# rezashkv/unlearn-ft

Hardware: AMD Instinct MI355X
Metric: bilevel train-step images/sec @512^2 pruned-SD2.1 (higher is better)
Workload: dtype bf16; 1 GPU; BASELINE configs[1] model+batch (MAC-budget-0.55 SD-2.1 student [ratio 0.556, 223.7 GMAC/img] + dense teacher [402.1 GMAC/img], B=8/GPU, 64x64 latents = 512^2 px, losses 1.0 ddpm(min-SNR 5) + 2.0 distill + 0.1 block) under the bilevel cadence of configs[2] (upper concept-suppression step every 10th iteration, second AdamW); global_batch=8, parallelism=dp1, student_params=483766084, weights=random-init, attention_precision=activation dtype, dist_backend=none, rccl_ranks=0, dp_mode=allreduce, teacher_prefetch=True

## Files before the change

### include/pdmk.h

```cpp
#ifndef PDMK_H
#define PDMK_H
#include <stdint.h>
#ifdef __cplusplus
extern "C" {
#endif

#define PDMK_F32 0
#define PDMK_BF16 1

typedef void* pdmk_stream;

int pdmk_version(void);

#define PDMK_A_ROWK 0
#define PDMK_A_CONV 1
#define PDMK_A_COLK 2
#define PDMK_B_ROWK 0
#define PDMK_B_COLK 1
#define PDMK_B_COLK_CONV 2

typedef struct pdmk_gemm_args {
    const void* A;
    const void* B;
    void* C;
    const float* bias;
    const float* rowvec;
    const void* R;
    float* colsum_out;
    int32_t M, N, K;
    int32_t lda, ldb, ldc, ldr;
    int32_t rows_per_b;
    int32_t a_mode, b_mode;
    int32_t conv_b, conv_hi, conv_wi, conv_ci, conv_ho, conv_wo, conv_mode, conv_ld;
    int32_t dtype;
    int32_t out_f32;
    int32_t accumulate;
    int32_t splitk;
    float alpha;
    int32_t ldrv;
    int32_t epilogue;
    int32_t ldc2;
    void* C2;
    int64_t* colstat;
    int32_t cs_ld;
    int32_t cs_col0;
    const float* ln_gamma;
    const float* ln_beta;
    float* ln_stats;
    void* ln_out;
    int32_t ld_ln_out;
    float ln_eps;
} pdmk_gemm_args;
int pdmk_gemm_ln_supported(const pdmk_gemm_args* args);

#define PDMK_EPI_NONE 0
#define PDMK_EPI_GEGLU 1
#define PDMK_EPI_GEGLU_BWD 2

int pdmk_gemm(const pdmk_gemm_args* args, pdmk_stream stream);
int pdmk_conv_up2_supported(int B, int H, int W, int Ci, int Co, int dtype);
int pdmk_groupnorm_apply_colstat(const void* x, void* y, const float* gamma, const float* beta, float* stats, const int64_t* colstat,
                                 int cs_ld, int cs_col0, int B, int HW, int C, int ldx, int ldy, int G, int gs, float eps,
                                 int silu, int dtype, pdmk_stream stream);
int pdmk_up2_pack_weights(const float* w3, void* wp, void* wpt, int Co, int Ci, int dtype, pdmk_stream stream);
int pdmk_up2_combine_wgrad(const float* dwp, float* dw3, int Co, int Ci, pdmk_stream stream);
#define PDMK_COLSTAT_SCALE 1073741824.0
#define PDMK_GEMM_GROUP_MAX 8
int pdmk_gemm_group(const pdmk_gemm_args* args, int n, pdmk_stream stream, int32_t* grouped_out);
int pdmk_gemm_plan(const pdmk_gemm_args* args, pdmk_stream stream, int32_t* splitk_out);
int pdmk_gemm_last_candidate(void);
int pdmk_gemm_candidate_name(int a_mode, int b_mode, int id, char* buf, int n);
int pdmk_splitk_finish(const float* ws, void* C, const float* bias, const float* rowvec, const void* R, int64_t M,
                       int N, int ldc, int ldr, int rows_per_b, int ldrv , int nslab ,
                       int accumulate, int dtype, pdmk_stream stream);
int pdmk_splitk_finish_colstat(const float* ws, void* C, const float* bias, const float* rowvec, const void* R, int64_t M,
                               int N, int ldc, int ldr, int rows_per_b, int ldrv, int nslab, int accumulate, int64_t* colstat,
                               int cs_ld, int cs_col0, int dtype, pdmk_stream stream);
#define PDMK_SLAB_GROUP_MAX 32
typedef struct pdmk_slab_item {
    const float* ws;
    float* dst;
    int64_t n;
    int32_t nslab, pad_;
} pdmk_slab_item;
int pdmk_splitk_finish_group(const pdmk_slab_item* items, int n_items, pdmk_stream stream);
int64_t pdmk_gemm_splitk_workspace_bytes(int64_t M, int N, int splitk);

int pdmk_plan_export(const char* path);
int pdmk_plan_import(const char* path);
int pdmk_plan_size(void);
int pdmk_plan_clear(void);
int pdmk_debug_scratch_violations(void);

int pdmk_groupnorm_fwd(const void* x, void* y, const float* gamma, const float* beta, float* stats, double* ws,
                       int B, int HW, int C, int ldx, int ldy, int G, int gs, float eps, int silu, int dtype,
                       pdmk_stream stream);
int pdmk_groupnorm_bwd(const void* x, const void* dy, void* dx, const float* gamma, const float* beta,
                       const float* stats, float* dgamma, float* dbeta, double* ws, float* part_ws,
                       int64_t part_ws_elems, int B, int HW, int C, int ldx, int lddy, int lddx, int G, int gs,
                       int silu, int accumulate_dx, const void* add, int ldadd, int dtype, pdmk_stream stream);
#define PDMK_PARTIAL_GROUP_MAX 32
typedef struct pdmk_partial_item {
    const float* part;
    float* out0;
    float* out1;
    int32_t nblk, n;
} pdmk_partial_item;
int pdmk_groupnorm_bwd_partial_dims(int B, int HW, int C, int G, int gs, int dtype, int32_t* nblk, int32_t* n);
int pdmk_layernorm_bwd_partial_dims(int M, int C, int32_t* nblk, int32_t* n);
int pdmk_reduce_partials_group(const pdmk_partial_item* items, int n_items, pdmk_stream stream);
int64_t pdmk_groupnorm_workspace_bytes(int B, int G);
int64_t pdmk_groupnorm_bwd_part_workspace_bytes(int G, int gs);

int pdmk_layernorm_fwd(const void* x, void* y, const float* gamma, const float* beta, float* stats, int M, int C,
                       int ldx, int ldy, float eps, int dtype, pdmk_stream stream);
int pdmk_layernorm_bwd(const void* x, const void* dy, void* dx, const float* gamma, const float* stats,
                       float* dgamma, float* dbeta, float* part_ws, int64_t part_ws_elems ,
                       int M, int C, int ldx, int lddy, int lddx, int accumulate_dx, const void* add, int ldadd, int dtype,
                       pdmk_stream stream);
int64_t pdmk_layernorm_bwd_part_workspace_bytes(int M, int C);

int pdmk_attn_fwd(const void* q, const void* k, const void* v, void* o, float* lse, int B, int H, int Nq, int Nk,
                  int64_t q_bs, int q_ld, int64_t k_bs, int k_ld, int64_t v_bs, int v_ld, int64_t o_bs, int o_ld,
                  float scale, int dtype, pdmk_stream stream);
int pdmk_attn_bwd(const void* q, const void* k, const void* v, const void* o, const void* d_o, const float* lse,
                  float* delta, void* dq, void* dk, void* dv, int B, int H, int Nq, int Nk, int64_t q_bs, int q_ld,
                  int64_t k_bs, int k_ld, int64_t v_bs, int v_ld, int64_t o_bs, int o_ld, int64_t dq_bs, int dq_ld,
                  int64_t dk_bs, int dk_ld, int64_t dv_bs, int dv_ld, float scale, float* ws, int64_t ws_elems,
                  int dtype, pdmk_stream stream);
int64_t pdmk_attn_bwd_workspace_bytes(int B, int H, int Nq, int Nk);

int pdmk_geglu_fwd(const void* x, void* y, int M, int F, int ldx, int ldy, int layout, int dtype, pdmk_stream stream);
int pdmk_geglu_bwd(const void* x, const void* dy, void* dx, int M, int F, int ldx, int lddy, int lddx, int layout,
                   int dtype, pdmk_stream stream);
int pdmk_silu_fwd(const void* x, void* y, int64_t n, int dtype, pdmk_stream stream);
int pdmk_quantize_e4m3(const void* x, void* y, int64_t n, int dtype, pdmk_stream stream);
int pdmk_silu_bwd(const void* x, const void* dy, void* dx, int64_t n, int dtype, pdmk_stream stream);
int pdmk_copy2d(const void* src, void* dst, int64_t rows, int cols, int lds, int ldd, int accumulate, int dtype,
                pdmk_stream stream);
// ... 113 lines not shown
```

### unlearn-ft_amd/csrc/abi_util.hip

```cpp
#include "common.h"

extern "C" int64_t pdmk_gemm_splitk_workspace_bytes(int64_t M, int N, int splitk) {
    if (M <= 0 || N <= 0) return -1;
    return (int64_t)(splitk > 1 ? splitk : 1) * M * N * 4;
}

extern "C" int64_t pdmk_groupnorm_workspace_bytes(int B, int G) {
    if (B <= 0 || G <= 0) return -1;
    return (int64_t)B * G * 64 * 8;
}

extern "C" int64_t pdmk_groupnorm_bwd_part_workspace_bytes(int G, int gs) {
    if (G <= 0 || gs <= 0) return -1;
    return (int64_t)2048 * 2 * G * gs * 4;
}

extern "C" int64_t pdmk_layernorm_bwd_part_workspace_bytes(int M, int C) {
    if (M <= 0 || C <= 0) return -1;
    return ((int64_t)M / 16 + 1) * 2 * C * 4;
}

extern "C" int64_t pdmk_attn_bwd_workspace_bytes(int B, int H, int Nq, int Nk) {
    if (B <= 0 || H <= 0 || Nq <= 0 || Nk <= 0) return -1;
    if (!(Nk <= 128 && Nq >= 512)) return 0;
    return (int64_t)2 * 16 * B * H * Nk * 64 * 4;
}
```

### unlearn-ft_amd/csrc/gemm.hip

```cpp
#include <cstdio>
#include <cstdlib>
#include <cstring>
#include <map>
#include <mutex>
#include <vector>

#include "common.h"
#include <algorithm>

namespace {

#define PDMK_GEMM_NBUF 2
#ifndef PDMK_GEMM_PF2
#define PDMK_GEMM_PF2 0
#endif
constexpr int BM = 128, BN = 128;
template <typename T, int KCHUNKS, int NW> struct TileCfg {
    static constexpr int NTHREADS = 64 * NW;
    static constexpr int IM = 8 / NW * 2;
    static constexpr int TPR = NTHREADS / 128;
    static constexpr int NLD = KCHUNKS / TPR;
    static constexpr int ROW_BYTES = KCHUNKS == 8 ? 144 : 96;
    static constexpr int OPERAND_BYTES = 128 * ROW_BYTES;
    static constexpr int CH = Mma<T>::CH;
// ... 446 lines not shown

struct PlanKey {
    int v[10];
    bool operator<(const PlanKey& o) const { return memcmp(v, o.v, sizeof v) < 0; }
};
std::mutex g_plan_mu;
std::map<PlanKey, int> g_plan_cfg;
std::map<PlanKey, int> g_plan_sk;
thread_local int g_last_candidate = -1;
bool g_plan_file_loaded = false;

void plan_file_load() {
    if (g_plan_file_loaded) return;
    g_plan_file_loaded = true;
    const char* path = getenv("PDMK_PLAN_CACHE");
    if (!path) return;
    FILE* f = fopen(path, "r");
    if (!f) return;
    int ver = 0;
    if (fscanf(f, " pdmk-plan %d", &ver) != 1 || ver != pdmk_version()) {
        fclose(f);
        return;
    }
    char kind;
    PlanKey k;
    int val;
    while (fscanf(f, " %c %d %d %d %d %d %d %d %d %d %d %d", &kind, &k.v[0], &k.v[1], &k.v[2], &k.v[3], &k.v[4], &k.v[5],
                  &k.v[6], &k.v[7], &k.v[8], &k.v[9], &val) == 12) {
        if (kind == 'c') g_plan_cfg[k] = val;
        else if (kind == 's') g_plan_sk[k] = val;
    }
    fclose(f);
}
void plan_file_append(char kind, const PlanKey& k, int val) {
    const char* path = getenv("PDMK_PLAN_CACHE");
    if (!path) return;
    FILE* probe = fopen(path, "r");
    int ver = 0;
    const bool fresh = !probe || fscanf(probe, " pdmk-plan %d", &ver) != 1 || ver != pdmk_version();
    if (probe) fclose(probe);
    FILE* f = fopen(path, fresh ? "w" : "a");
    if (!f) return;
    if (fresh) fprintf(f, "pdmk-plan %d\n", pdmk_version());
    fprintf(f, "%c %d %d %d %d %d %d %d %d %d %d %d\n", kind, k.v[0], k.v[1], k.v[2], k.v[3], k.v[4], k.v[5], k.v[6], k.v[7],
            k.v[8], k.v[9], val);
    fclose(f);
}
void* g_scratch = nullptr;
size_t g_scratch_bytes = 0;

PlanKey make_key(const pdmk_gemm_args& g, int sk) {
    PlanKey k;
    const bool cv = g.a_mode == PDMK_A_CONV || g.b_mode == PDMK_B_COLK_CONV;
    const int slabw = (g.a_mode == PDMK_A_COLK && g.accumulate == 2) ? 1000 : 0;
    const int v[10] = {g.M, g.N, g.K, g.a_mode, g.b_mode, (cv ? g.conv_mode : 100 * g.epilogue) + slabw, cv ? g.conv_hi : 0,
                       cv ? g.conv_wi : 0, cv ? g.conv_ci : 0, sk};
    memcpy(k.v, v, sizeof v);
    return k;
}

bool ring_eligible(const pdmk_gemm_args& g) {
    return g.dtype == PDMK_BF16 && g.b_mode == PDMK_B_ROWK && g.a_mode != PDMK_A_COLK;
}

bool wgrad_eligible(const pdmk_gemm_args& g) {
    return g.dtype == PDMK_BF16 && g.a_mode == PDMK_A_COLK && g.b_mode != PDMK_B_ROWK && g.out_f32 &&
           (g.b_mode == PDMK_B_COLK || g.conv_mode <= 2 || (g.conv_mode >= 5 && g.conv_mode <= 8));
}

bool operand_bytes(const pdmk_gemm_args& g, long* ab, long* bb) {
    const long in_px = (long)g.conv_b * g.conv_hi * g.conv_wi * ((g.a_mode == PDMK_A_CONV && g.conv_mode >= 9) ? 4 : 1);
    const long conv_bytes = ((in_px - 1) * g.conv_ld + g.conv_ci) * 2;
    const long krows = (g.a_mode == PDMK_A_COLK && g.b_mode == PDMK_B_COLK_CONV && g.conv_mode >= 5) ? 4L * g.K : (long)g.K;
    *ab = g.a_mode == PDMK_A_ROWK ? ((long)(g.M - 1) * g.lda + g.K) * 2
        : g.a_mode == PDMK_A_CONV ? conv_bytes : ((krows - 1) * g.lda + g.M) * 2;
    *bb = g.b_mode == PDMK_B_ROWK ? ((long)(g.N - 1) * g.ldb + g.K) * 2
        : g.b_mode == PDMK_B_COLK ? ((long)(g.K - 1) * g.ldb + g.N) * 2 : conv_bytes;
    return *ab < (1L << 31) && *bb < (1L << 31);
}

int launch_legacy(const pdmk_gemm_args& g, hipStream_t st) {
    if (g.colstat) return -2;
    if ((g.a_mode == PDMK_A_CONV || g.b_mode == PDMK_B_COLK_CONV) && g.conv_mode >= 5) return -2;
    const long nblocks = (long)((g.M + 127) / 128) * ((g.N + 127) / 128) * (g.splitk > 1 ? g.splitk : 1);
    long ab, bb;
    if (dma_mode() && (nblocks >= 384 || dma_mode() == 2) && ring_eligible(g) && (g.K % 32) == 0 && operand_bytes(g, &ab, &bb)) {
        const int rc = pdmk_gemm_dma_launch(g, st, ab, bb);
        if (rc <= 0) return rc;
    }
    return g.dtype == PDMK_BF16 ? launch<bf16>(g, st) : launch<float>(g, st);
}

int launch_candidate(const pdmk_gemm_args& g, hipStream_t st, int id) {
    if (id <= 0) return launch_legacy(g, st);
    long ab, bb;
    if (!operand_bytes(g, &ab, &bb)) return 1;
    if (g.a_mode == PDMK_A_COLK) return pdmk_wgrad_ring_launch(g, st, ab, bb, id - 1);
    return pdmk_gemm_ring_launch(g, st, ab, bb, id - 1);
}

static int debug_scratch();
long out_rows(const pdmk_gemm_args& g) {
    const bool phase_fwd = g.a_mode == PDMK_A_CONV && g.conv_mode >= 5 && g.conv_mode <= 8;
    if (phase_fwd && debug_scratch() == 2 && 3L * g.M * g.N * 4 + 4096 <= (1L << 20)) return (long)g.M;
    return phase_fwd ? 4L * g.M : (long)g.M;
}

bool can_tune(hipStream_t st) {
    if (!tune_mode() || !ring_mode()) return false;
    hipStreamCaptureStatus cs = hipStreamCaptureStatusNone;
    if (hipStreamIsCapturing(st, &cs) != hipSuccess) { (void)hipGetLastError(); return false; }
    return cs == hipStreamCaptureStatusNone;
}

constexpr size_t kCanaryBytes = 1 << 20;
size_t g_scratch_req = 0;
int g_scratch_violations = 0;
static int debug_scratch() { static int c = INT32_MIN; return env_int("PDMK_DEBUG_SCRATCH", 0, &c); }
static_assert(kCanaryBytes == (1 << 20), "out_rows() sizes its deliberate overrun against the band");

bool ensure_scratch(size_t bytes) {
    if (debug_scratch()) {
        if (g_scratch) (void)hipFree(g_scratch);
        g_scratch = nullptr;
        g_scratch_bytes = 0;
        bytes = (bytes + 255) & ~(size_t)255;
        if (hipMalloc(&g_scratch, bytes + kCanaryBytes) != hipSuccess) { (void)hipGetLastError(); return false; }
        if (hipMemset(reinterpret_cast<char*>(g_scratch) + bytes, 0xA5, kCanaryBytes) != hipSuccess) { (void)hipGetLastError(); return false; }
        (void)hipDeviceSynchronize();
        g_scratch_bytes = bytes + kCanaryBytes;
        g_scratch_req = bytes;
        return true;
    }
    if (bytes <= g_scratch_bytes) return true;
    if (g_scratch) (void)hipFree(g_scratch);
    g_scratch = nullptr;
    g_scratch_bytes = 0;
    if (hipMalloc(&g_scratch, bytes) != hipSuccess) { (void)hipGetLastError(); return false; }
    g_scratch_bytes = bytes;
    return true;
}

bool scratch_check() {
    if (!debug_scratch() || !g_scratch) return true;
    (void)hipDeviceSynchronize();
    std::vector<unsigned char> host(kCanaryBytes);
    if (hipMemcpy(host.data(), reinterpret_cast<char*>(g_scratch) + g_scratch_req, kCanaryBytes, hipMemcpyDeviceToHost) != hipSuccess) {
        (void)hipGetLastError();
        return false;
    }
    for (size_t i = 0; i < kCanaryBytes; ++i)
        if (host[i] != 0xA5) {
            ++g_scratch_violations;
            fprintf(stderr, "[pdmk] tuner scratch overrun: byte %zu behind a %zu-byte scratch was overwritten\n", i, g_scratch_req);
            return false;
        }
    return true;
}

float time_candidate(const pdmk_gemm_args& a, hipStream_t st, int id, float* ws, void* fin_out, hipEvent_t e0, hipEvent_t e1) {
    static const int reps = getenv("PDMK_TUNE_REPS") ? std::max(1, atoi(getenv("PDMK_TUNE_REPS"))) : 3;
    auto once = [&]() -> int {
        if (a.splitk > 1 && a.a_mode != PDMK_A_COLK) {
            const int rc = launch_candidate(a, st, id);
            if (rc) return rc;
            return pdmk_splitk_finish(ws, fin_out, nullptr, nullptr, nullptr, a.M, a.N, a.N, 0, 1, 0, a.splitk, 0, a.dtype,
                                      st);
        }
        return launch_candidate(a, st, id);
    };
    if (once() != 0) { (void)hipGetLastError(); return 1e30f; }
    float best = 1e30f;
    for (int round = 0; round < 2; ++round) {
        (void)hipEventRecord(e0, st);
        for (int r = 0; r < reps; ++r)
            if (once() != 0) { (void)hipGetLastError(); return 1e30f; }
        (void)hipEventRecord(e1, st);
        if (hipEventSynchronize(e1) != hipSuccess) { (void)hipGetLastError(); return 1e30f; }
        float ms = 0.f;
        (void)hipEventElapsedTime(&ms, e0, e1);
        if (ms < best) best = ms;
    }
    float us = best * 1000.f / reps;
    if (a.a_mode == PDMK_A_COLK && a.accumulate == 2) us += (float)(a.splitk + 1) * (float)a.M * (float)a.N * 4.f / 4.0e6f;
    return us;
}

int tune_cfg(const pdmk_gemm_args& g, hipStream_t st, int sk, float* t_out) {
    const size_t out_bytes = (size_t)out_rows(g) * g.N * 4;
    if (!ensure_scratch((size_t)(sk > 1 ? sk : 1) * out_bytes + out_bytes + (size_t)g.M * 4 + 256)) return -1;
    (void)hipDeviceSynchronize();
    hipEvent_t e0, e1;
    if (hipEventCreate(&e0) != hipSuccess || hipEventCreate(&e1) != hipSuccess) { (void)hipGetLastError(); return -1; }
    pdmk_gemm_args a = g;
    float* ws = reinterpret_cast<float*>(g_scratch);
    void* out2 = reinterpret_cast<char*>(g_scratch) + (size_t)(sk > 1 ? sk : 1) * out_bytes;
    a.accumulate = 0;
    a.splitk = sk;
    a.ldc = g.N;
    a.colstat = nullptr;
    if (g.epilogue == PDMK_EPI_GEGLU_BWD) a.ldc = 2 * g.N;
    else a.C2 = nullptr;
    if (a.colsum_out)
        a.colsum_out = reinterpret_cast<float*>(reinterpret_cast<char*>(out2) + out_bytes);
    if (g.a_mode == PDMK_A_COLK) {
        a.C = ws;
        if (g.accumulate == 2 && sk > 1) a.accumulate = 2;
    }
    else if (sk > 1) { a.C = ws; a.out_f32 = 1; a.accumulate = 2; a.bias = nullptr; a.rowvec = nullptr; a.R = nullptr; }
    else a.C = out2;
    int best = -1;
    float bt = 1e30f;
    const int ncand = 1 + (g.a_mode == PDMK_A_COLK ? pdmk_wgrad_ring_num_configs() : pdmk_gemm_ring_num_configs());
    for (int id = g.epilogue ? 1 : 0; id < ncand; ++id) {
        const float t = time_candidate(a, st, id, ws, out2, e0, e1);
        if (t < bt) { bt = t; best = id; }
    }
    (void)hipEventDestroy(e0);
    (void)hipEventDestroy(e1);
    if (getenv("PDMK_TUNE_LOG"))
        fprintf(stderr, "[pdmk tune] M=%d N=%d K=%d amode=%d cmode=%d sk=%d -> cand %d (%.1f us)\n", g.M, g.N, g.K, g.a_mode,
                g.conv_mode, sk, best, bt);
    if (!scratch_check()) return -1;
    *t_out = bt;
    return best;
}

int heuristic_cfg(const pdmk_gemm_args& g) {
    if (!ring_mode()) return 0;
    if (g.a_mode == PDMK_A_COLK) return (g.b_mode == PDMK_B_COLK_CONV || g.conv_mode >= 5) ? 2 : 0;
    return 1 + pdmk_gemm_ring_pick(g);
}

int heuristic_wgrad_sk(const pdmk_gemm_args& g) {
    const int tiles = ((g.M + 127) / 128) * ((g.N + 127) / 128);
    const int nk = g.K / 64 > 0 ? g.K / 64 : 1;
    int s = 512 / (tiles > 0 ? tiles : 1);
    if (s > nk / 16) s = nk / 16;
    if (s > 64) s = 64;
    return s < 1 ? 1 : s;
}

int heuristic_sk(const pdmk_gemm_args& g) {
    if (g.N & 3) return 1;
    const bool conv0 = g.a_mode == PDMK_A_CONV && g.conv_mode == 0;
    const int bm = conv0 ? (g.M >= 8192 ? 256 : 128) : (g.M >= 8192 ? 128 : 64);
    const int bn = conv0 ? 160 : 128;
    const long tiles = (long)((g.M + bm - 1) / bm) * ((g.N + bn - 1) / bn);
    const int nk = (g.K + 63) / 64;
    if (tiles >= 160 || nk < 30) return 1;
    long s = (256 + tiles - 1) / tiles;
    if (s > nk / 8) s = nk / 8;
    if (conv0 && s > (g.conv_ci + 63) / 64) s = (g.conv_ci + 63) / 64;
    return s < 1 ? 1 : (s > 16 ? 16 : (int)s);
}

}

static int validate_args(const pdmk_gemm_args& g) {
    if (!g.A || !g.B || !g.C) return -1;
    if (g.M <= 0 || g.N <= 0 || g.K <= 0) return -1;
    const int ch = g.dtype == PDMK_BF16 ? 8 : 4;
    const int g4 = 4 * ch;
    if (g.dtype != PDMK_BF16 && g.dtype != PDMK_F32) return -2;
    if (g.a_mode != PDMK_A_COLK && (g.K % g4)) return -1;
    if (((uintptr_t)g.A | (uintptr_t)g.B) & 15) return -1;
    if (g.a_mode == PDMK_A_ROWK && (g.lda % ch)) return -1;
    if (g.a_mode == PDMK_A_COLK && ((g.lda % ch) || (g.M % g4))) return -1;
    if (g.b_mode == PDMK_B_ROWK && (g.ldb % ch)) return -1;
    if (g.b_mode == PDMK_B_COLK && ((g.ldb % ch) || (g.N % g4))) return -1;
    if (g.a_mode == PDMK_A_CONV || g.b_mode == PDMK_B_COLK_CONV) {
        if (g.conv_ci <= 0 || (g.conv_ci % g4) || (g.conv_ld % ch) || g.conv_mode < 0 || g.conv_mode > 13) return -1;
        if (g.conv_mode >= 5) {
            if (g.dtype != PDMK_BF16 || g.conv_ho != g.conv_hi || g.conv_wo != g.conv_wi) return -2;
            if (g.b_mode == PDMK_B_COLK_CONV && g.conv_mode > 8) return -1;
        }
        if (g.conv_mode == 4 && (g.b_mode == PDMK_B_COLK_CONV || (g.conv_hi & 1) || (g.conv_wi & 1))) return -1;
        if (g.conv_b <= 0 || g.conv_hi <= 0 || g.conv_wi <= 0 || g.conv_ho <= 0 || g.conv_wo <= 0) return -1;
        const long px = (long)g.conv_b * g.conv_ho * g.conv_wo;
        if (px >= (1L << 30) || (long)g.conv_b * g.conv_hi * g.conv_wi >= (1L << 30)) return -1;
        const int ntaps = g.conv_mode == 13 ? 16 : (g.conv_mode >= 5 ? 4 : 9);
        if (g.a_mode == PDMK_A_CONV && (g.M != px || g.K != ntaps * g.conv_ci)) return -1;
        if (g.b_mode == PDMK_B_COLK_CONV && (g.K != px || g.N != ntaps * g.conv_ci)) return -1;
        if (g.conv_mode >= 5 && (long)g.conv_b * g.conv_hi * g.conv_wi * 4 >= (1L << 30)) return -1;
        const bool half = g.conv_mode == 1 || g.conv_mode == 4, twice = g.conv_mode == 2 || g.conv_mode == 3;
        const int eh = half ? (g.conv_hi + 1) / 2 : (twice ? 2 * g.conv_hi : g.conv_hi);
        const int ew = half ? (g.conv_wi + 1) / 2 : (twice ? 2 * g.conv_wi : g.conv_wi);
        if (g.conv_ho != eh || g.conv_wo != ew) return -1;
    }
    if (g.splitk > 1 && !(g.out_f32 || g.dtype == PDMK_F32)) return -1;
    if (g.accumulate == 2 && (g.splitk <= 1 || !(g.out_f32 || g.dtype == PDMK_F32) || g.bias || g.rowvec || g.R)) return -1;
    if (g.accumulate < 0 || g.accumulate > 2) return -1;
    if (g.rowvec && g.rows_per_b <= 0) return -1;
    if (g.epilogue != PDMK_EPI_NONE) {
        if (g.epilogue != PDMK_EPI_GEGLU && g.epilogue != PDMK_EPI_GEGLU_BWD) return -2;
        if (g.dtype != PDMK_BF16 || g.a_mode != PDMK_A_ROWK || g.b_mode != PDMK_B_ROWK || g.out_f32) return -2;
        if (g.epilogue == PDMK_EPI_GEGLU) {
            if ((g.N % 16) || (g.ldc % 8) || (g.C2 && (g.ldc2 % 8)) || g.splitk > 1 || g.accumulate || g.R || g.rowvec ||
                g.alpha != 1.0f || (g.K % 8))
                return -1;
        } else {
            if ((g.N % 8) || (g.ldc % 8) || !g.C2 || (g.ldc2 % 8) || g.splitk > 1 || g.accumulate || g.R || g.rowvec || g.bias ||
                g.alpha != 1.0f || (g.K % 8) || (((uintptr_t)g.C2 | (uintptr_t)g.C) & 15))
                return -1;
        }
        if (!ring_mode()) return -2;
    }
    if (g.colstat) {
        if (g.dtype != PDMK_BF16 || g.a_mode == PDMK_A_COLK || g.b_mode != PDMK_B_ROWK || g.out_f32 || g.epilogue) return -2;
        if (g.rows_per_b <= 0 || (g.rows_per_b % 64) || (g.M % 64) || (g.N % 8) || (g.ldc % 8) || (g.R && (g.ldr % 8)) ||
            g.splitk > 1 || g.accumulate == 2 || g.cs_col0 < 0 || g.cs_ld < g.cs_col0 + g.N || (g.K % 8))
            return -1;
        if (g.a_mode == PDMK_A_CONV && g.conv_mode >= 9) return -1;
        if (!ring_mode()) return -2;
    }
    return 0;
}

int pdmk_gemm_rowblock_launch(const pdmk_gemm_args& g, hipStream_t st, long a_bytes, long b_bytes, int id, bool dry);
int pdmk_gemm_rowblock_num_configs();
static int ln_candidate(const pdmk_gemm_args& g, long* ab, long* bb) {
    if (g.dtype != PDMK_BF16 || g.a_mode != PDMK_A_ROWK || g.b_mode != PDMK_B_ROWK || g.splitk > 1 || g.colstat || g.out_f32 ||
        !ring_mode() || !operand_bytes(g, ab, bb))
        return -1;
    for (int id = 0; id < pdmk_gemm_rowblock_num_configs(); ++id)
        if (pdmk_gemm_rowblock_launch(g, nullptr, *ab, *bb, id, true) == 0) return id;
    return -1;
}
extern "C" int pdmk_gemm_ln_supported(const pdmk_gemm_args* a) {
    if (!a || !a->ln_gamma || validate_args(*a)) return 0;
    long ab, bb;
    return ln_candidate(*a, &ab, &bb) >= 0 ? 1 : 0;
}

extern "C" int pdmk_gemm(const pdmk_gemm_args* a, pdmk_stream stream) {
    if (!a) return -1;
    const pdmk_gemm_args& g = *a;
    if (const int vrc = validate_args(g)) return vrc;
    hipStream_t st = reinterpret_cast<hipStream_t>(stream);
    g_last_candidate = 0;
    if (g.ln_gamma) {
        long ab, bb;
        const int id = ln_candidate(g, &ab, &bb);
        if (id < 0) return -2;
        const int rc = pdmk_gemm_rowblock_launch(g, st, ab, bb, id, false);
        g_last_candidate = 1 + pdmk_gemm_ring_num_configs() - pdmk_gemm_rowblock_num_configs() + id;
        return rc == 1 ? -2 : rc;
    }
    if (!(ring_eligible(g) && (g.K % 8) == 0) && !wgrad_eligible(g)) return launch_legacy(g, st);
    if ((g.a_mode == PDMK_A_COLK ? forced_wcfg() >= 0 : forced_cfg() >= 0) && !(g.epilogue && forced_cfg() == 0)) {
        const int rc = launch_candidate(g, st, g.a_mode == PDMK_A_COLK ? forced_wcfg() : forced_cfg());
        g_last_candidate = rc == 1 ? 0 : (g.a_mode == PDMK_A_COLK ? forced_wcfg() : forced_cfg());
        if (g.epilogue && rc == 1) return -2;
        const bool phase = (g.a_mode == PDMK_A_CONV || g.b_mode == PDMK_B_COLK_CONV) && g.conv_mode >= 5;
        if (!((phase || g.colstat) && rc == 1)) return rc == 1 ? launch_legacy(g, st) : rc;
    }
    const int sk = g.splitk > 1 ? g.splitk : 1;
    int id;
    {
        std::lock_guard<std::mutex> lk(g_plan_mu);
        plan_file_load();
        const PlanKey key = make_key(g, sk);
        auto it = g_plan_cfg.find(key);
        if (it != g_plan_cfg.end()) id = it->second;
        else if (can_tune(st)) {
            float t;
            id = tune_cfg(g, st, sk, &t);
            if (id < 0) id = heuristic_cfg(g);
            g_plan_cfg[key] = id;
            plan_file_append('c', key, id);
        } else id = heuristic_cfg(g);
    }
    if ((g.epilogue || g.colstat) && id <= 0) id = 1 + pdmk_gemm_ring_pick(g);
    int rc = launch_candidate(g, st, id);
    if (g.colstat && rc == 1) {
        id = 1 + pdmk_gemm_ring_pick(g);
        rc = launch_candidate(g, st, id);
    }
    if (g.epilogue && rc == 1) return -2;
    g_last_candidate = rc == 1 ? 0 : id;
    return rc == 1 ? launch_legacy(g, st) : rc;
}

int pdmk_gemm_ring_group_launch(const pdmk_gemm_args* gs, int n, hipStream_t st, const long* a_bytes, const long* b_bytes, int id);
int pdmk_wgrad_ring_group_launch(const pdmk_gemm_args* gs, int n, hipStream_t st, const long* a_bytes, const long* b_bytes, int id);
static int group_mode() { static int c = INT32_MIN; return env_int("PDMK_GEMM_GROUP", 1, &c); }
static int forced_group() { static int c = INT32_MIN; return env_int("PDMK_GROUP_CFG", -1, &c); }

namespace {

std::map<std::vector<int>, int> g_group_plan;

int member_plan(const pdmk_gemm_args& g, hipStream_t st) {
    const int sk = g.splitk > 1 ? g.splitk : 1;
    std::lock_guard<std::mutex> lk(g_plan_mu);
    plan_file_load();
    const PlanKey key = make_key(g, sk);
    auto it = g_plan_cfg.find(key);
    if (it != g_plan_cfg.end()) return it->second;
    if (!can_tune(st)) return heuristic_cfg(g);
    float t;
    int id = tune_cfg(g, st, sk, &t);
    if (id < 0) id = heuristic_cfg(g);
    g_plan_cfg[key] = id;
    plan_file_append('c', key, id);
    return id;
}

int group_launch(const pdmk_gemm_args* a, int n, hipStream_t st, int id) {
    long ab[PDMK_GEMM_GROUP_MAX], bb[PDMK_GEMM_GROUP_MAX];
    for (int i = 0; i < n; ++i)
        if (!operand_bytes(a[i], &ab[i], &bb[i])) return 1;
    if (id <= 0) return 1;
    if (a[0].a_mode == PDMK_A_COLK) return pdmk_wgrad_ring_group_launch(a, n, st, ab, bb, id - 1);
    return pdmk_gemm_ring_group_launch(a, n, st, ab, bb, id - 1);
}

template <typename F> float time_us(F fn, hipStream_t st, hipEvent_t e0, hipEvent_t e1, int reps = 3) {
    if (fn() != 0) { (void)hipGetLastError(); return 1e30f; }
    float best = 1e30f;
    for (int round = 0; round < 2; ++round) {
        (void)hipEventRecord(e0, st);
        for (int r = 0; r < reps; ++r)
            if (fn() != 0) { (void)hipGetLastError(); return 1e30f; }
        (void)hipEventRecord(e1, st);
        if (hipEventSynchronize(e1) != hipSuccess) { (void)hipGetLastError(); return 1e30f; }
        float ms = 0.f;
        (void)hipEventElapsedTime(&ms, e0, e1);
        if (ms < best) best = ms;
    }
    return best * 1000.f / reps;
}

int tune_group(const pdmk_gemm_args* a, int n, const int* ids, hipStream_t st) {
    pdmk_gemm_args t[PDMK_GEMM_GROUP_MAX];
    size_t off[PDMK_GEMM_GROUP_MAX + 1];
    off[0] = 0;
    for (int i = 0; i < n; ++i) {
        const size_t out = (size_t)out_rows(a[i]) * (size_t)a[i].N * 4;
        const size_t slabs = (a[i].accumulate == 2 && a[i].splitk > 1) ? (size_t)a[i].splitk : 1;
        off[i + 1] = off[i] + ((out * slabs + (size_t)a[i].M * 4 + 1023) & ~(size_t)1023);
    }
    {
        std::lock_guard<std::mutex> lk(g_plan_mu);
        if (!ensure_scratch(off[n] + 256)) return -1;
    }
    (void)hipDeviceSynchronize();
    for (int i = 0; i < n; ++i) {
        t[i] = a[i];
        char* base = reinterpret_cast<char*>(g_scratch) + off[i];
        t[i].C = base;
        t[i].ldc = a[i].N;
        t[i].colstat = nullptr;
        if (t[i].epilogue == PDMK_EPI_GEGLU_BWD) t[i].ldc = 2 * a[i].N;
        else t[i].C2 = nullptr;
        if (t[i].accumulate == 1) t[i].accumulate = 0;
        if (t[i].epilogue == PDMK_EPI_GEGLU) t[i].ldc = a[i].N / 2;
        if (t[i].colsum_out)
            t[i].colsum_out = reinterpret_cast<float*>(base + (off[i + 1] - off[i]) - (((size_t)a[i].M * 4 + 15) & ~(size_t)15));
    }
    hipEvent_t e0, e1;
    if (hipEventCreate(&e0) != hipSuccess || hipEventCreate(&e1) != hipSuccess) { (void)hipGetLastError(); return -1; }
    const float t_sep = time_us([&]() -> int {
        for (int i = 0; i < n; ++i) {
            int rc = launch_candidate(t[i], st, ids[i]);
            if (rc == 1) rc = launch_legacy(t[i], st);
            if (rc) return rc;
        }
        return 0;
    }, st, e0, e1);
    int best = -1;
    float bt = t_sep * 0.98f;
    int cands[PDMK_GEMM_GROUP_MAX + 12], nc = 0;
    for (int i = 0; i < n; ++i) cands[nc++] = ids[i];
    cands[nc++] = heuristic_cfg(a[0]);
    if (a[0].a_mode == PDMK_A_CONV)
        for (int h = 0; h < 4; ++h) cands[nc++] = 1 + 12 + h;
    if (a[0].a_mode == PDMK_A_COLK && a[0].b_mode == PDMK_B_COLK)
        for (int w = 0; w < 5; ++w) cands[nc++] = 1 + w;
    for (int i = 0; i < nc; ++i) {
        bool seen = cands[i] <= 0;
        for (int j = 0; j < i; ++j) seen = seen || cands[j] == cands[i];
        if (seen) continue;
        const float tg = time_us([&]() -> int { return group_launch(t, n, st, cands[i]); }, st, e0, e1);
        if (tg < bt) { bt = tg; best = cands[i]; }
    }
    (void)hipEventDestroy(e0);
    (void)hipEventDestroy(e1);
    if (getenv("PDMK_TUNE_LOG")) {
        fprintf(stderr, "[pdmk group] n=%d", n);
        for (int i = 0; i < n; ++i) fprintf(stderr, " (%d,%d,%d|a%d sk%d id%d)", a[i].M, a[i].N, a[i].K, a[i].a_mode, a[i].splitk, ids[i]);
        fprintf(stderr, " separate %.1f us -> %s %d (%.1f us)\n", t_sep, best > 0 ? "grouped cand" : "separate", best, best > 0 ? bt : t_sep);
    }
    {
        std::lock_guard<std::mutex> lk(g_plan_mu);
        if (!scratch_check()) return -1;
    }
    return best;
}

}

extern "C" int pdmk_gemm_group(const pdmk_gemm_args* a, int n, pdmk_stream stream, int32_t* grouped_out) {
    if (grouped_out) *grouped_out = 0;
    if (!a || n < 1 || n > PDMK_GEMM_GROUP_MAX) return -1;
    bool any_ln = false;
    for (int i = 0; i < n; ++i) {
        if (const int vrc = validate_args(a[i])) return vrc;
        any_ln = any_ln || a[i].ln_gamma;
    }
    hipStream_t st = reinterpret_cast<hipStream_t>(stream);
    auto separate = [&]() -> int {
        for (int i = 0; i < n; ++i)
            if (const int rc = pdmk_gemm(&a[i], stream)) return rc;
        return 0;
    };
    if (n > 1 && forced_group() >= 1 && !any_ln) {
        const int rc = group_launch(a, n, st, forced_group());
        if (rc == 0) {
            g_last_candidate = forced_group();
            if (grouped_out) *grouped_out = n;
            return 0;
        }
        return rc == 1 ? separate() : rc;
    }
    if (n == 1 || any_ln || !group_mode() || !ring_mode() || forced_cfg() >= 0 || forced_wcfg() >= 0) return separate();
    bool fw = true, wg = true;
    for (int i = 0; i < n; ++i) {
        fw = fw && ring_eligible(a[i]) && (a[i].K % 8) == 0 && (a[i].a_mode == a[0].a_mode);
        wg = wg && wgrad_eligible(a[i]) && (a[i].b_mode == a[0].b_mode);
    }
    if (!fw && !wg) return separate();
    int ids[PDMK_GEMM_GROUP_MAX];
    std::vector<int> key;
    for (int i = 0; i < n; ++i) {
        ids[i] = member_plan(a[i], st);
        if ((a[i].epilogue || a[i].colstat) && ids[i] <= 0) ids[i] = 1 + pdmk_gemm_ring_pick(a[i]);
        const PlanKey k = make_key(a[i], a[i].splitk > 1 ? a[i].splitk : 1);
        key.insert(key.end(), k.v, k.v + 10);
        key.push_back(a[i].accumulate);
    }
    int id = -2;
    {
        std::lock_guard<std::mutex> lk(g_plan_mu);
        auto it = g_group_plan.find(key);
        if (it != g_group_plan.end()) id = it->second;
    }
    if (id == -2) {
        if (can_tune(st)) {
            id = tune_group(a, n, ids, st);
            std::lock_guard<std::mutex> lk(g_plan_mu);
            g_group_plan[key] = id;
        } else {
            id = ids[0];
            for (int i = 1; i < n; ++i)
                if (ids[i] != ids[0]) id = -1;
        }
    }
    if (id > 0) {
        const int rc = group_launch(a, n, st, id);
        if (rc == 0) {
            g_last_candidate = id;
            if (grouped_out) *grouped_out = n;
            return 0;
        }
        if (rc != 1) return rc;
    }
    return separate();
}

extern "C" int pdmk_gemm_last_candidate(void) { return g_last_candidate; }
int pdmk_gemm_ring_name(int id, int conv, char* buf, int n);
int pdmk_wgrad_ring_name(int id, int conv, char* buf, int n);
extern "C" int pdmk_gemm_candidate_name(int a_mode, int b_mode, int id, char* buf, int n) {
    if (!buf || n <= 0) return -1;
    if (id <= 0) {
        snprintf(buf, n, "igemm_kernel / pdmk_dma::igemm_dma_kernel (K-step-32)");
        return 0;
    }
    if (a_mode == PDMK_A_COLK) return pdmk_wgrad_ring_name(id - 1, b_mode == PDMK_B_COLK_CONV, buf, n);
    return pdmk_gemm_ring_name(id - 1, a_mode == PDMK_A_CONV, buf, n);
}

extern "C" int pdmk_gemm_plan(const pdmk_gemm_args* a, pdmk_stream stream, int32_t* splitk_out) {
    if (!a || !splitk_out) return -1;
    const pdmk_gemm_args& g = *a;
    hipStream_t st = reinterpret_cast<hipStream_t>(stream);
    *splitk_out = 1;
    if (g.M <= 0 || g.N <= 0 || g.K <= 0) return -1;
    if ((g.N & 3) || g.epilogue) return 0;
    const bool wg = wgrad_eligible(g);
    if (g.a_mode == PDMK_A_COLK && !wg) {
        *splitk_out = heuristic_wgrad_sk(g);
        return 0;
    }
    if (!wg && (!ring_eligible(g) || (g.K % 8) || forced_cfg() >= 0)) {
        *splitk_out = heuristic_sk(g);
        return 0;
    }
    std::lock_guard<std::mutex> lk(g_plan_mu);
    plan_file_load();
    const PlanKey key0 = make_key(g, 0);
    auto it = g_plan_sk.find(key0);
    if (it != g_plan_sk.end()) { *splitk_out = it->second; return 0; }
    if (!can_tune(st) || !a->A || !a->B) { *splitk_out = wg ? heuristic_wgrad_sk(g) : heuristic_sk(g); return 0; }
    const int tiles = ((g.M + 127) / 128) * ((g.N + 127) / 128);
    const int nk = (g.K + 63) / 64;
    const int cands[12] = {1, 2, 3, 4, 6, 8, 12, 16, 24, 32, 48, 64};
    int best_sk = 1;
    float bt = 1e30f;
    for (int c = 0; c < 12; ++c) {
        const int sk = cands[c];
        if (wg) {
            if (sk > 1 && (nk / sk < 4 || (long)tiles * sk > 1280)) continue;
            if ((long)tiles * sk * 4 < 128 && sk < 64 && nk / (2 * sk) >= 4) continue;
        } else if (sk > 16 || (sk > 1 && (tiles > 200 || nk < 10 || nk / sk < 3 || (long)tiles * sk > 768))) continue;
        float t = 1e30f;
        const int id = tune_cfg(g, st, sk, &t);
        if (id < 0) continue;
        g_plan_cfg[make_key(g, sk)] = id;
        plan_file_append('c', make_key(g, sk), id);
        static const float margin = getenv("PDMK_SPLIT_MARGIN") ? 1.0f - 0.01f * (float)atof(getenv("PDMK_SPLIT_MARGIN")) : 0.97f;
        if (t < bt * (sk > 1 ? margin : 1.0f)) { bt = t; best_sk = sk; }
    }
    g_plan_sk[key0] = best_sk;
    plan_file_append('s', key0, best_sk);
    *splitk_out = best_sk;
    return 0;
}

extern "C" int pdmk_plan_size(void) {
    std::lock_guard<std::mutex> lk(g_plan_mu);
    return (int)(g_plan_cfg.size() + g_plan_sk.size());
}
extern "C" int pdmk_plan_export(const char* path) {
    if (!path) return -1;
    std::lock_guard<std::mutex> lk(g_plan_mu);
    FILE* f = fopen(path, "w");
    if (!f) return -1;
    fprintf(f, "pdmk-plan %d\n", pdmk_version());
    for (int pass = 0; pass < 2; ++pass)
        for (const auto& kv : (pass ? g_plan_sk : g_plan_cfg)) {
            const PlanKey& k = kv.first;
            fprintf(f, "%c %d %d %d %d %d %d %d %d %d %d %d\n", pass ? 's' : 'c', k.v[0], k.v[1], k.v[2], k.v[3], k.v[4], k.v[5],
                    k.v[6], k.v[7], k.v[8], k.v[9], kv.second);
        }
    return fclose(f) == 0 ? 0 : -1;
}
extern "C" int pdmk_plan_import(const char* path) {
    if (!path) return -1;
    std::lock_guard<std::mutex> lk(g_plan_mu);
    FILE* f = fopen(path, "r");
    if (!f) return -1;
    int ver = 0;
    if (fscanf(f, " pdmk-plan %d", &ver) != 1 || ver != pdmk_version()) {
        fclose(f);
        return -2;
    }
    char kind;
    PlanKey k;
    int val, n = 0;
    while (fscanf(f, " %c %d %d %d %d %d %d %d %d %d %d %d", &kind, &k.v[0], &k.v[1], &k.v[2], &k.v[3], &k.v[4], &k.v[5],
                  &k.v[6], &k.v[7], &k.v[8], &k.v[9], &val) == 12) {
        if (kind == 'c') g_plan_cfg[k] = val;
        else if (kind == 's') g_plan_sk[k] = val;
        ++n;
    }
    fclose(f);
    return n;
}
extern "C" int pdmk_plan_clear(void) {
    std::lock_guard<std::mutex> lk(g_plan_mu);
    g_plan_cfg.clear();
    g_plan_sk.clear();
    g_group_plan.clear();
    if (g_scratch) (void)hipFree(g_scratch);
    g_scratch = nullptr;
    g_scratch_bytes = 0;
    return 0;
}

extern "C" int pdmk_debug_scratch_violations(void) {
    std::lock_guard<std::mutex> lk(g_plan_mu);
    return g_scratch_violations;
}

extern "C" int pdmk_version(void) { return 121; }
```

### unlearn-ft_amd/csrc/gemm_ring.hip

```cpp
#include "common.h"

#include <stdio.h>
#include <stdlib.h>

#ifndef PDMK_WGRAD_XCD
#define PDMK_WGRAD_XCD 1
#endif
#ifndef PDMK_HALO_PAIRS
#define PDMK_HALO_PAIRS 1
#endif
#ifndef PDMK_RING_SPLIT_ISSUE
#define PDMK_RING_SPLIT_ISSUE 0
#endif
#ifndef PDMK_HALO_SPLIT_ISSUE
#define PDMK_HALO_SPLIT_ISSUE 1
#endif

#ifndef PDMK_PRIO
#define PDMK_PRIO 0
#endif

namespace pdmk_ring {

constexpr int BK = 64, NT = 512;
// ... 5 lines not shown
};

struct LC {
    unsigned bx, by, gx, gy;
};
__device__ __forceinline__ LC lc_plain() { return LC{blockIdx.x, blockIdx.y, gridDim.x, gridDim.y}; }
__device__ __forceinline__ LC lc_split_xcd() {
    const unsigned gx = gridDim.x, gy = gridDim.y;
    if (gy == 1) return LC{blockIdx.x, 0u, gx, 1u};
    const unsigned t = (unsigned)xcd_remap((int)(blockIdx.y * gx + blockIdx.x), (int)(gx * gy));
    const unsigned z = t / gx;
    return LC{t - z * gx, z, gx, gy};
}
__device__ __forceinline__ bool lc_group(const pdmk_gemm_group_dev& gg, int& pi, LC& lc) {
    const unsigned b = blockIdx.x;
    pi = 0;
#pragma unroll
    for (int i = 1; i < PDMK_GEMM_GROUP_MAX; ++i)
        if (i < gg.n && b >= (unsigned)gg.start[i]) pi = i;
    const unsigned local = b - (unsigned)gg.start[pi];
    const unsigned gx = (unsigned)gg.gx[pi], gy = (unsigned)gg.gy[pi];
    if (local >= gx * gy) return false;
    const unsigned t = gy > 1 ? (unsigned)xcd_remap((int)local, (int)(gx * gy)) : local;
    const unsigned z = t / gx;
    lc = LC{t - z * gx, z, gx, gy};
    return true;
}

__device__ __forceinline__ int conv_src_pixel(const ConvGeom& g, int b, int oy, int ox, int tap) {
    if (g.mode >= 5) {
        const int ph = g.mode - 5, vy = oy + (tap >> 1) - 1 + (ph >> 1), vx = ox + (tap & 1) - 1 + (ph & 1);
        const bool ok = (unsigned)vy < (unsigned)g.hi && (unsigned)vx < (unsigned)g.wi && tap < 4;
        return ok ? (b * g.hi + vy) * g.wi + vx : -1;
    }
    const int ky = (tap * 11) >> 5;
    const int kx = tap - 3 * ky;
    const bool s2 = g.mode == 1 || g.mode == 4, up = g.mode == 2 || g.mode == 3;
    const int pad = g.mode == 4 ? 0 : 1;
    const int vy = (s2 ? 2 * oy : oy) + ky - pad, vx = (s2 ? 2 * ox : ox) + kx - pad;
    const int hv = up ? 2 * g.hi : g.hi, wv = up ? 2 * g.wi : g.wi;
    bool ok = (unsigned)vy < (unsigned)hv && (unsigned)vx < (unsigned)wv && tap < 9;
    if (g.mode == 3) ok = ok && (((vy | vx) & 1) == 0);
    const int iy = up ? (vy >> 1) : vy, ix = up ? (vx >> 1) : vx;
    return ok ? (b * g.hi + iy) * g.wi + ix : -1;
}

__device__ __forceinline__ void wait_vmcnt_dyn(int n) { pdmk_wait_vmcnt(n); }
__device__ __forceinline__ void prio_static(int wave) {
    if (PDMK_PRIO == 1 && wave >= 4) __builtin_amdgcn_s_setprio(1);
}
#define PDMK_PRIO_UP() do { if (PDMK_PRIO == 2) __builtin_amdgcn_s_setprio(1); } while (0)
#define PDMK_PRIO_DOWN() do { if (PDMK_PRIO == 2) __builtin_amdgcn_s_setprio(0); } while (0)

template <int BM, int NJ, int LDS_BYTES, bool TILE2D = false, bool OUTMAP = false>
__device__ __forceinline__ void ring_epilogue(const pdmk_gemm_args& g, const LC wgc, f32x4 (&acc)[BM / 64][NJ], unsigned char* smem,
                                              int m0, int n0, int tw = 0, int img_w = 0) {
    auto row_of = [&](int l) { return TILE2D ? m0 + (l / tw) * img_w + (l % tw) : m0 + l; };
    auto out_row = [&](int m) -> long {
        if (!OUTMAP) return (long)m;
        const int hw = g.conv_hi * g.conv_wi, b = m / hw, rem = m - b * hw, y = rem / g.conv_wi, x = rem - y * g.conv_wi;
        const int ph = g.conv_mode - 5;
        return ((long)(b * 2 * g.conv_hi + 2 * y + (ph >> 1)) * (2 * g.conv_wi) + 2 * x + (ph & 1));
    };
    constexpr int BN = 32 * NJ, IM = BM / 64;
    const int tid = threadIdx.x, lane = tid & 63, wave = __builtin_amdgcn_readfirstlane(tid >> 6);
    const int wm = wave >> 1, wn = wave & 1;
    const bool first = wgc.by == 0;
    const bool slab = g.accumulate == 2;
    const bool atomic = wgc.gy > 1 && !slab;
    const bool acc1 = g.accumulate == 1;
    const bool f32out = g.out_f32 != 0;
    const bool vec8 = ((g.N & 7) == 0) && ((g.ldc & 7) == 0) && (g.R == nullptr || (g.ldr & 7) == 0);
    constexpr int SROW = BN + 4;
    constexpr int C8 = BN / 8;
    constexpr int ITEMS = (64 * C8 + NT - 1) / NT;
    constexpr int RS = NT / C8, CS_STRIDE = RS * C8, ITEMS_CS = (64 + RS - 1) / RS;
    constexpr bool CS_OK = RS * 2 * BN * 4 <= LDS_BYTES;
    static_assert(ITEMS_CS >= ITEMS && (CS_OK || NJ < 2), "statistics epilogue of the forward tile shapes");
    float* stage = reinterpret_cast<float*>(smem);
    static_assert(64 * SROW * 4 <= LDS_BYTES, "staging image must fit the ring");
    float* Cf = reinterpret_cast<float*>(g.C) + (slab ? (long)wgc.by * g.M * g.ldc : 0L);
    bf16* Ct = reinterpret_cast<bf16*>(g.C);
    const bf16* Rp = reinterpret_cast<const bf16*>(g.R);
    float cs1[8] = {0.f, 0.f, 0.f, 0.f, 0.f, 0.f, 0.f, 0.f}, cs2[8] = {0.f, 0.f, 0.f, 0.f, 0.f, 0.f, 0.f, 0.f};
#pragma unroll
    for (int pass = 0; pass < BM / 64; ++pass) {
        __syncthreads();
        if ((wm * 16 * IM) / 64 == pass) {
            const int lrb = (wm * 16 * IM) % 64;
#pragma unroll
            for (int i = 0; i < IM; ++i)
#pragma unroll
                for (int j = 0; j < NJ; ++j) {
                    f32x4 v = acc[i][j];
#pragma unroll
                    for (int r = 0; r < 4; ++r) v[r] *= g.alpha;
                    *reinterpret_cast<f32x4*>(stage + (lrb + i * 16 + (lane & 15)) * SROW + wn * (16 * NJ) + j * 16 + (lane >> 4) * 4) = v;
                }
        }
        if (atomic) {
            __syncthreads();
            for (int rr = 0; rr < 8; ++rr) {
                const int lr2 = wave * 8 + rr, m = row_of(pass * 64 + lr2);
                if (m >= g.M) break;
#pragma unroll
                for (int h = 0; h < (BN + 63) / 64; ++h) {
                    const int cl = h * 64 + lane, n = n0 + cl;
                    if (cl < BN && n < g.N) {
                        float v = stage[lr2 * SROW + cl];
                        if (first) {
                            if (g.bias) v += g.bias[n];
                            if (g.rowvec) v += g.rowvec[(long)(m / g.rows_per_b) * (g.ldrv ? g.ldrv : g.N) + n];
                            if (Rp) v += (float)Rp[(long)m * g.ldr + n];
                        }
                        unsafeAtomicAdd(Cf + (long)m * g.ldc + n, v);
                    }
                }
            }
        } else if (vec8 && g.epilogue == PDMK_EPI_GEGLU) {
            constexpr int C16 = BN / 16;
            constexpr int ITEMS2 = (64 * C16 + NT - 1) / NT;
            bf16* C2 = reinterpret_cast<bf16*>(g.C2);
            __syncthreads();
#pragma unroll
            for (int it = 0; it < ITEMS2; ++it) {
                const int item = tid + it * NT;
                const int lr2 = item / C16, p = item - lr2 * C16;
                const int m = row_of(pass * 64 + lr2), n = n0 + p * 16;
                if (!(item < 64 * C16 && m < g.M && n < g.N)) continue;
                float v[16];
#pragma unroll
                for (int q = 0; q < 4; ++q) {
                    const f32x4 t4 = *reinterpret_cast<const f32x4*>(stage + lr2 * SROW + p * 16 + q * 4);
#pragma unroll
                    for (int r = 0; r < 4; ++r) v[q * 4 + r] = t4[r];
                }
                if (g.bias) {
#pragma unroll
                    for (int q = 0; q < 4; ++q) {
                        const float4 b4 = *reinterpret_cast<const float4*>(g.bias + n + q * 4);
                        v[q * 4] += b4.x; v[q * 4 + 1] += b4.y; v[q * 4 + 2] += b4.z; v[q * 4 + 3] += b4.w;
                    }
                }
                bf16x8 hb, gb, o;
#pragma unroll
                for (int r = 0; r < 8; ++r) { hb[r] = (bf16)v[r]; gb[r] = (bf16)v[8 + r]; }
                if (C2) {
                    st_stream(reinterpret_cast<bf16x8*>(C2 + (long)m * g.ldc2 + n), hb);
                    st_stream(reinterpret_cast<bf16x8*>(C2 + (long)m * g.ldc2 + n + 8), gb);
                }
#pragma unroll
                for (int r = 0; r < 8; ++r) o[r] = (bf16)((float)hb[r] * gelu_f((float)gb[r]));
                st_stream(reinterpret_cast<bf16x8*>(Ct + (long)m * g.ldc + (n >> 1)), o);
            }
        } else if (vec8 && g.epilogue == PDMK_EPI_GEGLU_BWD) {
            const bf16* X2 = reinterpret_cast<const bf16*>(g.C2);
            bf16x8 hb[ITEMS], gb[ITEMS];
#pragma unroll
            for (int it = 0; it < ITEMS; ++it) {
                const int item = tid + it * NT;
                const int lr2 = item / C8, c8 = item - lr2 * C8;
                const int m = row_of(pass * 64 + lr2), n = n0 + c8 * 8;
                if (item < 64 * C8 && m < g.M && n < g.N) {
                    hb[it] = *reinterpret_cast<const bf16x8*>(X2 + (long)m * g.ldc2 + 2 * n);
                    gb[it] = *reinterpret_cast<const bf16x8*>(X2 + (long)m * g.ldc2 + 2 * n + 8);
                }
            }
            __syncthreads();
#pragma unroll
            for (int it = 0; it < ITEMS; ++it) {
                const int item = tid + it * NT;
                const int lr2 = item / C8, c8 = item - lr2 * C8;
                const int m = row_of(pass * 64 + lr2), n = n0 + c8 * 8;
                if (!(item < 64 * C8 && m < g.M && n < g.N)) continue;
                const f32x4 lo = *reinterpret_cast<const f32x4*>(stage + lr2 * SROW + c8 * 8);
                const f32x4 hi = *reinterpret_cast<const f32x4*>(stage + lr2 * SROW + c8 * 8 + 4);
                bf16x8 dh, dg;
#pragma unroll
                for (int r = 0; r < 8; ++r) {
                    const float d = (float)(bf16)(r < 4 ? lo[r] : hi[r - 4]);
                    const float hv = (float)hb[it][r], gv = (float)gb[it][r];
                    dh[r] = (bf16)(d * gelu_f(gv));
                    dg[r] = (bf16)(d * hv * gelu_grad_f(gv));
                }
                st_stream(reinterpret_cast<bf16x8*>(Ct + (long)m * g.ldc + 2 * n), dh);
                st_stream(reinterpret_cast<bf16x8*>(Ct + (long)m * g.ldc + 2 * n + 8), dg);
            }
        } else if (vec8) {
            bf16x8 rres[ITEMS_CS], cprev[ITEMS_CS];
            const int istride = g.colstat ? CS_STRIDE : NT;
            const bool tid_ok = !g.colstat || tid < CS_STRIDE;
#pragma unroll
            for (int it = 0; it < ITEMS_CS; ++it) {
                const int item = tid + it * istride;
                const int lr2 = item / C8, c8 = item - lr2 * C8;
                const int m = row_of(pass * 64 + lr2), n = n0 + c8 * 8;
                const bool ok = tid_ok && item < 64 * C8 && m < g.M && n < g.N;
                const long off = out_row(m) * g.ldc + n;
                if (ok && Rp) rres[it] = *reinterpret_cast<const bf16x8*>(Rp + (long)m * g.ldr + n);
                if (ok && acc1 && !f32out) cprev[it] = *reinterpret_cast<const bf16x8*>(Ct + off);
            }
            __syncthreads();
#pragma unroll
            for (int it = 0; it < ITEMS_CS; ++it) {
                const int item = tid + it * istride;
                const int lr2 = item / C8, c8 = item - lr2 * C8;
                const int m = row_of(pass * 64 + lr2), n = n0 + c8 * 8;
                if (!(tid_ok && item < 64 * C8 && m < g.M && n < g.N)) continue;
                float v[8];
                const f32x4 lo = *reinterpret_cast<const f32x4*>(stage + lr2 * SROW + c8 * 8);
                const f32x4 hi = *reinterpret_cast<const f32x4*>(stage + lr2 * SROW + c8 * 8 + 4);
#pragma unroll
                for (int r = 0; r < 4; ++r) { v[r] = lo[r]; v[4 + r] = hi[r]; }
                if (g.bias) {
                    const float4 b0 = *reinterpret_cast<const float4*>(g.bias + n), b1 = *reinterpret_cast<const float4*>(g.bias + n + 4);
                    v[0] += b0.x; v[1] += b0.y; v[2] += b0.z; v[3] += b0.w; v[4] += b1.x; v[5] += b1.y; v[6] += b1.z; v[7] += b1.w;
                }
                if (g.rowvec) {
                    const float* rv = g.rowvec + (long)(m / g.rows_per_b) * (g.ldrv ? g.ldrv : g.N) + n;
                    const float4 b0 = *reinterpret_cast<const float4*>(rv), b1 = *reinterpret_cast<const float4*>(rv + 4);
                    v[0] += b0.x; v[1] += b0.y; v[2] += b0.z; v[3] += b0.w; v[4] += b1.x; v[5] += b1.y; v[6] += b1.z; v[7] += b1.w;
                }
                if (Rp) {
#pragma unroll
                    for (int r = 0; r < 8; ++r) v[r] += (float)rres[it][r];
                }
                const long off = out_row(m) * g.ldc + n;
                if (f32out) {
                    float4 o0 = make_float4(v[0], v[1], v[2], v[3]), o1 = make_float4(v[4], v[5], v[6], v[7]);
                    if (acc1) {
                        const float4 c0 = *reinterpret_cast<const float4*>(Cf + off), c1 = *reinterpret_cast<const float4*>(Cf + off + 4);
                        o0.x += c0.x; o0.y += c0.y; o0.z += c0.z; o0.w += c0.w;
                        o1.x += c1.x; o1.y += c1.y; o1.z += c1.z; o1.w += c1.w;
                    }
                    *reinterpret_cast<float4*>(Cf + off) = o0;
                    *reinterpret_cast<float4*>(Cf + off + 4) = o1;
                } else {
                    if (acc1) {
#pragma unroll
                        for (int r = 0; r < 8; ++r) v[r] += (float)cprev[it][r];
                    }
                    bf16x8 o;
#pragma unroll
                    for (int r = 0; r < 8; ++r) o[r] = (bf16)v[r];
                    st_stream(reinterpret_cast<bf16x8*>(Ct + off), o);
                    if (g.colstat) {
#pragma unroll
                        for (int r = 0; r < 8; ++r) {
                            const float x = (float)o[r];
                            cs1[r] += x;
                            cs2[r] += x * x;
                        }
                    }
                }
            }
            if (CS_OK && g.colstat) {
                const int mp0 = row_of(pass * 64);
                const int img = mp0 / g.rows_per_b;
                const bool flush = pass == BM / 64 - 1 || row_of((pass + 1) * 64) >= g.M || row_of((pass + 1) * 64) / g.rows_per_b != img;
                if (flush && mp0 < g.M) {
                    __syncthreads();
                    if (tid < CS_STRIDE) {
                        float* d = stage + (tid / C8) * (2 * BN) + (tid % C8) * 8;
                        *reinterpret_cast<f32x4*>(d) = f32x4{cs1[0], cs1[1], cs1[2], cs1[3]};
                        *reinterpret_cast<f32x4*>(d + 4) = f32x4{cs1[4], cs1[5], cs1[6], cs1[7]};
                        *reinterpret_cast<f32x4*>(d + BN) = f32x4{cs2[0], cs2[1], cs2[2], cs2[3]};
                        *reinterpret_cast<f32x4*>(d + BN + 4) = f32x4{cs2[4], cs2[5], cs2[6], cs2[7]};
                    }
                    __syncthreads();
                    for (int c = tid; c < 2 * BN; c += NT) {
                        const int col = c < BN ? c : c - BN;
                        if (n0 + col >= g.N) continue;
                        float sum = 0.f;
#pragma unroll
                        for (int r = 0; r < RS; ++r) sum += stage[r * (2 * BN) + c];
                        cs_add(g.colstat + ((long)img * 4 + (c < BN ? 0 : 2)) * g.cs_ld + g.cs_col0 + n0 + col, g.cs_ld, sum, c >= BN);
                    }
#pragma unroll
                    for (int r = 0; r < 8; ++r) cs1[r] = cs2[r] = 0.f;
                }
            }
        } else {
            __syncthreads();
            for (int item = tid; item < 64 * C8; item += NT) {
                const int lr2 = item / C8, c8 = item - lr2 * C8;
                const int m = row_of(pass * 64 + lr2), n = n0 + c8 * 8;
                if (m >= g.M || n >= g.N) continue;
                const float* rv = g.rowvec ? g.rowvec + (long)(m / g.rows_per_b) * (g.ldrv ? g.ldrv : g.N) : nullptr;
                const long off = out_row(m) * g.ldc + n;
                const int nv = min(8, g.N - n);
                for (int r = 0; r < nv; ++r) {
                    float x = stage[lr2 * SROW + c8 * 8 + r];
                    if (g.bias) x += g.bias[n + r];
                    if (rv) x += rv[n + r];
                    if (Rp) x += (float)Rp[(long)m * g.ldr + n + r];
                    if (f32out) Cf[off + r] = x + (acc1 ? Cf[off + r] : 0.f);
                    else Ct[off + r] = (bf16)(x + (acc1 ? (float)Ct[off + r] : 0.f));
                }
            }
        }
    }
}

constexpr int ring_smem_bytes(int BM, int NJ, int STAGES) { return STAGES * (BM * 128 + 32 * NJ * 128); }

template <bool CONV, int BM, int NJ, int STAGES, int OCC>
__device__ __forceinline__ void igemm_ring_body(const pdmk_gemm_args& g, unsigned a_bytes, unsigned b_bytes, const LC wgc,
                                                unsigned char* smem) {
    typedef Mma<bf16> MM;
    constexpr int BN = 32 * NJ;
    constexpr int IM = BM / 64;
    constexpr int A_BYTES = BM * 128, B_BYTES = BN * 128, SLOT = A_BYTES + B_BYTES;
    constexpr int NA = BM / 64;
    constexpr int NBLK_B = BN / 8, NB = (NBLK_B + 7) / 8;
    static_assert(STAGES >= 2 && STAGES * SLOT * (OCC / 2) <= 160 * 1024, "ring(s) must fit the 160 KiB LDS");
    static_assert(STAGES * SLOT == ring_smem_bytes(BM, NJ, STAGES), "smem size of the kernel wrappers");

    const int tid = threadIdx.x, lane = tid & 63, wave = __builtin_amdgcn_readfirstlane(tid >> 6);
    const int wm = wave >> 1, wn = wave & 1;
    const int ntn = (g.N + BN - 1) / BN;
    const int tile = xcd_remap(wgc.bx, wgc.gx);
    const int ntm = (g.M + BM - 1) / BM;
    const bool nmajor = g.a_mode != PDMK_A_COLK && g.M <= 1024 && g.N > g.M;
    const int m0 = (nmajor ? tile % ntm : tile / ntn) * BM, n0 = (nmajor ? tile / ntm : tile % ntn) * BN;
    const int nk_total = (g.K + BK - 1) / BK;
    const int per = (nk_total + wgc.gy - 1) / wgc.gy;
    const int kt0 = wgc.by * per;
    const int kt1 = min(nk_total, kt0 + per);
    if (kt0 >= kt1 && g.accumulate != 2) return;

    const auto rsrcA = __builtin_amdgcn_make_buffer_rsrc(const_cast<void*>(g.A), (short)0, (int)a_bytes, 0x00020000);
    const auto rsrcB = __builtin_amdgcn_make_buffer_rsrc(const_cast<void*>(g.B), (short)0, (int)b_bytes, 0x00020000);
    const ConvGeom cg{g.conv_hi, g.conv_wi, g.conv_ci, g.conv_ho, g.conv_wo, g.conv_ld, g.conv_mode};

    const int sr = lane >> 3;
    const int lc = (lane & 7) ^ (((wave & 1) * 4) + (sr >> 1));
    unsigned a_base[NA], b_base[NB];
    int a_b[NA], a_oy[NA], a_ox[NA];
#pragma unroll
    for (int i = 0; i < NA; ++i) {
        a_base[i] = OOB; a_b[i] = -1; a_oy[i] = 0; a_ox[i] = 0;
        const int m = m0 + (i * 8 + wave) * 8 + sr;
        if (m < g.M) {
            if (CONV) {
                const int hw = cg.ho * cg.wo;
                a_b[i] = m / hw;
                const int rem = m - a_b[i] * hw;
                a_oy[i] = rem / cg.wo;
                a_ox[i] = rem - a_oy[i] * cg.wo;
            } else {
                a_base[i] = (unsigned)m * (unsigned)g.lda * 2u;
            }
        }
    }
#pragma unroll
    for (int i = 0; i < NB; ++i) {
        const int n = n0 + (i * 8 + wave) * 8 + sr;
        b_base[i] = (n < g.N) ? (unsigned)n * (unsigned)g.ldb * 2u : OOB;
    }
    const int nb_wave = NBLK_B / 8 + (wave < (NBLK_B % 8) ? 1 : 0);
    const int ndma = NA + nb_wave;
    int kl = kt0 * BK + lc * 8;
    int tap = 0, cc = 0;
    if (CONV) {
        tap = kl / cg.ci;
        cc = kl - tap * cg.ci;
    }

    auto issue = [&](int slot) {
        unsigned char* sa = smem + slot * SLOT;
        const bool kok = kl < g.K;
#pragma unroll
        for (int i = 0; i < NA; ++i) {
            unsigned va;
            if (CONV) {
                const int px = a_b[i] >= 0 ? conv_src_pixel(cg, a_b[i], a_oy[i], a_ox[i], tap) : -1;
                va = px >= 0 ? ((unsigned)px * (unsigned)cg.ld + (unsigned)cc) * 2u : OOB;
            } else {
                va = (a_base[i] != OOB && kok) ? a_base[i] + (unsigned)kl * 2u : OOB;
            }
            __builtin_amdgcn_raw_ptr_buffer_load_lds(rsrcA, (lds_void*)(sa + (i * 8 + wave) * 1024), 16, (int)va, 0, 0, 0);
        }
// ... 18 lines not shown
#pragma unroll
        for (int j = 0; j < NJ; ++j) acc[i][j] = f32x4{0.f, 0.f, 0.f, 0.f};

    const int fr = lane & 15;
    const int fsw = (fr >> 1) & 7;
    const unsigned fch0 = (unsigned)(((lane >> 4) ^ fsw) * 16), fch1 = (unsigned)(((4 + (lane >> 4)) ^ fsw) * 16);
    const unsigned a_row = (unsigned)(wm * (16 * IM) + fr) * 128u;
    const unsigned b_row = (unsigned)(wn * (16 * NJ) + fr) * 128u;

#pragma unroll
    for (int s = 0; s < STAGES - 1; ++s)
        if (kt0 + s < kt1) issue(s);

    int slot = 0;
    prio_static(wave);
    for (int kt = kt0; kt < kt1; ++kt) {
        if (STAGES == 2) {
            asm volatile("s_waitcnt vmcnt(0)" ::: "memory");
        } else if (kt + STAGES - 1 <= kt1) {
            if ((NBLK_B % 8) == 0 || wave < (NBLK_B % 8)) asm volatile("s_waitcnt vmcnt(%0)" ::"n"((STAGES - 2) * (NA + NB)) : "memory");
            else asm volatile("s_waitcnt vmcnt(%0)" ::"n"((STAGES - 2) * (NA + NB - 1)) : "memory");
        } else {
            wait_vmcnt_dyn(min(STAGES - 2, kt1 - 1 - kt) * ndma);
        }
        __builtin_amdgcn_s_barrier();
        const bool late = PDMK_RING_SPLIT_ISSUE && wave >= 4;
        if (!late && kt + STAGES - 1 < kt1) issue(slot == 0 ? STAGES - 1 : slot - 1);
        const unsigned char* sa = smem + slot * SLOT;
        const unsigned char* sb = sa + A_BYTES;
#pragma unroll
        for (int kk = 0; kk < 2; ++kk) {
            const unsigned fch = kk ? fch1 : fch0;
            bf16x8 af[IM], bf[NJ];
#pragma unroll
            for (int i = 0; i < IM; ++i) af[i] = *reinterpret_cast<const bf16x8*>(sa + a_row + fch + i * 2048);
#pragma unroll
            for (int j = 0; j < NJ; ++j) bf[j] = *reinterpret_cast<const bf16x8*>(sb + b_row + fch + j * 2048);
            PDMK_PRIO_UP();
#pragma unroll
            for (int i = 0; i < IM; ++i)
#pragma unroll
                for (int j = 0; j < NJ; ++j) acc[i][j] = MM::mma(bf[j], af[i], acc[i][j]);
            PDMK_PRIO_DOWN();
            if (kk == 0 && late) {
                __builtin_amdgcn_sched_barrier(0);
                if (kt + STAGES - 1 < kt1) issue(slot == 0 ? STAGES - 1 : slot - 1);
                __builtin_amdgcn_sched_barrier(0);
            }
        }
        slot = slot + 1 == STAGES ? 0 : slot + 1;
    }

    if (PDMK_PRIO == 1) __builtin_amdgcn_s_setprio(0);
    ring_epilogue<BM, NJ, STAGES * SLOT>(g, wgc, acc, smem, m0, n0);
}

template <bool CONV, int BM, int NJ, int STAGES, int OCC>
__global__ __launch_bounds__(NT, OCC) void igemm_ring_kernel(pdmk_gemm_args g, unsigned a_bytes, unsigned b_bytes) {
    __shared__ __attribute__((aligned(1024))) unsigned char smem[ring_smem_bytes(BM, NJ, STAGES)];
    igemm_ring_body<CONV, BM, NJ, STAGES, OCC>(g, a_bytes, b_bytes, lc_plain(), smem);
}
template <bool CONV, int BM, int NJ, int STAGES, int OCC>
__global__ __launch_bounds__(NT, OCC) void igemm_ring_group_kernel(pdmk_gemm_group_dev gg) {
    __shared__ __attribute__((aligned(1024))) unsigned char smem[ring_smem_bytes(BM, NJ, STAGES)];
    int pi;
    LC wgc;
    if (!lc_group(gg, pi, wgc)) return;
    igemm_ring_body<CONV, BM, NJ, STAGES, OCC>(gg.p[pi], gg.a_bytes[pi], gg.b_bytes[pi], wgc, smem);
}

constexpr int halo_smem_bytes(int NJ, int BSTAGES, int PMAX) { return 2 * PMAX * 128 + BSTAGES * 32 * NJ * 128; }

template <int BM, int NJ, int BSTAGES, int PMAX, int NTAPS = 9>
__device__ __forceinline__ void conv_halo_body(const pdmk_gemm_args& g, unsigned a_bytes, unsigned b_bytes, int tw, const LC wgc,
                                               unsigned char* smem) {
    typedef Mma<bf16> MM;
    constexpr int BN = 32 * NJ, IM = BM / 64;
    constexpr int P_BYTES = PMAX * 128, B_BYTES = BN * 128;
    constexpr int NBLK_B = BN / 8, NB = (NBLK_B + 7) / 8;
    constexpr int NPW = (PMAX / 8 + 7) / 8;
    static_assert(PMAX % 8 == 0 && (NTAPS == 4 || NPW <= 9 - (BSTAGES - 1)), "whole pieces; next block's patch issued before its first weight tile");
    static_assert(NTAPS == 9 || (NTAPS == 4 && BSTAGES >= 4 && PDMK_HALO_PAIRS), "phase convs run the two-taps-per-barrier path");
    const int phm = NTAPS == 4 ? g.conv_mode - 5 : 0;
    const bool merged = NTAPS == 4 && phm == 8;
    const bool dgr = NTAPS == 4 && phm >= 4;
    const int pa_ = merged ? 0 : (phm & 3) >> 1, pb_ = merged ? 0 : phm & 1;
    const int ta0 = dgr ? 1 - pa_ : pa_, tb0 = dgr ? 1 - pb_ : pb_;
    static_assert(2 * P_BYTES + BSTAGES * B_BYTES <= 160 * 1024, "LDS");
    static_assert(64 * (BN + 4) * 4 <= 2 * P_BYTES, "epilogue staging fits the patch buffers");
    static_assert(2 * P_BYTES + BSTAGES * B_BYTES == halo_smem_bytes(NJ, BSTAGES, PMAX), "smem size of the kernel wrappers");
    unsigned char* const bring = smem + 2 * P_BYTES;

    const int tid = threadIdx.x, lane = tid & 63, wave = __builtin_amdgcn_readfirstlane(tid >> 6);
    const int wm = wave >> 1, wn = wave & 1;
    const int ntn = (g.N + BN - 1) / BN;
    const int tile = xcd_remap(wgc.bx, wgc.gx);
    const int ntm = (g.M + BM - 1) / BM;
    const bool nmajor = g.a_mode != PDMK_A_COLK && g.M <= 1024 && g.N > g.M;
    const int m0 = (nmajor ? tile % ntm : tile / ntn) * BM, n0 = (nmajor ? tile / ntm : tile % ntn) * BN;
    const int H = g.conv_hi, W = g.conv_wi, Ci = g.conv_ci, HW = H * W;
    const int ncb1 = (Ci + 63) / 64;
    const int ncb_total = (NTAPS == 4 && g.conv_mode == 13) ? 4 * ncb1 : ncb1;
    const int per = (ncb_total + wgc.gy - 1) / wgc.gy;
    const int cb0 = wgc.by * per, cb1 = min(ncb_total, cb0 + per);
    if (cb0 >= cb1 && g.accumulate != 2) return;

    const int rimg = HW >= BM ? BM / tw : H;
    const int W2 = tw + 2, pimg = (rimg + 2) * W2;
    const int nimg = HW >= BM ? 1 : BM / HW;
    const int prows = nimg * pimg;
    int img0, y0, x0 = 0;
    if (tw == W) {
        img0 = m0 / HW;
        y0 = (m0 - img0 * HW) / W;
    } else {
        const int tpr = W / tw, tpi = (H / rimg) * tpr, tm = m0 / BM;
        img0 = tm / tpi;
        const int r = tm - img0 * tpi;
        y0 = (r / tpr) * rimg;
        x0 = (r - (r / tpr) * tpr) * tw;
    }
    const int mbase = tw == W ? m0 : (img0 * H + y0) * W + x0;

    const auto rsrcA = __builtin_amdgcn_make_buffer_rsrc(const_cast<void*>(g.A), (short)0, (int)a_bytes, 0x00020000);
    const auto rsrcB = __builtin_amdgcn_make_buffer_rsrc(const_cast<void*>(g.B), (short)0, (int)b_bytes, 0x00020000);

    const int sr = lane >> 3;
    const int lcp = (lane & 7) ^ sr;
    unsigned poff[NPW];
#pragma unroll
    for (int j = 0; j < NPW; ++j) {
        const int prow = (j * 8 + wave) * 8 + sr;
        poff[j] = OOB;
        if (prow < prows) {
            const int il = prow / pimg, rem = prow - il * pimg;
            const int py = rem / W2, px = rem - py * W2;
            const int b = img0 + il, y = y0 + py - 1, x = x0 + px - 1;
            if (b < g.conv_b && (unsigned)y < (unsigned)H && (unsigned)x < (unsigned)W)
                poff[j] = (dgr ? (unsigned)((b * 2 * H + 2 * y + pa_) * (2 * W) + 2 * x + pb_)
                               : (unsigned)((b * H + y) * W + x)) * (unsigned)g.conv_ld * 2u;
        }
    }
    const int lcb = (lane & 7) ^ (((wave & 1) * 4) + (sr >> 1));
    unsigned b_base[NB];
#pragma unroll
    for (int i = 0; i < NB; ++i) {
        const int n = n0 + (i * 8 + wave) * 8 + sr;
        b_base[i] = (n < g.N) ? (unsigned)n * (unsigned)g.ldb * 2u : OOB;
    }
    const int nb_wave = NBLK_B / 8 + (wave < (NBLK_B % 8) ? 1 : 0);

    auto blk_ph = [&](int vcb) { return merged ? (vcb >= 2 * ncb1 ? (vcb >= 3 * ncb1 ? 3 : 2) : (vcb >= ncb1 ? 1 : 0)) : 0; };
    auto issue_piece = [&](int vcb, unsigned off, int jj) {
        const int ph = blk_ph(vcb), cb = vcb - ph * ncb1;
        const int ch = cb * 64 + lcp * 8;
        const unsigned pho = merged ? (unsigned)((ph >> 1) * 2 * W + (ph & 1)) * (unsigned)g.conv_ld * 2u : 0u;
        const unsigned va = (off != OOB && ch < Ci && vcb < cb1) ? off + pho + (unsigned)ch * 2u : OOB;
        __builtin_amdgcn_raw_ptr_buffer_load_lds(rsrcA, (lds_void*)(smem + (vcb & 1) * P_BYTES + (jj * 8 + wave) * 1024), 16,
// ... 127 lines not shown
        }
    } else {
    #pragma unroll
        for (int j = 0; j < NPW; ++j)
            if (nsteps > 0 && (j * 8 + wave) * 8 < prows) issue_piece(cb0, poff[j], j);
    #pragma unroll
        for (int s = 0; s < BSTAGES - 1; ++s)
            if (s < nsteps) issue_b(cb0 + s / 9, s % 9, s);

        const int n_ss = (BSTAGES - 2) * (nb_wave + 1) + 1;
        constexpr int N_SS_HI = (BSTAGES - 2) * (NB + 1) + 1;
        constexpr int N_SS_LO = (BSTAGES - 2) * NB + 1;
        int s = 0, slot_c = 0, slot_i = BSTAGES - 1;
        for (int cb = cb0; cb < cb1; ++cb) {
            const unsigned char* pbuf = smem + (cb & 1) * P_BYTES;
    #pragma unroll
            for (int i = 0; i < IM; ++i) asm volatile("" : "+v"(prow0[i]));
            const bool steady = cb > cb0 && cb + 1 < cb1;
    #pragma unroll
            for (int tap = 0; tap < 9; ++tap, ++s) {
                if (steady) {
                    if ((NBLK_B % 8) == 0 || wave < (NBLK_B % 8)) asm volatile("s_waitcnt vmcnt(%0)" ::"n"(N_SS_HI) : "memory");
                    else asm volatile("s_waitcnt vmcnt(%0)" ::"n"(N_SS_LO) : "memory");
                    __builtin_amdgcn_s_barrier();
                    constexpr int ahead = BSTAGES - 1;
                    issue_b(cb + ((tap + ahead) >= 9 ? 1 : 0), (tap + ahead) % 9, slot_i);
                    const bool own = tap < NPW && (tap * 8 + wave) * 8 < prows;
                    issue_piece(cb + 1, own ? poff[tap < NPW ? tap : 0] : poff[0], own ? tap : 0);
                    slot_i = slot_i + 1 == BSTAGES ? 0 : slot_i + 1;
                } else {
                    const bool tail = s + BSTAGES - 1 >= nsteps;
                    if (tail) wait_vmcnt_dyn(0);
                    else if (s <= BSTAGES - 2) wait_vmcnt_dyn((BSTAGES - 2 - s) * nb_wave + s * (nb_wave + 1));
                    else wait_vmcnt_dyn(n_ss);
                    __builtin_amdgcn_s_barrier();
                    if (!tail) {
                        const int sn = s + BSTAGES - 1;
                        const int cbn = cb0 + sn / 9, tapn = sn - (sn / 9) * 9;
                        issue_b(cbn, tapn, slot_i);
                        slot_i = slot_i + 1 == BSTAGES ? 0 : slot_i + 1;
                        if (tap < NPW && (tap * 8 + wave) * 8 < prows) issue_piece(cb + 1, poff[tap < NPW ? tap : 0], tap);
                        else issue_piece(cb + 1, poff[0], 0);
                    }
                }
                tap_compute(pbuf, bring + slot_c * B_BYTES, tap, []() {});
                slot_c = slot_c + 1 == BSTAGES ? 0 : slot_c + 1;
            }
        }
    }
    asm volatile("s_waitcnt vmcnt(0)" ::: "memory");
    if (PDMK_PRIO == 1) __builtin_amdgcn_s_setprio(0);
    __builtin_amdgcn_s_barrier();
    if (NTAPS == 4 && !dgr) {
        if (tw == W) ring_epilogue<BM, NJ, 2 * P_BYTES + BSTAGES * B_BYTES, false, NTAPS == 4>(g, wgc, acc, smem, m0, n0);
        else ring_epilogue<BM, NJ, 2 * P_BYTES + BSTAGES * B_BYTES, true, NTAPS == 4>(g, wgc, acc, smem, mbase, n0, tw, W);
        return;
    }
    if (tw == W) ring_epilogue<BM, NJ, 2 * P_BYTES + BSTAGES * B_BYTES>(g, wgc, acc, smem, m0, n0);
    else ring_epilogue<BM, NJ, 2 * P_BYTES + BSTAGES * B_BYTES, true>(g, wgc, acc, smem, mbase, n0, tw, W);
}

template <int BM, int NJ, int BSTAGES, int PMAX, int NTAPS = 9>
__global__ __launch_bounds__(NT, 2) void conv_halo_kernel(pdmk_gemm_args g, unsigned a_bytes, unsigned b_bytes, int tw) {
    __shared__ __attribute__((aligned(1024))) unsigned char smem[halo_smem_bytes(NJ, BSTAGES, PMAX)];
    conv_halo_body<BM, NJ, BSTAGES, PMAX, NTAPS>(g, a_bytes, b_bytes, tw, lc_plain(), smem);
}
template <int BM, int NJ, int BSTAGES, int PMAX, int NTAPS = 9>
__global__ __launch_bounds__(NT, 2) void conv_halo_group_kernel(pdmk_gemm_group_dev gg) {
    __shared__ __attribute__((aligned(1024))) unsigned char smem[halo_smem_bytes(NJ, BSTAGES, PMAX)];
    int pi;
    LC wgc;
    if (!lc_group(gg, pi, wgc)) return;
    conv_halo_body<BM, NJ, BSTAGES, PMAX, NTAPS>(gg.p[pi], gg.a_bytes[pi], gg.b_bytes[pi], gg.aux0[pi], wgc, smem);
}

constexpr int wgrad_smem_bytes(int BM, int NJ, int STAGES) { return STAGES * (64 * BM * 2 + 64 * 32 * NJ * 2); }

template <bool CONV, int BM, int NJ, int STAGES, int OCC>
__device__ __forceinline__ void wgrad_ring_body(const pdmk_gemm_args& g, int lg_wo, int lg_howo, unsigned a_bytes, unsigned b_bytes,
                                                const LC wgc, unsigned char* smem) {
    typedef Mma<bf16> MM;
    constexpr int BN = 32 * NJ, IM = BM / 64;
    constexpr int RA = BM * 2, RB = BN * 2;
    constexpr int A_BYTES = 64 * RA, B_BYTES = 64 * RB, SLOT = A_BYTES + B_BYTES;
    constexpr int PA = A_BYTES / 1024 / 8, PB = B_BYTES / 1024 / 8;
    static_assert((BM == 64 || BM == 128) && (BN == 64 || BN == 128), "tile");
    static_assert(STAGES >= 2 && STAGES * SLOT * (OCC / 2) <= 160 * 1024, "ring(s) must fit the 160 KiB LDS");
    static_assert(64 * (BN + 4) * 4 <= STAGES * SLOT, "epilogue staging");
    static_assert(STAGES * SLOT == wgrad_smem_bytes(BM, NJ, STAGES), "smem size of the kernel wrappers");

    const int tid = threadIdx.x, lane = tid & 63, wave = __builtin_amdgcn_readfirstlane(tid >> 6);
    const int wm = wave >> 1, wn = wave & 1;
    const int ntn = (g.N + BN - 1) / BN;
    const int tile = xcd_remap(wgc.bx, wgc.gx);
    const int ntm = (g.M + BM - 1) / BM;
    const bool nmajor = g.a_mode != PDMK_A_COLK && g.M <= 1024 && g.N > g.M;
    const int m0 = (nmajor ? tile % ntm : tile / ntn) * BM, n0 = (nmajor ? tile / ntm : tile % ntn) * BN;
    const int nk_total = (g.K + BK - 1) / BK;
    const int per = (nk_total + wgc.gy - 1) / wgc.gy;
    const int kt0 = wgc.by * per;
    const int kt1 = min(nk_total, kt0 + per);
    if (kt0 >= kt1 && g.accumulate != 2) return;

    const auto rsrcA = __builtin_amdgcn_make_buffer_rsrc(const_cast<void*>(g.A), (short)0, (int)a_bytes, 0x00020000);
    const auto rsrcB = __builtin_amdgcn_make_buffer_rsrc(const_cast<void*>(g.B), (short)0, (int)b_bytes, 0x00020000);
    const ConvGeom cg{g.conv_hi, g.conv_wi, g.conv_ci, g.conv_ho, g.conv_wo, g.conv_ld, g.conv_mode};

    auto lane_row = [&](int rbytes) { return rbytes == 256 ? (lane >> 4) : (lane >> 3); };
    auto lane_lc = [&](int rbytes) {
        if (rbytes == 256) return (lane & 15) ^ (((lane >> 4) | (((wave >> 1) & 1) << 2)) << 1);
        return (lane & 7) ^ (((((lane >> 3) >> 1) & 1) | ((wave & 1) << 1)) << 1);
    };
    const int a_row = lane_row(RA), b_rowl = lane_row(RB);
    const int acol = m0 + lane_lc(RA) * 8, bcol = n0 + lane_lc(RB) * 8;
    const bool a_ok = acol < g.M, b_ok = bcol < g.N;
    int b_tap = 0, b_ci = 0;
    if (CONV) {
        b_tap = bcol / cg.ci;
        b_ci = bcol - b_tap * cg.ci;
    }

    auto issue = [&](int kt, int slot) {
        unsigned char* sa = smem + slot * SLOT;
#pragma unroll
        for (int i = 0; i < PA; ++i) {
            const int piece = i * 8 + wave;
            const int kr = kt * BK + piece * (1024 / RA) + a_row;
            unsigned krs = (unsigned)kr;
            if (CONV && cg.mode >= 5 && kr < g.K) {
                const int hw = cg.ho * cg.wo, b = kr / hw, rem = kr - b * hw, oy = rem / cg.wo, ox = rem - oy * cg.wo;
                const int ph = cg.mode - 5;
                krs = (unsigned)((b * 2 * cg.ho + 2 * oy + (ph >> 1)) * (2 * cg.wo) + 2 * ox + (ph & 1));
            }
            const unsigned va = (kr < g.K && a_ok) ? (krs * (unsigned)g.lda + (unsigned)acol) * 2u : OOB;
            __builtin_amdgcn_raw_ptr_buffer_load_lds(rsrcA, (lds_void*)(sa + piece * 1024), 16, (int)va, 0, 0, 0);
        }
#pragma unroll
        for (int i = 0; i < PB; ++i) {
            const int piece = i * 8 + wave;
            const int kr = kt * BK + piece * (1024 / RB) + b_rowl;
            const bool kok = kr < g.K;
            unsigned vb = OOB;
            if (CONV) {
                if (kok && b_ok) {
                    int b, oy, ox;
                    if (lg_wo >= 0) {
                        b = kr >> lg_howo;
                        const int rem = kr & ((1 << lg_howo) - 1);
                        oy = rem >> lg_wo;
                        ox = rem & ((1 << lg_wo) - 1);
                    } else {
                        const int hw = cg.ho * cg.wo;
                        b = kr / hw;
                        const int rem = kr - b * hw;
                        oy = rem / cg.wo;
// ... 25 lines not shown
    const int f256 = (tq | ((tg & 1) << 2)) << 1, f128 = (((tq >> 1) & 1) | ((tg & 1) << 1)) << 1;
    typedef __attribute__((address_space(3))) s16x4 lds_s16x4;
    auto tr_frag = [&](const unsigned char* base, int rbytes, int kk, int col0) -> bf16x8 {
        const unsigned ch = (unsigned)(((col0 >> 3) ^ (rbytes == 256 ? f256 : f128)) | (tp >> 1));
        const unsigned char* a0 = base + (unsigned)(kk + 8 * tg + tq) * (unsigned)rbytes + ch * 16u + (unsigned)(tp & 1) * 8u;
        s16x4 lo = __builtin_amdgcn_ds_read_tr16_b64_v4i16((lds_s16x4*)(a0));
        s16x4 hi = __builtin_amdgcn_ds_read_tr16_b64_v4i16((lds_s16x4*)(a0 + 4 * rbytes));
        s16x8 v = __builtin_shufflevector(lo, hi, 0, 1, 2, 3, 4, 5, 6, 7);
        return __builtin_bit_cast(bf16x8, v);
    };

#pragma unroll
    for (int s = 0; s < STAGES - 1; ++s)
        if (kt0 + s < kt1) issue(kt0 + s, s);

    int slot = 0;
    prio_static(wave);
    for (int kt = kt0; kt < kt1; ++kt) {
        if (STAGES == 2) asm volatile("s_waitcnt vmcnt(0)" ::: "memory");
        else if (kt + STAGES - 1 <= kt1) asm volatile("s_waitcnt vmcnt(%0)" ::"n"((STAGES - 2) * (PA + PB)) : "memory");
        else wait_vmcnt_dyn(min(STAGES - 2, kt1 - 1 - kt) * (PA + PB));
        __builtin_amdgcn_s_barrier();
        if (kt + STAGES - 1 < kt1) issue(kt + STAGES - 1, slot == 0 ? STAGES - 1 : slot - 1);
        const unsigned char* sa = smem + slot * SLOT;
        const unsigned char* sb = sa + A_BYTES;
#pragma unroll
        for (int kk = 0; kk < BK; kk += 32) {
            bf16x8 af[IM], bf[NJ];
#pragma unroll
            for (int i = 0; i < IM; ++i) af[i] = tr_frag(sa, RA, kk, wm * (16 * IM) + i * 16);
#pragma unroll
            for (int j = 0; j < NJ; ++j) bf[j] = tr_frag(sb, RB, kk, wn * (16 * NJ) + j * 16);
            PDMK_PRIO_UP();
#pragma unroll
            for (int i = 0; i < IM; ++i)
#pragma unroll
                for (int j = 0; j < NJ; ++j) acc[i][j] = MM::mma(bf[j], af[i], acc[i][j]);
            PDMK_PRIO_DOWN();
            if (do_colsum) {
#pragma unroll
                for (int i = 0; i < IM; ++i) acs[i] = MM::mma(ones, af[i], acs[i]);
            }
        }
        slot = slot + 1 == STAGES ? 0 : slot + 1;
    }
    if (PDMK_PRIO == 1) __builtin_amdgcn_s_setprio(0);
    if (do_colsum && (lane >> 4) == 0) {
#pragma unroll
        for (int i = 0; i < IM; ++i) {
            const int m = m0 + wm * (16 * IM) + i * 16 + (lane & 15);
            if (m < g.M) unsafeAtomicAdd(g.colsum_out + m, acs[i][0]);
        }
    }
    ring_epilogue<BM, NJ, STAGES * SLOT>(g, wgc, acc, smem, m0, n0);
}

template <bool CONV, int BM, int NJ, int STAGES, int OCC>
__global__ __launch_bounds__(NT, OCC) void wgrad_ring_kernel(pdmk_gemm_args g, int lg_wo, int lg_howo, unsigned a_bytes,
                                                             unsigned b_bytes) {
    __shared__ __attribute__((aligned(1024))) unsigned char smem[wgrad_smem_bytes(BM, NJ, STAGES)];
    wgrad_ring_body<CONV, BM, NJ, STAGES, OCC>(g, lg_wo, lg_howo, a_bytes, b_bytes, PDMK_WGRAD_XCD ? lc_split_xcd() : lc_plain(), smem);
}
template <bool CONV, int BM, int NJ, int STAGES, int OCC>
__global__ __launch_bounds__(NT, OCC) void wgrad_ring_group_kernel(pdmk_gemm_group_dev gg) {
    __shared__ __attribute__((aligned(1024))) unsigned char smem[wgrad_smem_bytes(BM, NJ, STAGES)];
    int pi;
    LC wgc;
    if (!lc_group(gg, pi, wgc)) return;
    wgrad_ring_body<CONV, BM, NJ, STAGES, OCC>(gg.p[pi], gg.aux0[pi], gg.aux1[pi], gg.a_bytes[pi], gg.b_bytes[pi], wgc, smem);
}

struct Config {
    int bm, nj, stages, occ;
};
static const Config kConfigs[] = {
    {256, 4, 3, 2}, {256, 5, 3, 2}, {128, 4, 4, 2}, {128, 5, 4, 2}, {64, 4, 6, 2}, {64, 5, 5, 2},
    {128, 4, 2, 4}, {64, 4, 3, 4},  {64, 5, 2, 4},  {128, 6, 3, 2}, {64, 6, 4, 2},  {128, 5, 2, 4},
    {64, 2, 4, 4},  {128, 2, 3, 4}, {64, 3, 4, 4},
};
constexpr int kNumConfigs = sizeof(kConfigs) / sizeof(kConfigs[0]);
constexpr int kNumBase = 12;

static int halo_tile_w(const pdmk_gemm_args& g, int h, int splitk) {
    const bool phase = g.conv_mode >= 5 && g.conv_mode <= 13;
    if (g.a_mode != PDMK_A_CONV || !(g.conv_mode == 0 || phase) || g.conv_ho != g.conv_hi || g.conv_wo != g.conv_wi) return 0;
    if (phase && (h < 2 || !PDMK_HALO_PAIRS || g.R || (splitk > 1))) return 0;
    if ((g.conv_ci % 8) || g.conv_wi < 4) return 0;
    if (phase ? ((g.ldb % 8) || g.ldb < (g.conv_mode == 13 ? 16 : 4) * g.conv_ci) : g.ldb != 9 * g.conv_ci) return 0;
    if ((splitk > 1 ? splitk : 1) > (g.conv_ci + 63) / 64) return 0;
    const int bm = h < 2 ? 256 : 128, pmax = h < 2 ? 400 : 264;
    const int H = g.conv_hi, W = g.conv_wi, HW = H * W;
    if (HW < bm) return (bm % HW) == 0 && (bm / HW) * (H + 2) * (W + 2) <= pmax ? W : 0;
    if (HW % bm) return 0;
    static const int pref = getenv("PDMK_HALO_TW") ? atoi(getenv("PDMK_HALO_TW")) : 0;
    if (pref > 0 && pref < W && (W % pref) == 0 && (bm % pref) == 0 && (H % (bm / pref)) == 0 &&
        (bm / pref + 2) * (pref + 2) <= pmax)
        return pref;
    if ((bm % W) == 0 && (bm / W + 2) * (W + 2) <= pmax) return W;
    for (int tw = 128; tw >= 8; tw >>= 1) {
        if (tw >= W || (W % tw) || (bm % tw)) continue;
        const int rows = bm / tw;
        if ((H % rows) == 0 && (rows + 2) * (tw + 2) <= pmax) return tw;
    }
    return 0;
}
static bool halo_ok(const pdmk_gemm_args& g, int h, int splitk) { return halo_tile_w(g, h, splitk) > 0; }

static int pick_config(const pdmk_gemm_args& g, int splitk) {
    enum { R256x128, R256x160, R128x128, R128x160, R64x128, R64x160, S128x128, S64x128, S64x160, R128x192, R64x192, S128x160 };
    const bool n160 = (g.N % 160) == 0 || (g.N > 256 && (g.N % 128) != 0);
    if (g.a_mode == PDMK_A_CONV && g.conv_mode >= 5) return kNumBase + (halo_ok(g, n160 ? 2 : 3, splitk) ? (n160 ? 2 : 3) : (n160 ? 3 : 2));
    if (g.a_mode == PDMK_A_CONV && g.conv_mode == 0) {
        const long t256 = (long)((g.M + 255) / 256) * ((g.N + 159) / 160);
        const int h = (g.M >= 8192 && t256 >= 128) ? (n160 ? 0 : 1) : (n160 ? 2 : 3);
        if (halo_ok(g, h, splitk)) return kNumBase + h;
        if (halo_ok(g, h | 2, splitk)) return kNumBase + (h | 2);
    }
    if (g.M >= 8192) return n160 ? S128x160 : S128x128;
    if (g.M >= 4096) return S64x160;
    if (g.M >= 2048 && n160 && g.N >= 1280) return S64x160;
    return S64x128;
}

}

constexpr int kNumHalo = 4;
int pdmk_gemm_rowblock_num_configs();
int pdmk_gemm_rowblock_name(int id, char* buf, int n);
int pdmk_gemm_rowblock_launch(const pdmk_gemm_args& g, hipStream_t st, long a_bytes, long b_bytes, int id, bool dry = false);
static int conv_halo_launch(const pdmk_gemm_args& g, hipStream_t st, long a_bytes, long b_bytes, int id) {
    using namespace pdmk_ring;
    const int tw = halo_tile_w(g, id, g.splitk);
    if (tw <= 0) return 1;
    const int bm = id < 2 ? 256 : 128, nj = (id & 1) ? 4 : 5;
    const int sk = g.splitk > 1 ? g.splitk : 1;
    const int bn = 32 * nj;
    dim3 grid(((g.M + bm - 1) / bm) * ((g.N + bn - 1) / bn), sk);
    if (g.conv_mode >= 5) {
        if (id == 2) hipLaunchKernelGGL((conv_halo_kernel<128, 5, 4, 264, 4>), grid, dim3(NT), 0, st, g, (unsigned)a_bytes, (unsigned)b_bytes, tw);
        else hipLaunchKernelGGL((conv_halo_kernel<128, 4, 5, 264, 4>), grid, dim3(NT), 0, st, g, (unsigned)a_bytes, (unsigned)b_bytes, tw);
        return hipGetLastError() == hipSuccess ? 0 : -1000;
    }
    switch (id) {
        case 0: hipLaunchKernelGGL((conv_halo_kernel<256, 5, 3, 400>), grid, dim3(NT), 0, st, g, (unsigned)a_bytes, (unsigned)b_bytes, tw); break;
        case 1: hipLaunchKernelGGL((conv_halo_kernel<256, 4, 3, 400>), grid, dim3(NT), 0, st, g, (unsigned)a_bytes, (unsigned)b_bytes, tw); break;
        case 2: hipLaunchKernelGGL((conv_halo_kernel<128, 5, 4, 264>), grid, dim3(NT), 0, st, g, (unsigned)a_bytes, (unsigned)b_bytes, tw); break;
        case 3: hipLaunchKernelGGL((conv_halo_kernel<128, 4, 5, 264>), grid, dim3(NT), 0, st, g, (unsigned)a_bytes, (unsigned)b_bytes, tw); break;
        default: return 1;
    }
    return hipGetLastError() == hipSuccess ? 0 : -1000;
}

extern "C" int pdmk_conv_up2_supported(int B, int H, int W, int Ci, int Co, int dtype) {
    if (dtype != PDMK_BF16 || B <= 0 || H <= 0 || W <= 0 || Ci <= 0 || Co <= 0 || (Ci % 32) || (Co % 32)) return 0;
    pdmk_gemm_args g = {};
    g.a_mode = PDMK_A_CONV;
    g.b_mode = PDMK_B_ROWK;
    g.dtype = PDMK_BF16;
    g.conv_b = B;
    g.conv_hi = g.conv_ho = H;
    g.conv_wi = g.conv_wo = W;
    g.M = B * H * W;
    bool ok = true;
    for (int dir = 0; dir < 2; ++dir) {
        g.conv_mode = dir ? 13 : 5;
        g.conv_ci = dir ? Co : Ci;
        g.N = dir ? Ci : Co;
        g.K = (dir ? 16 : 4) * g.conv_ci;
        g.ldb = g.K;
        ok = ok && (pdmk_ring::halo_tile_w(g, 2, 1) > 0 || pdmk_ring::halo_tile_w(g, 3, 1) > 0);
    }
    return ok ? 1 : 0;
}

int pdmk_gemm_ring_num_configs() { return pdmk_ring::kNumConfigs + kNumHalo + pdmk_gemm_rowblock_num_configs(); }
int pdmk_gemm_ring_name(int id, int conv, char* buf, int n) {
    using namespace pdmk_ring;
    if (id >= kNumConfigs + kNumHalo) return pdmk_gemm_rowblock_name(id - (kNumConfigs + kNumHalo), buf, n);
    if (id < 0) return -1;
    if (id >= kNumBase && id < kNumBase + kNumHalo) {
        const int h = id - kNumBase;
        snprintf(buf, n, "pdmk_ring::conv_halo_kernel<%d, %d, %d, %d, 9>", h < 2 ? 256 : 128, (h & 1) ? 4 : 5,
                 h < 2 ? 3 : ((h & 1) ? 5 : 4), h < 2 ? 400 : 264);
        return 0;
    }
    const Config c = kConfigs[id < kNumBase ? id : id - kNumHalo];
    snprintf(buf, n, "pdmk_ring::igemm_ring_kernel<%s, %d, %d, %d, %d>", conv ? "true" : "false", c.bm, c.nj, c.stages, c.occ);
    return 0;
}
int pdmk_gemm_ring_pick(const pdmk_gemm_args& g) { return pdmk_ring::pick_config(g, g.splitk); }

int pdmk_gemm_ring_launch(const pdmk_gemm_args& g, hipStream_t st, long a_bytes, long b_bytes, int id) {
    using namespace pdmk_ring;
    if (g.dtype != PDMK_BF16 || g.b_mode != PDMK_B_ROWK || g.a_mode == PDMK_A_COLK) return 1;
    if ((g.K % 8) || (g.a_mode == PDMK_A_CONV && (g.conv_ci % 8))) return 1;
    if (g.ln_gamma && id < kNumConfigs + kNumHalo) return 1;
    if (id >= kNumBase && id < kNumBase + kNumHalo) return conv_halo_launch(g, st, a_bytes, b_bytes, id - kNumBase);
    if (g.a_mode == PDMK_A_CONV && g.conv_mode >= 5) return 1;
    if (id >= kNumConfigs + kNumHalo) return pdmk_gemm_rowblock_launch(g, st, a_bytes, b_bytes, id - (kNumConfigs + kNumHalo));
    if (id < 0) return 1;
    const int sk = g.splitk > 1 ? g.splitk : 1;
    const Config c = kConfigs[id < kNumBase ? id : id - kNumHalo];
    const int bn = 32 * c.nj;
    dim3 grid(((g.M + c.bm - 1) / c.bm) * ((g.N + bn - 1) / bn), sk);
    const bool conv = g.a_mode == PDMK_A_CONV;
#define PDMK_RING_GO(BMv, NJv, STv, OCv)                                                                              \
    case (BMv * 1000 + NJv * 100 + STv * 10 + OCv):                                                                   \
        if (conv) hipLaunchKernelGGL((igemm_ring_kernel<true, BMv, NJv, STv, OCv>), grid, dim3(NT), 0, st, g,         \
                                     (unsigned)a_bytes, (unsigned)b_bytes);                                           \
        else hipLaunchKernelGGL((igemm_ring_kernel<false, BMv, NJv, STv, OCv>), grid, dim3(NT), 0, st, g,             \
                                (unsigned)a_bytes, (unsigned)b_bytes);                                                \
        break;
    switch (c.bm * 1000 + c.nj * 100 + c.stages * 10 + c.occ) {
        PDMK_RING_GO(256, 4, 3, 2) PDMK_RING_GO(256, 5, 3, 2) PDMK_RING_GO(128, 4, 4, 2) PDMK_RING_GO(128, 5, 4, 2)
        PDMK_RING_GO(64, 4, 6, 2) PDMK_RING_GO(64, 5, 5, 2) PDMK_RING_GO(128, 4, 2, 4) PDMK_RING_GO(64, 4, 3, 4)
        PDMK_RING_GO(64, 5, 2, 4) PDMK_RING_GO(128, 6, 3, 2) PDMK_RING_GO(64, 6, 4, 2) PDMK_RING_GO(128, 5, 2, 4)
        PDMK_RING_GO(64, 2, 4, 4) PDMK_RING_GO(128, 2, 3, 4) PDMK_RING_GO(64, 3, 4, 4)
        default: return 1;
    }
#undef PDMK_RING_GO
    return hipGetLastError() == hipSuccess ? 0 : -1000;
}

namespace pdmk_ring {

constexpr int wgrad_halo_smem_bytes(int IMW, int STAGES) { return STAGES * (128 * (32 * IMW) * 2 + 288 * 128); }

template <int IMW, int STAGES>
__device__ __forceinline__ void conv_wgrad_halo_body(const pdmk_gemm_args& g, unsigned a_bytes, unsigned b_bytes, const LC wgc,
                                                     unsigned char* smem) {
    typedef Mma<bf16> MM;
    constexpr int PX = 128, PMAX = 288, BM = 32 * IMW, RA = BM * 2;
    constexpr int A_BYTES = PX * RA, P_BYTES = PMAX * 128, SLOT = A_BYTES + P_BYTES;
    constexpr int PA = A_BYTES / 1024 / 8;
    constexpr int NPW = (PMAX / 8 + 7) / 8;
    constexpr int NDMA = PA + NPW;
    static_assert(STAGES >= 2 && STAGES * SLOT <= 160 * 1024, "LDS");
    static_assert((IMW == 2 || IMW == 4) && BM * 68 * 4 <= STAGES * SLOT, "epilogue staging");
    static_assert(STAGES * SLOT == wgrad_halo_smem_bytes(IMW, STAGES), "smem size of the kernel wrappers");

    const int tid = threadIdx.x, lane = tid & 63, wave = __builtin_amdgcn_readfirstlane(tid >> 6);
    const int wm = wave >> 2, wn = wave & 3;
    const int Ci = g.conv_ci, H = g.conv_hi, W = g.conv_wi, HW = H * W;
    const int nct = (Ci + 63) / 64;
    const int tile = xcd_remap(wgc.bx, wgc.gx);
    const int m0 = (tile / nct) * BM, c0 = (tile - (tile / nct) * nct) * 64;
    const int nblk = (g.K + PX - 1) / PX;
    const int per = (nblk + wgc.gy - 1) / wgc.gy;
    const int kb0 = wgc.by * per, kb1 = min(nblk, kb0 + per);
    if (kb0 >= kb1 && g.accumulate != 2) return;

    const int rimg = HW >= PX ? PX / W : H;
    const int W2 = (W + 2 + 7) & ~7, pimg = (rimg + 2) * W2;
    const int nimg = HW >= PX ? 1 : PX / HW;
    const int prows = nimg * pimg;

    const auto rsrcA = __builtin_amdgcn_make_buffer_rsrc(const_cast<void*>(g.A), (short)0, (int)a_bytes, 0x00020000);
    const auto rsrcB = __builtin_amdgcn_make_buffer_rsrc(const_cast<void*>(g.B), (short)0, (int)b_bytes, 0x00020000);

    const int a_row = RA == 256 ? (lane >> 4) : (lane >> 3);
    const int a_lc = RA == 256 ? ((lane & 15) ^ (((lane >> 4) | (((wave >> 1) & 1) << 2)) << 1))
                               : ((lane & 7) ^ (((((lane >> 3) >> 1) & 1) | ((wave & 1) << 1)) << 1));
// ... 161 lines not shown
    __shared__ __attribute__((aligned(1024))) unsigned char smem[wgrad_halo_smem_bytes(IMW, STAGES)];
    int pi;
    LC wgc;
    if (!lc_group(gg, pi, wgc)) return;
    conv_wgrad_halo_body<IMW, STAGES>(gg.p[pi], gg.a_bytes[pi], gg.b_bytes[pi], wgc, smem);
}

static bool wgrad_halo_ok(const pdmk_gemm_args& g) {
    if (g.dtype != PDMK_BF16 || g.a_mode != PDMK_A_COLK || g.b_mode != PDMK_B_COLK_CONV || !g.out_f32) return false;
    if (g.conv_mode != 0 || g.conv_ho != g.conv_hi || g.conv_wo != g.conv_wi || g.alpha != 1.0f) return false;
    if ((g.conv_ci % 8) || (g.conv_ld % 8) || (g.lda % 8) || (g.M % 8) || g.N != 9 * g.conv_ci || g.conv_wi < 4) return false;
    const int H = g.conv_hi, W = g.conv_wi, HW = H * W, W2 = (W + 2 + 7) & ~7;
    if (HW >= 128) return (HW % 128) == 0 && (128 % W) == 0 && (128 / W + 2) * W2 <= 288;
    return (128 % HW) == 0 && (128 / HW) * (H + 2) * W2 <= 288;
}

}

namespace {
struct GroupGrid {
    pdmk_gemm_group_dev gg;
    unsigned total = 0;
    void add(int i, const pdmk_gemm_args& g, int tiles, int splits, long ab, long bb, int aux0 = 0, int aux1 = 0) {
        gg.start[i] = (int)total;
        gg.gx[i] = tiles;
        gg.gy[i] = splits;
        gg.a_bytes[i] = (unsigned)ab;
        gg.b_bytes[i] = (unsigned)bb;
        gg.aux0[i] = aux0;
        gg.aux1[i] = aux1;
        gg.p[i] = g;
        total += ((unsigned)tiles * (unsigned)splits + 7u) & ~7u;
    }
    void finish(int n) {
        gg.n = n;
        for (int i = n; i <= PDMK_GEMM_GROUP_MAX; ++i) gg.start[i] = (int)total;
        for (int i = n; i < PDMK_GEMM_GROUP_MAX; ++i) {
            gg.gx[i] = gg.gy[i] = 0;
            gg.a_bytes[i] = gg.b_bytes[i] = 0;
            gg.aux0[i] = gg.aux1[i] = 0;
            gg.p[i] = gg.p[0];
        }
    }
};
}

int pdmk_gemm_ring_group_launch(const pdmk_gemm_args* gs, int n, hipStream_t st, const long* a_bytes, const long* b_bytes, int id) {
    using namespace pdmk_ring;
    if (n < 2 || n > PDMK_GEMM_GROUP_MAX || id < 0) return 1;
    const bool halo = id >= kNumBase && id < kNumBase + kNumHalo;
    if (id >= kNumConfigs + kNumHalo) return 1;
    const bool conv = gs[0].a_mode == PDMK_A_CONV;
    GroupGrid G;
    for (int i = 0; i < n; ++i) {
        const pdmk_gemm_args& g = gs[i];
        if (g.dtype != PDMK_BF16 || g.b_mode != PDMK_B_ROWK || g.a_mode == PDMK_A_COLK) return 1;
        if ((g.K % 8) || (g.a_mode == PDMK_A_CONV && (g.conv_ci % 8))) return 1;
        if ((g.a_mode == PDMK_A_CONV) != conv) return 1;
        if (!halo && g.a_mode == PDMK_A_CONV && g.conv_mode >= 5) return 1;
        const int sk = g.splitk > 1 ? g.splitk : 1;
        if (halo) {
            const int h = id - kNumBase;
            const int tw = halo_tile_w(g, h, g.splitk);
            if (tw <= 0) return 1;
            const int bm = h < 2 ? 256 : 128, bn = 32 * ((h & 1) ? 4 : 5);
            G.add(i, g, ((g.M + bm - 1) / bm) * ((g.N + bn - 1) / bn), sk, a_bytes[i], b_bytes[i], tw);
        } else {
            const Config c = kConfigs[id < kNumBase ? id : id - kNumHalo];
            const int bn = 32 * c.nj;
            G.add(i, g, ((g.M + c.bm - 1) / c.bm) * ((g.N + bn - 1) / bn), sk, a_bytes[i], b_bytes[i]);
        }
    }
    G.finish(n);
    const dim3 grid(G.total);
    if (halo) {
        bool phase = gs[0].conv_mode >= 5;
        for (int i = 1; i < n; ++i)
            if ((gs[i].conv_mode >= 5) != phase) return 1;
        if (phase) {
            if (id - kNumBase == 2) hipLaunchKernelGGL((conv_halo_group_kernel<128, 5, 4, 264, 4>), grid, dim3(NT), 0, st, G.gg);
            else hipLaunchKernelGGL((conv_halo_group_kernel<128, 4, 5, 264, 4>), grid, dim3(NT), 0, st, G.gg);
            return hipGetLastError() == hipSuccess ? 0 : -1000;
        }
        switch (id - kNumBase) {
            case 0: hipLaunchKernelGGL((conv_halo_group_kernel<256, 5, 3, 400>), grid, dim3(NT), 0, st, G.gg); break;
            case 1: hipLaunchKernelGGL((conv_halo_group_kernel<256, 4, 3, 400>), grid, dim3(NT), 0, st, G.gg); break;
            case 2: hipLaunchKernelGGL((conv_halo_group_kernel<128, 5, 4, 264>), grid, dim3(NT), 0, st, G.gg); break;
            default: hipLaunchKernelGGL((conv_halo_group_kernel<128, 4, 5, 264>), grid, dim3(NT), 0, st, G.gg); break;
        }
        return hipGetLastError() == hipSuccess ? 0 : -1000;
    }
    const Config c = kConfigs[id < kNumBase ? id : id - kNumHalo];
#define PDMK_RING_GGO(BMv, NJv, STv, OCv)                                                                             \
    case (BMv * 1000 + NJv * 100 + STv * 10 + OCv):                                                                   \
        if (conv) hipLaunchKernelGGL((igemm_ring_group_kernel<true, BMv, NJv, STv, OCv>), grid, dim3(NT), 0, st, G.gg); \
        else hipLaunchKernelGGL((igemm_ring_group_kernel<false, BMv, NJv, STv, OCv>), grid, dim3(NT), 0, st, G.gg);   \
        break;
    switch (c.bm * 1000 + c.nj * 100 + c.stages * 10 + c.occ) {
        PDMK_RING_GGO(256, 4, 3, 2) PDMK_RING_GGO(256, 5, 3, 2) PDMK_RING_GGO(128, 4, 4, 2) PDMK_RING_GGO(128, 5, 4, 2)
        PDMK_RING_GGO(64, 4, 6, 2) PDMK_RING_GGO(64, 5, 5, 2) PDMK_RING_GGO(128, 4, 2, 4) PDMK_RING_GGO(64, 4, 3, 4)
        PDMK_RING_GGO(64, 5, 2, 4) PDMK_RING_GGO(128, 6, 3, 2) PDMK_RING_GGO(64, 6, 4, 2) PDMK_RING_GGO(128, 5, 2, 4)
        PDMK_RING_GGO(64, 2, 4, 4) PDMK_RING_GGO(128, 2, 3, 4) PDMK_RING_GGO(64, 3, 4, 4)
        default: return 1;
    }
#undef PDMK_RING_GGO
    return hipGetLastError() == hipSuccess ? 0 : -1000;
}

struct WCfg { int bm, nj, stages, occ; };
static const WCfg kWCfgs[] = {{128, 4, 4, 2}, {128, 4, 2, 4}, {64, 4, 3, 4}, {128, 2, 3, 4}, {64, 2, 4, 4}};
constexpr int kNumW = sizeof(kWCfgs) / sizeof(kWCfgs[0]);
int pdmk_wgrad_ring_num_configs() { return kNumW + 2; }
int pdmk_wgrad_ring_name(int id, int conv, char* buf, int n) {
    if (id == kNumW || id == kNumW + 1) {
        snprintf(buf, n, "pdmk_ring::conv_wgrad_halo_kernel<%d, %d>", id == kNumW ? 2 : 4, id == kNumW ? 3 : 2);
        return 0;
    }
    if (id < 0 || id >= kNumW) return -1;
    const WCfg c = kWCfgs[id];
    snprintf(buf, n, "pdmk_ring::wgrad_ring_kernel<%s, %d, %d, %d, %d>", conv ? "true" : "false", c.bm, c.nj, c.stages, c.occ);
    return 0;
}
int pdmk_wgrad_ring_launch(const pdmk_gemm_args& g, hipStream_t st, long a_bytes, long b_bytes, int id) {
    using namespace pdmk_ring;
    if (g.dtype != PDMK_BF16 || g.a_mode != PDMK_A_COLK || g.b_mode == PDMK_B_ROWK || !g.out_f32) return 1;
    const bool conv = g.b_mode == PDMK_B_COLK_CONV;
    if ((g.M % 8) || (g.N % 8) || (g.lda % 8) || (!conv && (g.ldb % 8))) return 1;
    if (conv && ((g.conv_ci % 8) || (g.conv_ld % 8) || g.conv_mode == 3 || g.conv_mode == 4 || g.conv_mode > 8)) return 1;
    if (id == kNumW || id == kNumW + 1) {
        if (!wgrad_halo_ok(g)) return 1;
        const int nblk = (g.K + 127) / 128, sk = g.splitk > 1 ? g.splitk : 1, bm = id == kNumW ? 64 : 128;
        if (sk > nblk) return 1;
        dim3 grid(((g.M + bm - 1) / bm) * ((g.conv_ci + 63) / 64), sk);
        if (bm == 64) hipLaunchKernelGGL((conv_wgrad_halo_kernel<2, 3>), grid, dim3(NT), 0, st, g, (unsigned)a_bytes, (unsigned)b_bytes);
        else hipLaunchKernelGGL((conv_wgrad_halo_kernel<4, 2>), grid, dim3(NT), 0, st, g, (unsigned)a_bytes, (unsigned)b_bytes);
        return hipGetLastError() == hipSuccess ? 0 : -1000;
    }
    if (id < 0 || id >= kNumW) return 1;
    int lg_wo = -1, lg_howo = -1;
    if (conv) {
        auto lg = [](int v) { int l = 0; if (v <= 0 || (v & (v - 1))) return -1; while ((1 << l) < v) ++l; return l; };
        lg_wo = lg(g.conv_wo);
        lg_howo = lg(g.conv_ho * g.conv_wo);
        if (lg_wo < 0 || lg_howo < 0) lg_wo = lg_howo = -1;
    }
    const WCfg c = kWCfgs[id];
    const int bn = 32 * c.nj;
    dim3 grid(((g.M + c.bm - 1) / c.bm) * ((g.N + bn - 1) / bn), g.splitk > 1 ? g.splitk : 1);
// ... 67 lines not shown
```

### unlearn-ft_amd/pdm/_pdmk.py

```python
import ctypes as C
import os

import torch

_HERE = os.path.dirname(os.path.abspath(__file__))
LIB_PATH = os.environ.get("PDMK_LIB") or os.path.join(os.path.dirname(_HERE), "libpdmk.so")

F32, BF16 = 0, 1
EPI_NONE, EPI_GEGLU, EPI_GEGLU_BWD = 0, 1, 2
A_ROWK, A_CONV, A_COLK = 0, 1, 2
B_ROWK, B_COLK, B_COLK_CONV = 0, 1, 2


class PdmkError(RuntimeError):
    pass


def _load():
    if not os.path.exists(LIB_PATH):
        raise PdmkError(f"libpdmk.so not found at {LIB_PATH}: build it with `python __graft_entry__.py` "
                        f"(or `make -C unlearn-ft_amd/csrc`); there is no CPU/PyTorch fallback for the hot path")
    return C.CDLL(LIB_PATH)


_lib = _load()

vp, i32, i64, f32, f64 = C.c_void_p, C.c_int32, C.c_int64, C.c_float, C.c_double


class GemmArgs(C.Structure):
    _fields_ = [("A", vp), ("B", vp), ("C", vp), ("bias", vp), ("rowvec", vp), ("R", vp), ("colsum_out", vp),
                ("M", i32), ("N", i32), ("K", i32),
                ("lda", i32), ("ldb", i32), ("ldc", i32), ("ldr", i32),
                ("rows_per_b", i32), ("a_mode", i32), ("b_mode", i32),
                ("conv_b", i32), ("conv_hi", i32), ("conv_wi", i32), ("conv_ci", i32), ("conv_ho", i32),
                ("conv_wo", i32), ("conv_mode", i32), ("conv_ld", i32),
                ("dtype", i32), ("out_f32", i32), ("accumulate", i32), ("splitk", i32), ("alpha", f32), ("ldrv", i32),
                ("epilogue", i32), ("ldc2", i32), ("C2", vp), ("colstat", vp), ("cs_ld", i32), ("cs_col0", i32),
                ("ln_gamma", vp), ("ln_beta", vp), ("ln_stats", vp), ("ln_out", vp), ("ld_ln_out", i32), ("ln_eps", f32)]


class PlmsRow(C.Structure):
    _fields_ = [("t", i64), ("mode", i32), ("nterms", i32), ("wslot", i32), ("rslot", i32 * 3), ("coef", f32 * 4),
                ("v_x", f32), ("v_v", f32), ("eps_scale", f32), ("x_scale", f32), ("vpred", i32), ("pad_", i32)]


_SIGS = {
    "pdmk_version": ([], i32),
    "pdmk_gemm": ([C.POINTER(GemmArgs), vp], i32),
    "pdmk_gemm_group": ([C.POINTER(GemmArgs), i32, vp, C.POINTER(i32)], i32),
    "pdmk_gemm_plan": ([C.POINTER(GemmArgs), vp, C.POINTER(i32)], i32),
    "pdmk_gemm_ln_supported": ([C.POINTER(GemmArgs)], i32),
    "pdmk_conv_up2_supported": ([i32, i32, i32, i32, i32, i32], i32),
    "pdmk_up2_pack_weights": ([vp, vp, vp, i32, i32, i32, vp], i32),
    "pdmk_up2_combine_wgrad": ([vp, vp, i32, i32, vp], i32),
    "pdmk_gemm_last_candidate": ([], i32),
    "pdmk_gemm_candidate_name": ([i32, i32, i32, C.c_char_p, i32], i32),
    "pdmk_splitk_finish": ([vp, vp, vp, vp, vp, i64, i32, i32, i32, i32, i32, i32, i32, i32, vp], i32),
    "pdmk_splitk_finish_colstat": ([vp, vp, vp, vp, vp, i64, i32, i32, i32, i32, i32, i32, i32, vp, i32, i32, i32, vp], i32),
    "pdmk_groupnorm_fwd": ([vp, vp, vp, vp, vp, vp, i32, i32, i32, i32, i32, i32, i32, f32, i32, i32, vp], i32),
    "pdmk_groupnorm_apply_colstat": ([vp, vp, vp, vp, vp, vp, i32, i32, i32, i32, i32, i32, i32, i32, i32, f32, i32, i32, vp], i32),
    "pdmk_groupnorm_bwd": ([vp, vp, vp, vp, vp, vp, vp, vp, vp, vp, i64, i32, i32, i32, i32, i32, i32, i32, i32, i32, i32, vp, i32, i32, vp], i32),
    "pdmk_groupnorm_bwd_partial_dims": ([i32, i32, i32, i32, i32, i32, C.POINTER(i32), C.POINTER(i32)], i32),
    "pdmk_layernorm_bwd_partial_dims": ([i32, i32, C.POINTER(i32), C.POINTER(i32)], i32),
    "pdmk_reduce_partials_group": ([vp, i32, vp], i32),
    "pdmk_splitk_finish_group": ([vp, i32, vp], i32),
    "pdmk_layernorm_fwd": ([vp, vp, vp, vp, vp, i32, i32, i32, i32, f32, i32, vp], i32),
    "pdmk_layernorm_bwd": ([vp, vp, vp, vp, vp, vp, vp, vp, i64, i32, i32, i32, i32, i32, i32, vp, i32, i32, vp], i32),
    "pdmk_attn_fwd": ([vp, vp, vp, vp, vp, i32, i32, i32, i32, i64, i32, i64, i32, i64, i32, i64, i32, f32, i32, vp], i32),
    "pdmk_attn_bwd": ([vp, vp, vp, vp, vp, vp, vp, vp, vp, vp, i32, i32, i32, i32,
                       i64, i32, i64, i32, i64, i32, i64, i32, i64, i32, i64, i32, i64, i32, f32, vp, i64, i32, vp], i32),
    "pdmk_geglu_fwd": ([vp, vp, i32, i32, i32, i32, i32, i32, vp], i32),
    "pdmk_geglu_bwd": ([vp, vp, vp, i32, i32, i32, i32, i32, i32, i32, vp], i32),
    "pdmk_quantize_e4m3": ([vp, vp, i64, i32, vp], i32),
    "pdmk_silu_fwd": ([vp, vp, i64, i32, vp], i32),
    "pdmk_silu_bwd": ([vp, vp, vp, i64, i32, vp], i32),
    "pdmk_copy2d": ([vp, vp, i64, i32, i32, i32, i32, i32, vp], i32),
    "pdmk_cast_permute": ([vp, vp, i32, i32, i32, i32, i32, vp], i32),
    "pdmk_colsum": ([vp, vp, i64, i32, i32, i32, i32, i32, i32, vp], i32),
    "pdmk_pool2x2_sum": ([vp, vp, i32, i32, i32, i32, i32, vp], i32),
    "pdmk_timestep_embed": ([vp, vp, vp, i32, i32, i32, vp], i32),
    "pdmk_add_noise_velocity": ([vp, vp, vp, vp, vp, vp, vp, i32, i32, i32, i32, i32, vp], i32),
    "pdmk_nchw_to_nhwc": ([vp, vp, i32, i32, i32, i32, i32, vp], i32),
    "pdmk_nhwc_to_nchw": ([vp, vp, i32, i32, i32, i32, i32, vp], i32),
    "pdmk_mse_fwd": ([vp, i32, vp, i32, vp, vp, i32, i32, i64, i32, i32, i32, f64, vp], i32),
    "pdmk_mse_bwd": ([vp, i32, vp, i32, vp, vp, i32, i64, i32, i32, i32, i32, f32, i32, vp], i32),
    "pdmk_mse_fwd_bwd": ([vp, i32, vp, i32, vp, vp, i32, vp, i32, i64, i32, i32, i32, i32, f64, f32, i32, vp], i32),
    "pdmk_axpby": ([vp, vp, f32, f32, i64, i32, vp], i32),
    "pdmk_adamw": ([vp, vp, vp, vp, i64, vp, f32, f32, f32, f32, vp, f32, i32, vp, vp], i32),
    "pdmk_transpose_tiles": ([vp, vp, vp, i32, i32, vp], i32),
    "pdmk_sumsq": ([vp, i64, vp, i32, vp], i32),
    "pdmk_zero": ([vp, i64, vp], i32),
    "pdmk_skinny_gemm": ([vp, i32, vp, vp, vp, i32, i32, i32, i32, i32, i32, i32, i32, i32, vp], i32),
    "pdmk_skinny_wgrad": ([vp, i32, vp, vp, vp, i32, i32, i32, i32, i32, i32, i32, vp], i32),
    "pdmk_softmax_rows": ([vp, vp, i64, i32, i64, i64, i32, vp], i32),
    "pdmk_latent_sample": ([vp, i32, vp, vp, i32, i32, i32, f32, i32, vp], i32),
    "pdmk_embed_tokens": ([vp, vp, vp, vp, i64, i32, i32, i32, i32, i32, i32, i32, vp], i32),
    "pdmk_attn_fwd_causal": ([vp, vp, vp, vp, vp, i32, i32, i32, i64, i32, i64, i32, i64, i32, i64, i32, f32, i32, vp], i32),
    "pdmk_gelu_fwd": ([vp, vp, i64, i32, vp], i32),
    "pdmk_image_prep": ([vp, i64, vp, vp, i32, i32, vp, vp], i32),
    "pdmk_image_prep_ex": ([vp, i64, vp, vp, i32, i32, i32, vp, vp, vp, vp], i32),
    "pdmk_patch_im2col": ([vp, vp, i32, i32, i32, i32, i32, vp], i32),
    "pdmk_vit_tokens": ([vp, i32, vp, vp, i32, vp, i32, i32, i32, i32, i32, vp], i32),
    "pdmk_quick_gelu_fwd": ([vp, vp, i64, i32, vp], i32),
    "pdmk_gather_rows": ([vp, i32, vp, i32, vp, i32, i32, i32, i32, vp], i32),
    "pdmk_clip_score_head": ([vp, i32, vp, i32, vp, vp, vp, i32, i32, vp], i32),
    "pdmk_plms_step": ([vp, i32, f32, f32, i32, vp, vp, vp, vp, i32, vp, vp, vp, i32, i32, i32, i32, i32, vp], i32),
    "pdmk_image_to_u8": ([vp, vp, i32, i32, i32, vp], i32),
    "pdmk_resize_bilinear_u8": ([vp, i64, vp, vp, i32, i32, vp, vp], i32),
    "pdmk_image_resize_u8": ([vp, i64, vp, vp, i32, i32, i32, vp, vp], i32),
    "pdmk_conv2d_fwd": ([vp, i32, vp, vp, vp, i32, i32, i32, i32, i32, i32, i32, i32, i32, i32, i32, i32, vp], i32),
    "pdmk_pool2d": ([vp, i32, vp, i32, i32, i32, i32, i32, i32, i32, i32, vp], i32),
    "pdmk_global_avgpool": ([vp, i32, vp, i32, i32, i32, vp], i32),
    "pdmk_fid_accumulate": ([vp, i32, i32, i32, vp, vp, vp], i32),
    "pdmk_gemm_splitk_workspace_bytes": ([i64, i32, i32], i64),
    "pdmk_groupnorm_workspace_bytes": ([i32, i32], i64),
    "pdmk_groupnorm_bwd_part_workspace_bytes": ([i32, i32], i64),
    "pdmk_layernorm_bwd_part_workspace_bytes": ([i32, i32], i64),
    "pdmk_attn_bwd_workspace_bytes": ([i32, i32, i32, i32], i64),
    "pdmk_plan_export": ([C.c_char_p], i32),
    "pdmk_plan_import": ([C.c_char_p], i32),
    "pdmk_plan_size": ([], i32),
    "pdmk_plan_clear": ([], i32),
    "pdmk_debug_scratch_violations": ([], i32),
    "pdmk_comm_unique_id": ([vp], i32),
    "pdmk_comm_create": ([vp, i32, i32, C.POINTER(vp)], i32),
    "pdmk_comm_allreduce_sum_f32": ([vp, vp, i64, vp], i32),
    "pdmk_comm_world": ([vp], i32),
    "pdmk_comm_rank": ([vp], i32),
    "pdmk_comm_reduce_scatter_sum_f32": ([vp, vp, i64, vp], i32),
    "pdmk_comm_allgather_f32": ([vp, vp, i64, vp], i32),
    "pdmk_stream_create": ([i32, C.POINTER(vp)], i32),
    "pdmk_stream_destroy": ([vp], i32),
    "pdmk_comm_destroy": ([vp], i32),
}
for _n, (_a, _r) in _SIGS.items():
    _f = getattr(_lib, _n)
    _f.argtypes, _f.restype = _a, _r

EXPORTS = tuple(_SIGS)


def version():
    return _lib.pdmk_version()


def dt(t):
    if t.dtype == torch.float32:
        return F32
    if t.dtype == torch.bfloat16:
        return BF16
    raise PdmkError(f"unsupported dtype {t.dtype}")


def _p(t):
    return None if t is None else t.data_ptr()


def _st():
    return torch.cuda.current_stream().cuda_stream


def _chk(rc, name):
    if rc != 0:
        raise PdmkError(f"{name} failed with status {rc}")


PROFILE = None
# ... 20 lines not shown
        global RECORD
        self.prev, self.recs = RECORD, []
        RECORD = self.recs
        return self

    def __exit__(self, *exc):
        global RECORD
        RECORD = self.prev
        return False


def _recordable(kind):
    def deco(fn):
        def wrapped(*a, **kw):
            if RECORD is not None:
                RECORD.append(Rec(kind, lambda: fn(*a, **kw)))
                return None
            return fn(*a, **kw)
        wrapped.__name__, wrapped.__doc__ = fn.__name__, fn.__doc__
        return wrapped
    return deco


def _launch_gemm(g, macs, shape):
    if PROFILE is None:
        _chk(_lib.pdmk_gemm(C.byref(g), _st()), "pdmk_gemm")
        return
    e0, e1 = torch.cuda.Event(enable_timing=True), torch.cuda.Event(enable_timing=True)
    e0.record()
    _chk(_lib.pdmk_gemm(C.byref(g), _st()), "pdmk_gemm")
    e1.record()
    kind = ("bf16" if g.dtype == BF16 else "f32", g.a_mode, g.b_mode, _lib.pdmk_gemm_last_candidate())
    PROFILE.append((kind, 2.0 * (macs if macs is not None else g.M * g.N * g.K), e0, e1, shape))


def gemm_group(recs):
    n = len(recs)
    arr = (GemmArgs * n)()
    for i, r in enumerate(recs):
        arr[i] = r.g
    got = i32(0)
    prof = PROFILE is not None
    if prof:
        e0, e1 = torch.cuda.Event(enable_timing=True), torch.cuda.Event(enable_timing=True)
        e0.record()
    _chk(_lib.pdmk_gemm_group(arr, n, _st(), C.byref(got)), "pdmk_gemm_group")
    STATS["launches"] += 1 if got.value == n else n
    STATS["grouped"] += got.value
    if prof:
        e1.record()
        g0 = recs[0].g
        kind = ("bf16" if g0.dtype == BF16 else "f32", g0.a_mode, g0.b_mode, _lib.pdmk_gemm_last_candidate(), int(got.value))
        flops = sum(2.0 * (r.macs if r.macs is not None else r.g.M * r.g.N * r.g.K) for r in recs)
        PROFILE.append((kind, flops, e0, e1, [(r.g.M, r.g.N, r.g.K, int(r.g.splitk), int(bool(r.g.R) or r.g.accumulate == 1))
                                               for r in recs]))
    return int(got.value)


def run_lockstep(ta, tb, group=True):
    last = {}
    for idx, r in enumerate(ta):
        last[(r.tag, r.kind)] = idx
    i = j = 0
    while i < len(ta) or j < len(tb):
        if i < len(ta) and j < len(tb) and ta[i].tag == tb[j].tag and ta[i].kind == tb[j].kind:
            a, b = ta[i], tb[j]
            i, j = i + 1, j + 1
            if group and a.kind == "gemm":
                gemm_group([a, b])
            elif group and a.kind in _GROUP_FNS:
                _GROUP_FNS[a.kind]([a, b])
                STATS["launches"] += 1
                STATS["grouped"] += 2
            else:
                a.run()
                b.run()
                STATS["launches"] += 2
        elif j < len(tb) and (i >= len(ta) or last.get((tb[j].tag, tb[j].kind), -1) < i):
            tb[j].run()
            j += 1
            STATS["launches"] += 1
        else:
            ta[i].run()
            i += 1
            STATS["launches"] += 1


_GROUP_FNS = {}


def gemm(A, B, Cout, M, N, K, lda, ldb, ldc, *, bias=None, rowvec=None, rows_per_b=0, R=None, ldr=0,
         a_mode=A_ROWK, b_mode=B_ROWK, conv=None, dtype=None, out_f32=False, accumulate=False, splitk=1, alpha=1.0,
         macs=None, colsum_out=None, ldrv=0, epilogue=EPI_NONE, C2=None, ldc2=0, colstat=None, ln=None):
    g = GemmArgs()
    g.colsum_out = _p(colsum_out)
    g.A, g.B, g.C = _p(A), _p(B), _p(Cout)
    g.bias, g.rowvec, g.R = _p(bias), _p(rowvec), _p(R)
    g.M, g.N, g.K = M, N, K
    g.lda, g.ldb, g.ldc, g.ldr = lda, ldb, ldc, ldr
    g.rows_per_b, g.ldrv = rows_per_b, ldrv
    g.a_mode, g.b_mode = a_mode, b_mode
    if conv is not None:
        (g.conv_b, g.conv_hi, g.conv_wi, g.conv_ci, g.conv_ho, g.conv_wo, g.conv_mode, g.conv_ld) = conv
    g.dtype = dt(A) if dtype is None else dtype
    g.out_f32, g.accumulate, g.splitk, g.alpha = int(out_f32), int(accumulate), int(splitk), float(alpha)
    g.epilogue, g.C2, g.ldc2 = int(epilogue), _p(C2), int(ldc2)
    if colstat is not None:
        g.colstat, g.cs_ld, g.cs_col0 = _p(colstat[0]), colstat[0].shape[2], int(colstat[1])
    _set_ln(g, ln)
    shape = (M, N, K, int(splitk), int(R is not None or int(accumulate) == 1))
    if RECORD is not None:
        RECORD.append(Rec("gemm", lambda: _launch_gemm(g, macs, shape), g=g, macs=macs,
                          keep=(A, B, Cout, bias, rowvec, R, colsum_out, C2, colstat, ln)))
        return
    _launch_gemm(g, macs, shape)


def _set_ln(g, ln):
    if ln is None:
        return
    gamma, beta, stats, out, eps = ln
    g.ln_gamma, g.ln_beta, g.ln_stats, g.ln_out = _p(gamma), _p(beta), _p(stats), _p(out)
    g.ld_ln_out, g.ln_eps = (0 if out is None else out.stride(0)), float(eps)


def gemm_ln_supported(A, B, M, N, K, lda, ldb, *, geglu=False, residual=False, bias=False):
    g = GemmArgs()
    g.A, g.B, g.C = _p(A), _p(B), _p(A)
    g.M, g.N, g.K, g.lda, g.ldb, g.ldc = M, N, K, lda, ldb, (N // 2 if geglu else N)
    g.a_mode, g.b_mode, g.dtype, g.splitk, g.alpha = A_ROWK, B_ROWK, dt(A), 1, 1.0
    g.epilogue = EPI_GEGLU if geglu else EPI_NONE
    if residual:
        g.R, g.ldr = _p(A), N
    if bias or geglu:
        g.bias = _p(B)
    g.ln_gamma = g.ln_beta = _p(B)
    g.ln_eps = 1e-5
    return bool(_lib.pdmk_gemm_ln_supported(C.byref(g)))


def _ws_bytes(n):
    if n < 0:
        raise PdmkError("workspace query rejected its arguments")
    return int(n)


def plan_export(path):
    _chk(_lib.pdmk_plan_export(os.fsencode(path)), "pdmk_plan_export")


def plan_import(path):
    n = _lib.pdmk_plan_import(os.fsencode(path))
    if n < 0:
        raise PdmkError(f"pdmk_plan_import({path!r}) failed with status {n}")
    return n


def plan_size():
    return int(_lib.pdmk_plan_size())


def plan_clear():
    _chk(_lib.pdmk_plan_clear(), "pdmk_plan_clear")


def debug_scratch_violations():
# ... 39 lines not shown
            self._h = None


_ROLE_STREAMS = {}


def role_stream(device, role, high_priority=False):
    dev = torch.device(device)
    key = (dev.index if dev.index is not None else torch.cuda.current_device(), role)
    s = _ROLE_STREAMS.get(key)
    if s is None:
        h = vp()
        with torch.cuda.device(key[0]):
            _chk(_lib.pdmk_stream_create(int(high_priority), C.byref(h)), "pdmk_stream_create")
        s = torch.cuda.ExternalStream(h.value, device=torch.device("cuda", key[0]))
        _ROLE_STREAMS[key] = s
    return s


def groupnorm_ws(device, B, G, have=None):
    need = _ws_bytes(_lib.pdmk_groupnorm_workspace_bytes(B, G)) // 8
    if have is not None and have.numel() >= need:
        return have
    return torch.empty(max(need, 1 << 17), device=device, dtype=torch.float64)


def zeros(shape, device, dtype):
    n = 1
    for d in shape:
        n *= d
    esz = torch.empty((), dtype=dtype).element_size()
    pad = (-(n * esz)) % 16 // esz
    flat = torch.empty(n + pad, device=device, dtype=dtype)
    _chk(_lib.pdmk_zero(_p(flat), (n + pad) * esz, _st()), "pdmk_zero")
    return flat[:n].view(*shape)


def zero_(t):
    assert t.is_contiguous() and (t.numel() * t.element_size()) % 16 == 0
    _chk(_lib.pdmk_zero(_p(t), t.numel() * t.element_size(), _st()), "pdmk_zero")
    return t


def last_candidate():
    return int(_lib.pdmk_gemm_last_candidate())


def candidate_name(a_mode, b_mode, cand):
    buf = C.create_string_buffer(160)
    _chk(_lib.pdmk_gemm_candidate_name(a_mode, b_mode, cand, buf, 160), "pdmk_gemm_candidate_name")
    return buf.value.decode()


def splitk_plan(A, B, M, N, K, lda, ldb, a_mode=A_ROWK, conv=None):
    g = GemmArgs()
    g.A, g.B = _p(A), _p(B)
    g.M, g.N, g.K = M, N, K
    g.lda, g.ldb, g.ldc = lda, ldb, N
    g.a_mode, g.b_mode = a_mode, B_ROWK
    if conv is not None:
        (g.conv_b, g.conv_hi, g.conv_wi, g.conv_ci, g.conv_ho, g.conv_wo, g.conv_mode, g.conv_ld) = conv
    g.dtype = dt(A)
    g.splitk, g.alpha = 1, 1.0
    sk = i32(1)
    _chk(_lib.pdmk_gemm_plan(C.byref(g), _st(), C.byref(sk)), "pdmk_gemm_plan")
    return int(sk.value)


def wgrad_plan(dy, x, M, N, K, lda, ldb, b_mode=B_COLK, conv=None, slabs=False):
    g = GemmArgs()
    g.accumulate = 2 if slabs else 0
    g.A, g.B = _p(dy), _p(x)
    g.M, g.N, g.K = M, N, K
    g.lda, g.ldb, g.ldc = lda, ldb, N
    g.a_mode, g.b_mode = A_COLK, b_mode
    if conv is not None:
        (g.conv_b, g.conv_hi, g.conv_wi, g.conv_ci, g.conv_ho, g.conv_wo, g.conv_mode, g.conv_ld) = conv
    g.dtype = dt(x)
    g.out_f32, g.splitk, g.alpha = 1, 1, 1.0
    sk = i32(1)
    _chk(_lib.pdmk_gemm_plan(C.byref(g), _st(), C.byref(sk)), "pdmk_gemm_plan")
    return int(sk.value)


def gemm_auto(A, B, Cout, M, N, K, lda, ldb, ldc, *, bias=None, rowvec=None, rows_per_b=0, R=None, ldr=0,
              a_mode=A_ROWK, conv=None, accumulate=False, macs=None, ldrv=0, colstat=None):
    sk = splitk_plan(A, B, M, N, K, lda, ldb, a_mode, conv)
    if sk == 1:
        gemm(A, B, Cout, M, N, K, lda, ldb, ldc, bias=bias, rowvec=rowvec, rows_per_b=rows_per_b, R=R, ldr=ldr,
             a_mode=a_mode, conv=conv, accumulate=accumulate, macs=macs, ldrv=ldrv, colstat=colstat)
        return colstat is not None
    ws = torch.empty(_ws_bytes(_lib.pdmk_gemm_splitk_workspace_bytes(M, N, sk)) // 4, device=A.device, dtype=torch.float32)
    gemm(A, B, ws, M, N, K, lda, ldb, N, a_mode=a_mode, conv=conv, out_f32=True, splitk=sk, accumulate=2, macs=macs)
    splitk_finish(ws, Cout, M, N, ldc, sk, bias=bias, rowvec=rowvec, R=R, ldr=ldr, rows_per_b=rows_per_b, ldrv=ldrv,
                  accumulate=accumulate, colstat=colstat)
    return colstat is not None


@_recordable("splitk_finish")
def splitk_finish(ws, Cout, M, N, ldc, nslab, *, bias=None, rowvec=None, R=None, ldr=0, rows_per_b=0, ldrv=0,
                  accumulate=False, colstat=None):
    if colstat is not None:
        _chk(_lib.pdmk_splitk_finish_colstat(_p(ws), _p(Cout), _p(bias), _p(rowvec), _p(R), M, N, ldc, ldr, rows_per_b, ldrv,
                                             nslab, int(accumulate), _p(colstat[0]), colstat[0].shape[2], int(colstat[1]),
                                             dt(Cout), _st()), "pdmk_splitk_finish_colstat")
        return
    _chk(_lib.pdmk_splitk_finish(_p(ws), _p(Cout), _p(bias), _p(rowvec), _p(R), M, N, ldc, ldr, rows_per_b, ldrv, nslab,
                                 int(accumulate), dt(Cout), _st()), "pdmk_splitk_finish")


class SlabItem(C.Structure):
    _fields_ = [("ws", vp), ("dst", vp), ("n", i64), ("nslab", i32), ("pad_", i32)]


SLAB_GROUP_MAX = 32


class SlabQueue:

    def __init__(self, max_bytes=1 << 30):
        self.items, self.bytes, self.max_bytes = [], 0, max_bytes

    def add(self, ws, dW, n, nslab):
        self.items.append((ws, dW, n, nslab))
        self.bytes += ws.numel() * 4

    def full(self):
        return len(self.items) >= SLAB_GROUP_MAX or self.bytes >= self.max_bytes

    def flush(self):
        while self.items:
            chunk, self.items = self.items[:SLAB_GROUP_MAX], self.items[SLAB_GROUP_MAX:]
            arr = (SlabItem * len(chunk))()
            for a, (ws, dW, n, nslab) in zip(arr, chunk):
                a.ws, a.dst, a.n, a.nslab = _p(ws), _p(dW), n, nslab
            _chk(_lib.pdmk_splitk_finish_group(C.cast(arr, vp), len(chunk), _st()), "pdmk_splitk_finish_group")
        self.bytes = 0


def wgrad(dy, x, dW, M, N, K, lda, ldb, *, b_mode=B_COLK, conv=None, colsum_out=None, macs=None, queue=None):
    if queue is not None and (M * N) % 4 == 0 and dW.is_contiguous():
        sk = wgrad_plan(dy, x, M, N, K, lda, ldb, b_mode, conv, slabs=True)
        if sk > 1:
            if queue.full():
                queue.flush()
            ws = torch.empty(sk * M * N, device=dy.device, dtype=torch.float32)
            gemm(dy, x, ws, M, N, K, lda, ldb, N, a_mode=A_COLK, b_mode=b_mode, conv=conv, out_f32=True, splitk=sk,
                 accumulate=2, dtype=dt(x), macs=macs, colsum_out=colsum_out)
            queue.add(ws, dW, M * N, sk)
# ... 497 lines not shown
```

### unlearn-ft_amd/pdm/models/unet/engine.py

```python
import math
import os

import torch

from ... import _pdmk as k
from .params import ParamStore, kv_layout, temb_layout
from .spec import UNetConfig, padc


class Act:
    __slots__ = ("t", "_g", "rg", "pend", "src", "cs", "parked")

    def __init__(self, t, rg=True):
        self.t, self._g, self.rg, self.pend = t, None, rg, None
        self.parked = False
        self.cs = None
        self.src = None

    def flush(self):
        if self.pend is not None:
            p_, self.pend = self.pend, None
            if self._g is None:
                self._g = p_
                return
            k.copy2d(p_, self._g, p_.shape[0], p_.shape[1], p_.stride(0), self._g.stride(0), accumulate=True)

    @property
    def g(self):
        self.flush()
        return self._g

    @g.setter
    def g(self, v):
        assert self.pend is None
        self._g = v


def _ld(t):
    return t.stride(0)


class UNetEngine:
    def __init__(self, cfg: UNetConfig, blocks, store: ParamStore, dtype):
        self.cfg, self.blocks, self.P, self.dtype = cfg, blocks, store, dtype
        self.dev = store.master.device
        half = cfg.block_out_channels[0] // 2
        self.freqs = torch.exp(-math.log(10000.0) * torch.arange(half, dtype=torch.float32) / half).to(self.dev)
        self.ws = k.groupnorm_ws(self.dev, 64, cfg.norm_num_groups)
        self.tape = []
        self.train = False
        self.macs = 0
        self.count_macs = False
        self.grad_ready_cb = None
        self.temb_lay, self.temb_cols = temb_layout(cfg, blocks)
        self.kv_lay, self.kv_cols = kv_layout(blocks)
        ups = [r for b in blocks if b.kind == "up" for r in b.resnets]
        self.cat_ch = [None if r.dropped else padc(r.cin - r.skip) for r in reversed(ups)]
        self.wgrad_async = os.environ.get("PDMK_WGRAD_ASYNC", "0") == "1"
        self.wgrad_stream = None
        self.fuse_geglu = os.environ.get("PDMK_FUSE_GEGLU", "1") != "0"
        self.fuse_ln = int(os.environ.get("PDMK_FUSE_LN", "1"))
        self.attn_fp8 = False
        self.fuse_geglu_bwd = os.environ.get("PDMK_FUSE_GEGLU_BWD", "1") != "0"
        self.defer_fanin = os.environ.get("PDMK_DEFER_FANIN", "1") != "0"
        self._keep = []
        self.partials = k.PartialQueue() if os.environ.get("PDMK_DEFER_PARTIALS", "1") != "0" else None
        self.slabs = k.SlabQueue() if os.environ.get("PDMK_WGRAD_SLABS", "1") != "0" else None
        self.conv_slabs = os.environ.get("PDMK_WGRAD_SLABS_CONV", "0") == "1"
        self.up2 = os.environ.get("PDMK_CONV_UP2", "1") != "0"
        self.gn_epi = os.environ.get("PDMK_GN_EPI", "1") != "0" and dtype == torch.bfloat16
        self.group_wgrad = os.environ.get("PDMK_WGRAD_GROUP", "1") != "0" and dtype == torch.bfloat16 and self.slabs is not None
        self.group_conv_wgrad = self.group_wgrad and os.environ.get("PDMK_WGRAD_GROUP_CONV", "0") == "1"
        self._wg_items = None
        self._cs_arena, self._cs_off, self._cs_need, self._cs_old = None, 0, 0, []
        self._cs_views, self._cs_cats = {}, {}

    def _empty(self, rows, cols, dtype=None):
        return torch.empty((rows, cols), device=self.dev, dtype=dtype or self.dtype)

    def _grad_into(self, act, rows, cols, absorb=False):
        add = None
        if absorb:
            add, act.pend = act.pend, None
        elif act._g is None and act.pend is not None:
            p_, act.pend = act.pend, None
            act.g = self._empty(rows, cols, act.t.dtype)
            k.copy2d(p_, act._g, rows, cols, _ld(p_), _ld(act._g))
            return act._g, True
        if act._g is None:
            act.g = self._empty(rows, cols, act.t.dtype)
            return (act._g, False, add) if absorb else (act._g, False)
        act.flush()
        return (act._g, True, add) if absorb else (act._g, True)

    def _give(self, act, dy, park=False):
        if not act.rg:
            return
        if act._g is None and act.pend is not None:
            p_, act.pend = act.pend, None
            act.g = self._empty(p_.shape[0], p_.shape[1], act.t.dtype)
            k.copy2d(p_, act._g, p_.shape[0], p_.shape[1], _ld(p_), _ld(act._g))
        if act._g is None and park:
            act.pend = dy
            act.parked = True
        elif act._g is None:
            act.g = dy
        elif self.defer_fanin and dy.dtype == act._g.dtype:
            act.flush()
            act.pend = dy
        else:
            k.copy2d(dy, act._g, dy.shape[0], dy.shape[1], _ld(dy), _ld(act._g), accumulate=True)

    def _wgrad(self, fn, *operands):
        if not self.wgrad_async or torch.cuda.is_current_stream_capturing():
            fn()
            return
        main = torch.cuda.current_stream()
        if self.wgrad_stream is None:
            self.wgrad_stream = k.role_stream(self.dev, "wgrad")
        self.wgrad_stream.wait_stream(main)
        with torch.cuda.stream(self.wgrad_stream):
            fn()
        self._keep.extend(operands)

    def _join_wgrad(self):
        if self.wgrad_async and self._keep and self.wgrad_stream is not None:
            torch.cuda.current_stream().wait_stream(self.wgrad_stream)
            self._keep.clear()
# ... 477 lines not shown
            self.tape.append(self._wg_flush)
        n1 = self.groupnorm(x, p + ".norm1", B, H * W, G, r.cin // G, 1e-5, True)
        h1, _, _ = self.conv3(n1, p + ".conv1", B, H, W, 0, p + ".conv1.bias", rowvec=st, rv_cols=self.temb_lay[p][:2], cs=True)
        n2 = self.groupnorm(h1, p + ".norm2", B, H * W, r.groups2(G), r.cout // G, 1e-5, True)
        res = x if r.cin == r.cout else self.linear(x, p + ".conv_shortcut", bias=p + ".conv_shortcut.bias")
        y, _, _ = self.conv3(n2, p + ".conv2", B, H, W, 0, p + ".conv2.bias", residual=res, out=out, cs=cs)
        if self.train and self.group_conv_wgrad:
            self.tape.append(self._wg_open)
        return y

    def transformer(self, x, a, ehs, B, H, W, T, out=None, cs=True):
        G = self.cfg.norm_num_groups
        p, c, N = a.name, a.c, H * W
        t = p + ".transformer_blocks.0"
        d1, d2 = a.h1() * 64, a.h2() * 64
        self._mark(p + ".norm.weight")
        if self.train and self.group_wgrad:
            self.tape.append(self._wg_flush)
        n = self.groupnorm(x, p + ".norm", B, N, G, c // G, 1e-6, False)
        h = self.linear(n, p + ".proj_in", bias=p + ".proj_in.bias")
        qkv = self.linear(h, t + ".attn1.to_qkv", ln=t + ".norm1")
        if self.attn_fp8:
            k.quantize_e4m3_(qkv.t)
        o = self.attention(qkv.t[:, :d1], qkv.t[:, d1:2 * d1], qkv.t[:, 2 * d1:3 * d1], B, a.h1(), N, N, qkv, qkv,
                           (0, d1), ((d1, 2 * d1), (2 * d1, 3 * d1)), tag=t + ".attn1")
        h = self.linear(o, t + ".attn1.to_out.0", bias=t + ".attn1.to_out.0.bias", residual=h)
        q = self.linear(h, t + ".attn2.to_q", ln=t + ".norm2")
        if self.attn_fp8:
            k.quantize_e4m3_(q.t)
        kv, ko = ehs, self.kv_lay[p][0]
        o = self.attention(q.t[:, :d2], kv.t[:, ko:ko + d2], kv.t[:, ko + d2:ko + 2 * d2], B, a.h2(), N, T, q, kv, (0, d2),
                           ((ko, ko + d2), (ko + d2, ko + 2 * d2)), tag=t + ".attn2")
        h = self.linear(o, t + ".attn2.to_out.0", bias=t + ".attn2.to_out.0.bias", residual=h)
        gl = self.linear(h, t + ".ff.net.0.proj", bias=t + ".ff.net.0.proj.bias", geglu=True, ln=t + ".norm3")
        h = self.linear(gl, t + ".ff.net.2", bias=t + ".ff.net.2.bias", residual=h)
        y = self.linear(h, p + ".proj_out", bias=p + ".proj_out.bias", residual=x, out=out, cs=(B, N) if cs else None)
        if self.train and self.group_wgrad:
            self.tape.append(self._wg_open)
        return y

    def _wg_open(self):
        self._wg_items = []

    def _wg_flush(self):
        items, self._wg_items = self._wg_items, None
        if items:
            k.wgrad_group(items, self.slabs)

    def forward(self, x, timesteps, ehs, B, H, W, train):
        cfg = self.cfg
        self.train = train
        self.tape = []
        self._cs_begin()
        T = ehs.shape[0] // B
        c0 = cfg.block_out_channels[0]
        k.TAG = "time_embedding"
        te = self._empty(B, c0)
        k.timestep_embed(timesteps, self.freqs, te, B, c0)
        e1 = self.linear(Act(te, rg=False), "time_embedding.linear_1", bias="time_embedding.linear_1.bias")
        temb = self.linear(self.silu(e1), "time_embedding.linear_2", bias="time_embedding.linear_2.bias")
        st = self.silu(temb)
        if self.temb_cols:
            st = self.linear(st, "time_emb_proj_all", bias="time_emb_proj_all.bias", out_f32=True)
        ehs_act = Act(ehs, rg=False)
        if self.kv_cols:
            ehs_act = self.linear(ehs_act, "attn2_kv_all")
            ehs_act.rg = train
            if self.attn_fp8:
                k.quantize_e4m3_(ehs_act.t)
        c0p = padc(c0)
        nskip = 0

        def push(act, cat):
            nonlocal nskip
            skips.append((act, cat))
            nskip += 1

        skips = []
        cat, view = self._skip_view(nskip, B * H * W, c0p, B)
        h, _, _ = self.conv3(Act(x, rg=False), "conv_in", B, H, W, 0, "conv_in.bias", out=view, cs=True)
        push(h, cat)
        acts = {}
        for b in self.blocks:
            cb = padc(b.c)
            if b.kind == "down":
                for j, r in enumerate(b.resnets):
                    att = b.attns[j] if (b.attns and not b.attns[j].dropped) else None
                    cat, view = self._skip_view(nskip, B * H * W, cb, B)
                    made = False
                    if not r.dropped:
                        h = self.resblock(h, r, st, B, H, W, out=None if att is not None else view)
                        made = att is None
                    if att is not None:
                        h = self.transformer(h, att, ehs_act, B, H, W, T, out=view)
                        made = True
                    push(h, cat if made else None)
                if b.sampler:
                    cat, view = self._skip_view(nskip, B * ((H + 1) // 2) * ((W + 1) // 2), cb, B)
                    h, H, W = self.conv3(h, f"{b.name}.downsamplers.0.conv", B, H, W, 1,
                                         f"{b.name}.downsamplers.0.conv.bias", out=view, cs=True)
                    push(h, cat)
                acts[f"d{b.idx}"] = h
            elif b.kind == "mid":
                h = self.resblock(h, b.resnets[0], st, B, H, W)
                h = self.transformer(h, b.attns[0], ehs_act, B, H, W, T)
                h = self.resblock(h, b.resnets[1], st, B, H, W, out=self._left_view(skips, B * H * W, cb))
                acts["m"] = h
            else:
                n = len(b.resnets)
                for j, r in enumerate(b.resnets):
                    s, scat = skips.pop()
                    att = b.attns[j] if (b.attns and not b.attns[j].dropped) else None
                    nxt = None if (j == n - 1 and b.sampler) else self._left_view(skips, B * H * W, cb)
                    last = j == n - 1 and b.sampler
                    if not r.dropped:
                        h = self.resblock(self.concat(h, s, scat), r, st, B, H, W, out=None if att is not None else nxt,
                                          cs=att is not None or not last)
                    if att is not None:
                        h = self.transformer(h, att, ehs_act, B, H, W, T, out=nxt, cs=not last)
                if b.sampler:
                    h, H, W = self.conv3(h, f"{b.name}.upsamplers.0.conv", B, H, W, 2,
                                         f"{b.name}.upsamplers.0.conv.bias",
                                         out=self._left_view(skips, B * 4 * H * W, cb), cs=True)
                acts[f"u{b.idx}"] = h
        assert not skips
        n = self.groupnorm(h, "conv_norm_out", B, H * W, cfg.norm_num_groups, c0 // cfg.norm_num_groups, 1e-5, True)
        pred, _, _ = self.conv3(n, "conv_out", B, H, W, 0, "conv_out.bias")
        return pred, acts

    def backward(self):
        tape, self.tape = self.tape, []
        for fn in reversed(tape):
            fn()
        self._join_wgrad()
        self.flush_pending()
```

Measured before the change: 189.9 images/s.

## Fuse split-K reduction into GEMM launch via per-tile arrival counters

Adds an in-launch split-K form in which the last-arriving workgroup for each output tile sums the fp32 slabs and applies the normal bf16 epilogue (bias, residual, rowvec). This replaces the separate splitk_finish kernel and one extra read-back pass. The planner now tunes both the two-pass and the in-launch forms per shape and records the chosen form in the plan file. The change needs per-tile counters and cross-workgroup ordering through sc1 stores, which brings synchronisation and correctness risk and a possible tail on the reducing workgroup.

```diff
diff --git a/include/pdmk.h b/include/pdmk.h
--- a/include/pdmk.h
+++ b/include/pdmk.h
@@ -50,6 +50,8 @@
     void* ln_out;
     int32_t ld_ln_out;
     float ln_eps;
+    float* sk_ws;
+    int32_t* sk_cnt;
 } pdmk_gemm_args;
 int pdmk_gemm_ln_supported(const pdmk_gemm_args* args);
 
@@ -85,6 +87,8 @@
 } pdmk_slab_item;
 int pdmk_splitk_finish_group(const pdmk_slab_item* items, int n_items, pdmk_stream stream);
 int64_t pdmk_gemm_splitk_workspace_bytes(int64_t M, int N, int splitk);
+int64_t pdmk_gemm_splitk_counters(int64_t M, int N);
+int pdmk_gemm_plan_form(const pdmk_gemm_args* args, pdmk_stream stream, int32_t* splitk_out, int32_t* form_out);
 
 int pdmk_plan_export(const char* path);
 int pdmk_plan_import(const char* path);
diff --git a/unlearn-ft_amd/csrc/abi_util.hip b/unlearn-ft_amd/csrc/abi_util.hip
--- a/unlearn-ft_amd/csrc/abi_util.hip
+++ b/unlearn-ft_amd/csrc/abi_util.hip
@@ -3,6 +3,11 @@
 extern "C" int64_t pdmk_gemm_splitk_workspace_bytes(int64_t M, int N, int splitk) {
     if (M <= 0 || N <= 0) return -1;
     return (int64_t)(splitk > 1 ? splitk : 1) * M * N * 4;
+}
+
+extern "C" int64_t pdmk_gemm_splitk_counters(int64_t M, int N) {
+    if (M <= 0 || N <= 0) return -1;
+    return ((M + 63) / 64) * (((int64_t)N + 63) / 64);
 }
 
 extern "C" int64_t pdmk_groupnorm_workspace_bytes(int B, int G) {
diff --git a/unlearn-ft_amd/csrc/gemm.hip b/unlearn-ft_amd/csrc/gemm.hip
--- a/unlearn-ft_amd/csrc/gemm.hip
+++ b/unlearn-ft_amd/csrc/gemm.hip
@@ -522,7 +522,7 @@
 PlanKey make_key(const pdmk_gemm_args& g, int sk) {
     PlanKey k;
     const bool cv = g.a_mode == PDMK_A_CONV || g.b_mode == PDMK_B_COLK_CONV;
-    const int slabw = (g.a_mode == PDMK_A_COLK && g.accumulate == 2) ? 1000 : 0;
+    const int slabw = (g.a_mode == PDMK_A_COLK && g.accumulate == 2) ? 1000 : (g.accumulate >= 3 ? 2000 : 0);
     const int v[10] = {g.M, g.N, g.K, g.a_mode, g.b_mode, (cv ? g.conv_mode : 100 * g.epilogue) + slabw, cv ? g.conv_hi : 0,
                        cv ? g.conv_wi : 0, cv ? g.conv_ci : 0, sk};
     memcpy(k.v, v, sizeof v);
@@ -550,7 +550,7 @@
 }
 
 int launch_legacy(const pdmk_gemm_args& g, hipStream_t st) {
-    if (g.colstat) return -2;
+    if (g.colstat || g.accumulate >= 3) return -2;
     if ((g.a_mode == PDMK_A_CONV || g.b_mode == PDMK_B_COLK_CONV) && g.conv_mode >= 5) return -2;
     const long nblocks = (long)((g.M + 127) / 128) * ((g.N + 127) / 128) * (g.splitk > 1 ? g.splitk : 1);
     long ab, bb;
@@ -631,7 +631,7 @@
 float time_candidate(const pdmk_gemm_args& a, hipStream_t st, int id, float* ws, void* fin_out, hipEvent_t e0, hipEvent_t e1) {
     static const int reps = getenv("PDMK_TUNE_REPS") ? std::max(1, atoi(getenv("PDMK_TUNE_REPS"))) : 3;
     auto once = [&]() -> int {
-        if (a.splitk > 1 && a.a_mode != PDMK_A_COLK) {
+        if (a.splitk > 1 && a.a_mode != PDMK_A_COLK && a.accumulate < 3) {
             const int rc = launch_candidate(a, st, id);
             if (rc) return rc;
             return pdmk_splitk_finish(ws, fin_out, nullptr, nullptr, nullptr, a.M, a.N, a.N, 0, 1, 0, a.splitk, 0, a.dtype,
@@ -656,9 +656,11 @@
     return us;
 }
 
-int tune_cfg(const pdmk_gemm_args& g, hipStream_t st, int sk, float* t_out) {
+int tune_cfg(const pdmk_gemm_args& g, hipStream_t st, int sk, float* t_out, bool inl = false) {
     const size_t out_bytes = (size_t)out_rows(g) * g.N * 4;
-    if (!ensure_scratch((size_t)(sk > 1 ? sk : 1) * out_bytes + out_bytes + (size_t)g.M * 4 + 256)) return -1;
+    const size_t cnt_bytes = inl ? (size_t)pdmk_gemm_splitk_counters(g.M, g.N) * 4 : 0;
+    const size_t cnt_off = ((size_t)(sk > 1 ? sk : 1) * out_bytes + out_bytes + (size_t)g.M * 4 + 255) & ~(size_t)255;
+    if (!ensure_scratch(cnt_off + cnt_bytes + 256)) return -1;
     (void)hipDeviceSynchronize();
     hipEvent_t e0, e1;
     if (hipEventCreate(&e0) != hipSuccess || hipEventCreate(&e1) != hipSuccess) { (void)hipGetLastError(); return -1; }
@@ -677,20 +679,25 @@
         a.C = ws;
         if (g.accumulate == 2 && sk > 1) a.accumulate = 2;
     }
+    else if (sk > 1 && inl) {
+        a.C = out2; a.accumulate = 3; a.sk_ws = ws; a.bias = nullptr; a.rowvec = nullptr; a.R = nullptr;
+        a.sk_cnt = reinterpret_cast<int32_t*>(reinterpret_cast<char*>(g_scratch) + cnt_off);
+    }
     else if (sk > 1) { a.C = ws; a.out_f32 = 1; a.accumulate = 2; a.bias = nullptr; a.rowvec = nullptr; a.R = nullptr; }
     else a.C = out2;
     int best = -1;
     float bt = 1e30f;
     const int ncand = 1 + (g.a_mode == PDMK_A_COLK ? pdmk_wgrad_ring_num_configs() : pdmk_gemm_ring_num_configs());
-    for (int id = g.epilogue ? 1 : 0; id < ncand; ++id) {
+    for (int id = (g.epilogue || inl) ? 1 : 0; id < ncand; ++id) {
+        if (inl && hipMemsetAsync(a.sk_cnt, 0, cnt_bytes, st) != hipSuccess) { (void)hipGetLastError(); break; }
         const float t = time_candidate(a, st, id, ws, out2, e0, e1);
         if (t < bt) { bt = t; best = id; }
     }
     (void)hipEventDestroy(e0);
     (void)hipEventDestroy(e1);
     if (getenv("PDMK_TUNE_LOG"))
-        fprintf(stderr, "[pdmk tune] M=%d N=%d K=%d amode=%d cmode=%d sk=%d -> cand %d (%.1f us)\n", g.M, g.N, g.K, g.a_mode,
-                g.conv_mode, sk, best, bt);
+        fprintf(stderr, "[pdmk tune] M=%d N=%d K=%d amode=%d cmode=%d sk=%d%s -> cand %d (%.1f us)\n", g.M, g.N, g.K, g.a_mode,
+                g.conv_mode, sk, inl ? " in-launch" : "", best, bt);
     if (!scratch_check()) return -1;
     *t_out = bt;
     return best;
@@ -758,9 +765,16 @@
         const int ew = half ? (g.conv_wi + 1) / 2 : (twice ? 2 * g.conv_wi : g.conv_wi);
         if (g.conv_ho != eh || g.conv_wo != ew) return -1;
     }
-    if (g.splitk > 1 && !(g.out_f32 || g.dtype == PDMK_F32)) return -1;
+    if (g.splitk > 1 && g.accumulate < 3 && !(g.out_f32 || g.dtype == PDMK_F32)) return -1;
     if (g.accumulate == 2 && (g.splitk <= 1 || !(g.out_f32 || g.dtype == PDMK_F32) || g.bias || g.rowvec || g.R)) return -1;
-    if (g.accumulate < 0 || g.accumulate > 2) return -1;
+    if (g.accumulate < 0 || g.accumulate > 4) return -1;
+    if (g.accumulate >= 3) {
+        if (g.splitk <= 1 || !g.sk_ws || !g.sk_cnt || (((uintptr_t)g.sk_ws | (uintptr_t)g.C) & 15) || ((uintptr_t)g.sk_cnt & 3)) return -1;
+        if ((g.N % 8) || (g.ldc % 8) || (g.R && (g.ldr % 8))) return -1;
+        if (g.dtype != PDMK_BF16 || g.out_f32 || g.a_mode == PDMK_A_COLK || g.b_mode != PDMK_B_ROWK || g.epilogue || g.colstat ||
+            g.ln_gamma || (g.K % 8) || (g.a_mode == PDMK_A_CONV && g.conv_mode >= 5) || !ring_mode())
+            return -2;
+    }
     if (g.rowvec && g.rows_per_b <= 0) return -1;
     if (g.epilogue != PDMK_EPI_NONE) {
         if (g.epilogue != PDMK_EPI_GEGLU && g.epilogue != PDMK_EPI_GEGLU_BWD) return -2;
@@ -821,7 +835,7 @@
     if ((g.a_mode == PDMK_A_COLK ? forced_wcfg() >= 0 : forced_cfg() >= 0) && !(g.epilogue && forced_cfg() == 0)) {
         const int rc = launch_candidate(g, st, g.a_mode == PDMK_A_COLK ? forced_wcfg() : forced_cfg());
         g_last_candidate = rc == 1 ? 0 : (g.a_mode == PDMK_A_COLK ? forced_wcfg() : forced_cfg());
-        if (g.epilogue && rc == 1) return -2;
+        if ((g.epilogue || g.accumulate >= 3) && rc == 1) return -2;
         const bool phase = (g.a_mode == PDMK_A_CONV || g.b_mode == PDMK_B_COLK_CONV) && g.conv_mode >= 5;
         if (!((phase || g.colstat) && rc == 1)) return rc == 1 ? launch_legacy(g, st) : rc;
     }
@@ -835,19 +849,23 @@
         if (it != g_plan_cfg.end()) id = it->second;
         else if (can_tune(st)) {
             float t;
-            id = tune_cfg(g, st, sk, &t);
+            id = tune_cfg(g, st, sk, &t, g.accumulate >= 3);
             if (id < 0) id = heuristic_cfg(g);
             g_plan_cfg[key] = id;
             plan_file_append('c', key, id);
         } else id = heuristic_cfg(g);
     }
-    if ((g.epilogue || g.colstat) && id <= 0) id = 1 + pdmk_gemm_ring_pick(g);
+    if ((g.epilogue || g.colstat || g.accumulate >= 3) && id <= 0) id = 1 + pdmk_gemm_ring_pick(g);
     int rc = launch_candidate(g, st, id);
     if (g.colstat && rc == 1) {
         id = 1 + pdmk_gemm_ring_pick(g);
         rc = launch_candidate(g, st, id);
     }
-    if (g.epilogue && rc == 1) return -2;
+    if (g.accumulate >= 3 && rc == 1) {
+        id = 1 + pdmk_gemm_ring_pick(g);
+        rc = launch_candidate(g, st, id);
+    }
+    if ((g.epilogue || g.accumulate >= 3) && rc == 1) return -2;
     g_last_candidate = rc == 1 ? 0 : id;
     return rc == 1 ? launch_legacy(g, st) : rc;
 }
@@ -870,7 +888,7 @@
     if (it != g_plan_cfg.end()) return it->second;
     if (!can_tune(st)) return heuristic_cfg(g);
     float t;
-    int id = tune_cfg(g, st, sk, &t);
+    int id = tune_cfg(g, st, sk, &t, g.accumulate >= 3);
     if (id < 0) id = heuristic_cfg(g);
     g_plan_cfg[key] = id;
     plan_file_append('c', key, id);
@@ -925,6 +943,7 @@
         if (t[i].epilogue == PDMK_EPI_GEGLU_BWD) t[i].ldc = 2 * a[i].N;
         else t[i].C2 = nullptr;
         if (t[i].accumulate == 1) t[i].accumulate = 0;
+        if (t[i].accumulate == 4) t[i].accumulate = 3;
         if (t[i].epilogue == PDMK_EPI_GEGLU) t[i].ldc = a[i].N / 2;
         if (t[i].colsum_out)
             t[i].colsum_out = reinterpret_cast<float*>(base + (off[i + 1] - off[i]) - (((size_t)a[i].M * 4 + 15) & ~(size_t)15));
@@ -1005,7 +1024,7 @@
     std::vector<int> key;
     for (int i = 0; i < n; ++i) {
         ids[i] = member_plan(a[i], st);
-        if ((a[i].epilogue || a[i].colstat) && ids[i] <= 0) ids[i] = 1 + pdmk_gemm_ring_pick(a[i]);
+        if ((a[i].epilogue || a[i].colstat || a[i].accumulate >= 3) && ids[i] <= 0) ids[i] = 1 + pdmk_gemm_ring_pick(a[i]);
         const PlanKey k = make_key(a[i], a[i].splitk > 1 ? a[i].splitk : 1);
         key.insert(key.end(), k.v, k.v + 10);
         key.push_back(a[i].accumulate);
@@ -1052,8 +1071,15 @@
     return pdmk_gemm_ring_name(id - 1, a_mode == PDMK_A_CONV, buf, n);
 }
 
+static int inlaunch_mode() { static int c = INT32_MIN; return env_int("PDMK_SPLITK_INLAUNCH", 1, &c); }
+constexpr int kFormInl = 1000;
 extern "C" int pdmk_gemm_plan(const pdmk_gemm_args* a, pdmk_stream stream, int32_t* splitk_out) {
-    if (!a || !splitk_out) return -1;
+    int32_t form = 0;
+    return pdmk_gemm_plan_form(a, stream, splitk_out, &form);
+}
+extern "C" int pdmk_gemm_plan_form(const pdmk_gemm_args* a, pdmk_stream stream, int32_t* splitk_out, int32_t* form_out) {
+    if (!a || !splitk_out || !form_out) return -1;
+    *form_out = 0;
     const pdmk_gemm_args& g = *a;
     hipStream_t st = reinterpret_cast<hipStream_t>(stream);
     *splitk_out = 1;
@@ -1072,13 +1098,19 @@
     plan_file_load();
     const PlanKey key0 = make_key(g, 0);
     auto it = g_plan_sk.find(key0);
-    if (it != g_plan_sk.end()) { *splitk_out = it->second; return 0; }
+    if (it != g_plan_sk.end()) {
+        *splitk_out = it->second % kFormInl;
+        *form_out = (it->second >= kFormInl && inlaunch_mode()) ? 1 : 0;
+        return 0;
+    }
     if (!can_tune(st) || !a->A || !a->B) { *splitk_out = wg ? heuristic_wgrad_sk(g) : heuristic_sk(g); return 0; }
     const int tiles = ((g.M + 127) / 128) * ((g.N + 127) / 128);
     const int nk = (g.K + 63) / 64;
     const int cands[12] = {1, 2, 3, 4, 6, 8, 12, 16, 24, 32, 48, 64};
-    int best_sk = 1;
+    int best_sk = 1, best_form = 0;
     float bt = 1e30f;
+    const bool inl_ok = !wg && inlaunch_mode() && g.dtype == PDMK_BF16 && (g.N % 8) == 0 && !g.out_f32 &&
+                        !(g.a_mode == PDMK_A_CONV && g.conv_mode >= 5);
     for (int c = 0; c < 12; ++c) {
         const int sk = cands[c];
         if (wg) {
@@ -1091,11 +1123,27 @@
         g_plan_cfg[make_key(g, sk)] = id;
         plan_file_append('c', make_key(g, sk), id);
         static const float margin = getenv("PDMK_SPLIT_MARGIN") ? 1.0f - 0.01f * (float)atof(getenv("PDMK_SPLIT_MARGIN")) : 0.97f;
-        if (t < bt * (sk > 1 ? margin : 1.0f)) { bt = t; best_sk = sk; }
-    }
-    g_plan_sk[key0] = best_sk;
-    plan_file_append('s', key0, best_sk);
+        if (t < bt * (sk > 1 ? margin : 1.0f)) { bt = t; best_sk = sk; best_form = 0; }
+        if (sk > 1 && inl_ok) {
+            pdmk_gemm_args gi = g;
+            gi.accumulate = 3;
+            float ti = 1e30f;
+            const int idi = tune_cfg(gi, st, sk, &ti, true);
+            if (idi > 0) {
+                g_plan_cfg[make_key(gi, sk)] = idi;
+                plan_file_append('c', make_key(gi, sk), idi);
+                static const float imargin = getenv("PDMK_INLAUNCH_MARGIN") ? 1.0f - 0.01f * (float)atof(getenv("PDMK_INLAUNCH_MARGIN")) : 0.99f;
+                if (ti < bt * imargin) { bt = ti; best_sk = sk; best_form = 1; }
+            }
+        }
+    }
+    if (getenv("PDMK_TUNE_LOG"))
+        fprintf(stderr, "[pdmk plan] M=%d N=%d K=%d amode=%d cmode=%d -> sk %d %s (%.1f us)\n", g.M, g.N, g.K, g.a_mode, g.conv_mode,
+                best_sk, best_sk == 1 ? "unsplit" : (best_form ? "in-launch" : "two-pass"), bt);
+    g_plan_sk[key0] = best_sk + (best_form ? kFormInl : 0);
+    plan_file_append('s', key0, best_sk + (best_form ? kFormInl : 0));
     *splitk_out = best_sk;
+    *form_out = best_form;
     return 0;
 }
 
@@ -1155,4 +1203,4 @@
     return g_scratch_violations;
 }
 
-extern "C" int pdmk_version(void) { return 121; }
+extern "C" int pdmk_version(void) { return 122; }
diff --git a/unlearn-ft_amd/csrc/gemm_ring.hip b/unlearn-ft_amd/csrc/gemm_ring.hip
--- a/unlearn-ft_amd/csrc/gemm_ring.hip
+++ b/unlearn-ft_amd/csrc/gemm_ring.hip
@@ -81,9 +81,12 @@
 #define PDMK_PRIO_UP() do { if (PDMK_PRIO == 2) __builtin_amdgcn_s_setprio(1); } while (0)
 #define PDMK_PRIO_DOWN() do { if (PDMK_PRIO == 2) __builtin_amdgcn_s_setprio(0); } while (0)
 
-template <int BM, int NJ, int LDS_BYTES, bool TILE2D = false, bool OUTMAP = false>
-__device__ __forceinline__ void ring_epilogue(const pdmk_gemm_args& g, const LC wgc, f32x4 (&acc)[BM / 64][NJ], unsigned char* smem,
-                                              int m0, int n0, int tw = 0, int img_w = 0) {
+__device__ __forceinline__ void st_sc1(float* p, f32x4 v) {
+    asm volatile("global_store_dwordx4 %0, %1, off sc1\n\ts_nop 1" ::"v"(p), "v"(v) : "memory");
+}
+template <int BM, int NJ, int LDS_BYTES, bool TILE2D, bool OUTMAP, bool FROMSLAB, bool SC1 = false>
+__device__ __forceinline__ void ring_epilogue_passes(const pdmk_gemm_args& g, const LC wgc, f32x4 (&acc)[BM / 64][NJ], unsigned char* smem,
+                                                     int m0, int n0, int tw, int img_w) {
     auto row_of = [&](int l) { return TILE2D ? m0 + (l / tw) * img_w + (l % tw) : m0 + l; };
     auto out_row = [&](int m) -> long {
         if (!OUTMAP) return (long)m;
@@ -96,10 +99,10 @@
     const int wm = wave >> 1, wn = wave & 1;
     const bool first = wgc.by == 0;
     const bool slab = g.accumulate == 2;
-    const bool atomic = wgc.gy > 1 && !slab;
+    const bool atomic = !FROMSLAB && wgc.gy > 1 && !slab;
     const bool acc1 = g.accumulate == 1;
     const bool f32out = g.out_f32 != 0;
-    const bool vec8 = ((g.N & 7) == 0) && ((g.ldc & 7) == 0) && (g.R == nullptr || (g.ldr & 7) == 0);
+    const bool vec8 = FROMSLAB || (((g.N & 7) == 0) && ((g.ldc & 7) == 0) && (g.R == nullptr || (g.ldr & 7) == 0));
     constexpr int SROW = BN + 4;
     constexpr int C8 = BN / 8;
     constexpr int ITEMS = (64 * C8 + NT - 1) / NT;
@@ -115,7 +118,51 @@
 #pragma unroll
     for (int pass = 0; pass < BM / 64; ++pass) {
         __syncthreads();
-        if ((wm * 16 * IM) / 64 == pass) {
+        if constexpr (FROMSLAB) {
+            const float* wsp = reinterpret_cast<const float*>(g.sk_ws);
+            const long sstride = (long)g.M * g.N;
+            long soff[ITEMS];
+            f32x4 s0[ITEMS], s1[ITEMS];
+#pragma unroll
+            for (int it = 0; it < ITEMS; ++it) {
+                const int item = tid + it * NT;
+                const int lr2 = item / C8, c8 = item - lr2 * C8;
+                const int m = row_of(pass * 64 + lr2), n = n0 + c8 * 8;
+                soff[it] = (item < 64 * C8 && m < g.M && n < g.N) ? (long)m * g.N + n : 0L;
+                s0[it] = *reinterpret_cast<const f32x4*>(wsp + soff[it]);
+                s1[it] = *reinterpret_cast<const f32x4*>(wsp + soff[it] + 4);
+            }
+            {
+                f32x4 u0[ITEMS], u1[ITEMS];
+#pragma unroll
+                for (int it = 0; it < ITEMS; ++it) {
+                    u0[it] = *reinterpret_cast<const f32x4*>(wsp + sstride + soff[it]);
+                    u1[it] = *reinterpret_cast<const f32x4*>(wsp + sstride + soff[it] + 4);
+                }
+#pragma unroll
+                for (int it = 0; it < ITEMS; ++it) { s0[it] += u0[it]; s1[it] += u1[it]; }
+            }
+#pragma unroll 1
+            for (unsigned sl = 2; sl < wgc.gy; ++sl) {
+                f32x4 u0[ITEMS], u1[ITEMS];
+#pragma unroll
+                for (int it = 0; it < ITEMS; ++it) {
+                    u0[it] = *reinterpret_cast<const f32x4*>(wsp + sl * sstride + soff[it]);
+                    u1[it] = *reinterpret_cast<const f32x4*>(wsp + sl * sstride + soff[it] + 4);
+                }
+#pragma unroll
+                for (int it = 0; it < ITEMS; ++it) { s0[it] += u0[it]; s1[it] += u1[it]; }
+            }
+#pragma unroll
+            for (int it = 0; it < ITEMS; ++it) {
+                const int item = tid + it * NT;
+                const int lr2 = item / C8, c8 = item - lr2 * C8;
+                if (item < 64 * C8) {
+                    *reinterpret_cast<f32x4*>(stage + lr2 * SROW + c8 * 8) = s0[it];
+                    *reinterpret_cast<f32x4*>(stage + lr2 * SROW + c8 * 8 + 4) = s1[it];
+                }
+            }
+        } else if ((wm * 16 * IM) / 64 == pass) {
             const int lrb = (wm * 16 * IM) % 64;
 #pragma unroll
             for (int i = 0; i < IM; ++i)
@@ -146,7 +193,7 @@
                     }
                 }
             }
-        } else if (vec8 && g.epilogue == PDMK_EPI_GEGLU) {
+        } else if (!FROMSLAB && vec8 && g.epilogue == PDMK_EPI_GEGLU) {
             constexpr int C16 = BN / 16;
             constexpr int ITEMS2 = (64 * C16 + NT - 1) / NT;
             bf16* C2 = reinterpret_cast<bf16*>(g.C2);
@@ -182,7 +229,7 @@
                 for (int r = 0; r < 8; ++r) o[r] = (bf16)((float)hb[r] * gelu_f((float)gb[r]));
                 st_stream(reinterpret_cast<bf16x8*>(Ct + (long)m * g.ldc + (n >> 1)), o);
             }
-        } else if (vec8 && g.epilogue == PDMK_EPI_GEGLU_BWD) {
+        } else if (!FROMSLAB && vec8 && g.epilogue == PDMK_EPI_GEGLU_BWD) {
             const bf16* X2 = reinterpret_cast<const bf16*>(g.C2);
             bf16x8 hb[ITEMS], gb[ITEMS];
 #pragma unroll
@@ -255,7 +302,10 @@
                     for (int r = 0; r < 8; ++r) v[r] += (float)rres[it][r];
                 }
                 const long off = out_row(m) * g.ldc + n;
-                if (f32out) {
+                if (SC1) {
+                    st_sc1(Cf + off, f32x4{v[0], v[1], v[2], v[3]});
+                    st_sc1(Cf + off + 4, f32x4{v[4], v[5], v[6], v[7]});
+                } else if (f32out) {
                     float4 o0 = make_float4(v[0], v[1], v[2], v[3]), o1 = make_float4(v[4], v[5], v[6], v[7]);
                     if (acc1) {
                         const float4 c0 = *reinterpret_cast<const float4*>(Cf + off), c1 = *reinterpret_cast<const float4*>(Cf + off + 4);
@@ -331,9 +381,50 @@
     }
 }
 
+template <int BM, int NJ, int LDS_BYTES, bool TILE2D = false, bool OUTMAP = false, bool INL = true>
+__device__ __forceinline__ void ring_epilogue(const pdmk_gemm_args& g, const LC wgc, f32x4 (&acc)[BM / 64][NJ], unsigned char* smem,
+                                              int m0, int n0, int tw = 0, int img_w = 0) {
+    if constexpr (INL && !OUTMAP) {
+        if (wgc.gy > 1 && g.accumulate >= 3) {
+            pdmk_gemm_args gs = g;
+            gs.C = g.sk_ws;
+            gs.ldc = g.N;
+            gs.out_f32 = 1;
+            gs.accumulate = 2;
+            gs.epilogue = PDMK_EPI_NONE;
+            gs.bias = nullptr;
+            gs.rowvec = nullptr;
+            gs.R = nullptr;
+            gs.colstat = nullptr;
+            ring_epilogue_passes<BM, NJ, LDS_BYTES, TILE2D, false, false, true>(gs, wgc, acc, smem, m0, n0, tw, img_w);
+            asm volatile("s_waitcnt vmcnt(0)" ::: "memory");
+            __syncthreads();
+            volatile int* flag = reinterpret_cast<volatile int*>(smem);
+            if (threadIdx.x == 0) {
+                int* cnt = g.sk_cnt + wgc.bx;
+                const int ticket = __hip_atomic_fetch_add(cnt, 1, __ATOMIC_RELAXED, __HIP_MEMORY_SCOPE_AGENT);
+                const int last = ticket == (int)wgc.gy - 1 ? 1 : 0;
+                if (last) {
+                    __builtin_amdgcn_fence(__ATOMIC_ACQUIRE, "agent");
+                    asm volatile("s_waitcnt vmcnt(0)" ::: "memory");
+                    __hip_atomic_store(cnt, 0, __ATOMIC_RELAXED, __HIP_MEMORY_SCOPE_AGENT);
+                }
+                *flag = last;
+            }
+            __syncthreads();
+            if (__builtin_amdgcn_readfirstlane(*flag) == 0) return;
+            pdmk_gemm_args gf = g;
+            gf.accumulate = g.accumulate - 3;
+            ring_epilogue_passes<BM, NJ, LDS_BYTES, TILE2D, false, true>(gf, wgc, acc, smem, m0, n0, tw, img_w);
+            return;
+        }
+    }
+    ring_epilogue_passes<BM, NJ, LDS_BYTES, TILE2D, OUTMAP, false>(g, wgc, acc, smem, m0, n0, tw, img_w);
+}
+
 constexpr int ring_smem_bytes(int BM, int NJ, int STAGES) { return STAGES * (BM * 128 + 32 * NJ * 128); }
 
-template <bool CONV, int BM, int NJ, int STAGES, int OCC>
+template <bool CONV, int BM, int NJ, int STAGES, int OCC, bool INL = false>
 __device__ __forceinline__ void igemm_ring_body(const pdmk_gemm_args& g, unsigned a_bytes, unsigned b_bytes, const LC wgc,
                                                 unsigned char* smem) {
     typedef Mma<bf16> MM;
@@ -356,7 +447,7 @@
     const int per = (nk_total + wgc.gy - 1) / wgc.gy;
     const int kt0 = wgc.by * per;
     const int kt1 = min(nk_total, kt0 + per);
-    if (kt0 >= kt1 && g.accumulate != 2) return;
+    if (kt0 >= kt1 && g.accumulate < 2) return;
 
     const auto rsrcA = __builtin_amdgcn_make_buffer_rsrc(const_cast<void*>(g.A), (short)0, (int)a_bytes, 0x00020000);
     const auto rsrcB = __builtin_amdgcn_make_buffer_rsrc(const_cast<void*>(g.B), (short)0, (int)b_bytes, 0x00020000);
@@ -481,26 +572,26 @@
     }
 
     if (PDMK_PRIO == 1) __builtin_amdgcn_s_setprio(0);
-    ring_epilogue<BM, NJ, STAGES * SLOT>(g, wgc, acc, smem, m0, n0);
-}
-
-template <bool CONV, int BM, int NJ, int STAGES, int OCC>
+    ring_epilogue<BM, NJ, STAGES * SLOT, false, false, INL>(g, wgc, acc, smem, m0, n0);
+}
+
+template <bool CONV, int BM, int NJ, int STAGES, int OCC, bool INL = false>
 __global__ __launch_bounds__(NT, OCC) void igemm_ring_kernel(pdmk_gemm_args g, unsigned a_bytes, unsigned b_bytes) {
     __shared__ __attribute__((aligned(1024))) unsigned char smem[ring_smem_bytes(BM, NJ, STAGES)];
-    igemm_ring_body<CONV, BM, NJ, STAGES, OCC>(g, a_bytes, b_bytes, lc_plain(), smem);
-}
-template <bool CONV, int BM, int NJ, int STAGES, int OCC>
+    igemm_ring_body<CONV, BM, NJ, STAGES, OCC, INL>(g, a_bytes, b_bytes, lc_plain(), smem);
+}
+template <bool CONV, int BM, int NJ, int STAGES, int OCC, bool INL = false>
 __global__ __launch_bounds__(NT, OCC) void igemm_ring_group_kernel(pdmk_gemm_group_dev gg) {
     __shared__ __attribute__((aligned(1024))) unsigned char smem[ring_smem_bytes(BM, NJ, STAGES)];
     int pi;
     LC wgc;
     if (!lc_group(gg, pi, wgc)) return;
-    igemm_ring_body<CONV, BM, NJ, STAGES, OCC>(gg.p[pi], gg.a_bytes[pi], gg.b_bytes[pi], wgc, smem);
+    igemm_ring_body<CONV, BM, NJ, STAGES, OCC, INL>(gg.p[pi], gg.a_bytes[pi], gg.b_bytes[pi], wgc, smem);
 }
 
 constexpr int halo_smem_bytes(int NJ, int BSTAGES, int PMAX) { return 2 * PMAX * 128 + BSTAGES * 32 * NJ * 128; }
 
-template <int BM, int NJ, int BSTAGES, int PMAX, int NTAPS = 9>
+template <int BM, int NJ, int BSTAGES, int PMAX, int NTAPS = 9, bool INL = false>
 __device__ __forceinline__ void conv_halo_body(const pdmk_gemm_args& g, unsigned a_bytes, unsigned b_bytes, int tw, const LC wgc,
                                                unsigned char* smem) {
     typedef Mma<bf16> MM;
@@ -532,7 +623,7 @@
     const int ncb_total = (NTAPS == 4 && g.conv_mode == 13) ? 4 * ncb1 : ncb1;
     const int per = (ncb_total + wgc.gy - 1) / wgc.gy;
     const int cb0 = wgc.by * per, cb1 = min(ncb_total, cb0 + per);
-    if (cb0 >= cb1 && g.accumulate != 2) return;
+    if (cb0 >= cb1 && g.accumulate < 2) return;
 
     const int rimg = HW >= BM ? BM / tw : H;
     const int W2 = tw + 2, pimg = (rimg + 2) * W2;
@@ -766,26 +857,26 @@
     if (PDMK_PRIO == 1) __builtin_amdgcn_s_setprio(0);
     __builtin_amdgcn_s_barrier();
     if (NTAPS == 4 && !dgr) {
-        if (tw == W) ring_epilogue<BM, NJ, 2 * P_BYTES + BSTAGES * B_BYTES, false, NTAPS == 4>(g, wgc, acc, smem, m0, n0);
-        else ring_epilogue<BM, NJ, 2 * P_BYTES + BSTAGES * B_BYTES, true, NTAPS == 4>(g, wgc, acc, smem, mbase, n0, tw, W);
+        if (tw == W) ring_epilogue<BM, NJ, 2 * P_BYTES + BSTAGES * B_BYTES, false, NTAPS == 4, false>(g, wgc, acc, smem, m0, n0);
+        else ring_epilogue<BM, NJ, 2 * P_BYTES + BSTAGES * B_BYTES, true, NTAPS == 4, false>(g, wgc, acc, smem, mbase, n0, tw, W);
         return;
     }
-    if (tw == W) ring_epilogue<BM, NJ, 2 * P_BYTES + BSTAGES * B_BYTES>(g, wgc, acc, smem, m0, n0);
-    else ring_epilogue<BM, NJ, 2 * P_BYTES + BSTAGES * B_BYTES, true>(g, wgc, acc, smem, mbase, n0, tw, W);
-}
-
-template <int BM, int NJ, int BSTAGES, int PMAX, int NTAPS = 9>
+    if (tw == W) ring_epilogue<BM, NJ, 2 * P_BYTES + BSTAGES * B_BYTES, false, false, INL>(g, wgc, acc, smem, m0, n0);
+    else ring_epilogue<BM, NJ, 2 * P_BYTES + BSTAGES * B_BYTES, true, false, INL>(g, wgc, acc, smem, mbase, n0, tw, W);
+}
+
+template <int BM, int NJ, int BSTAGES, int PMAX, int NTAPS = 9, bool INL = false>
 __global__ __launch_bounds__(NT, 2) void conv_halo_kernel(pdmk_gemm_args g, unsigned a_bytes, unsigned b_bytes, int tw) {
     __shared__ __attribute__((aligned(1024))) unsigned char smem[halo_smem_bytes(NJ, BSTAGES, PMAX)];
-    conv_halo_body<BM, NJ, BSTAGES, PMAX, NTAPS>(g, a_bytes, b_bytes, tw, lc_plain(), smem);
-}
-template <int BM, int NJ, int BSTAGES, int PMAX, int NTAPS = 9>
+    conv_halo_body<BM, NJ, BSTAGES, PMAX, NTAPS, INL>(g, a_bytes, b_bytes, tw, lc_plain(), smem);
+}
+template <int BM, int NJ, int BSTAGES, int PMAX, int NTAPS = 9, bool INL = false>
 __global__ __launch_bounds__(NT, 2) void conv_halo_group_kernel(pdmk_gemm_group_dev gg) {
     __shared__ __attribute__((aligned(1024))) unsigned char smem[halo_smem_bytes(NJ, BSTAGES, PMAX)];
     int pi;
     LC wgc;
     if (!lc_group(gg, pi, wgc)) return;
-    conv_halo_body<BM, NJ, BSTAGES, PMAX, NTAPS>(gg.p[pi], gg.a_bytes[pi], gg.b_bytes[pi], gg.aux0[pi], wgc, smem);
+    conv_halo_body<BM, NJ, BSTAGES, PMAX, NTAPS, INL>(gg.p[pi], gg.a_bytes[pi], gg.b_bytes[pi], gg.aux0[pi], wgc, smem);
 }
 
 constexpr int wgrad_smem_bytes(int BM, int NJ, int STAGES) { return STAGES * (64 * BM * 2 + 64 * 32 * NJ * 2); }
@@ -814,7 +905,7 @@
     const int per = (nk_total + wgc.gy - 1) / wgc.gy;
     const int kt0 = wgc.by * per;
     const int kt1 = min(nk_total, kt0 + per);
-    if (kt0 >= kt1 && g.accumulate != 2) return;
+    if (kt0 >= kt1 && g.accumulate < 2) return;
 
     const auto rsrcA = __builtin_amdgcn_make_buffer_rsrc(const_cast<void*>(g.A), (short)0, (int)a_bytes, 0x00020000);
     const auto rsrcB = __builtin_amdgcn_make_buffer_rsrc(const_cast<void*>(g.B), (short)0, (int)b_bytes, 0x00020000);
@@ -946,7 +1037,7 @@
             if (m < g.M) unsafeAtomicAdd(g.colsum_out + m, acs[i][0]);
         }
     }
-    ring_epilogue<BM, NJ, STAGES * SLOT>(g, wgc, acc, smem, m0, n0);
+    ring_epilogue<BM, NJ, STAGES * SLOT, false, false, false>(g, wgc, acc, smem, m0, n0);
 }
 
 template <bool CONV, int BM, int NJ, int STAGES, int OCC>
@@ -1035,6 +1126,16 @@
         else hipLaunchKernelGGL((conv_halo_kernel<128, 4, 5, 264, 4>), grid, dim3(NT), 0, st, g, (unsigned)a_bytes, (unsigned)b_bytes, tw);
         return hipGetLastError() == hipSuccess ? 0 : -1000;
     }
+    if (g.accumulate >= 3) {
+        switch (id) {
+            case 0: hipLaunchKernelGGL((conv_halo_kernel<256, 5, 3, 400, 9, true>), grid, dim3(NT), 0, st, g, (unsigned)a_bytes, (unsigned)b_bytes, tw); break;
+            case 1: hipLaunchKernelGGL((conv_halo_kernel<256, 4, 3, 400, 9, true>), grid, dim3(NT), 0, st, g, (unsigned)a_bytes, (unsigned)b_bytes, tw); break;
+            case 2: hipLaunchKernelGGL((conv_halo_kernel<128, 5, 4, 264, 9, true>), grid, dim3(NT), 0, st, g, (unsigned)a_bytes, (unsigned)b_bytes, tw); break;
+            case 3: hipLaunchKernelGGL((conv_halo_kernel<128, 4, 5, 264, 9, true>), grid, dim3(NT), 0, st, g, (unsigned)a_bytes, (unsigned)b_bytes, tw); break;
+            default: return 1;
+        }
+        return hipGetLastError() == hipSuccess ? 0 : -1000;
+    }
     switch (id) {
         case 0: hipLaunchKernelGGL((conv_halo_kernel<256, 5, 3, 400>), grid, dim3(NT), 0, st, g, (unsigned)a_bytes, (unsigned)b_bytes, tw); break;
         case 1: hipLaunchKernelGGL((conv_halo_kernel<256, 4, 3, 400>), grid, dim3(NT), 0, st, g, (unsigned)a_bytes, (unsigned)b_bytes, tw); break;
@@ -1074,12 +1175,12 @@
     if (id < 0) return -1;
     if (id >= kNumBase && id < kNumBase + kNumHalo) {
         const int h = id - kNumBase;
-        snprintf(buf, n, "pdmk_ring::conv_halo_kernel<%d, %d, %d, %d, 9>", h < 2 ? 256 : 128, (h & 1) ? 4 : 5,
+        snprintf(buf, n, "pdmk_ring::conv_halo_kernel<%d, %d, %d, %d, 9, false>", h < 2 ? 256 : 128, (h & 1) ? 4 : 5,
                  h < 2 ? 3 : ((h & 1) ? 5 : 4), h < 2 ? 400 : 264);
         return 0;
     }
     const Config c = kConfigs[id < kNumBase ? id : id - kNumHalo];
-    snprintf(buf, n, "pdmk_ring::igemm_ring_kernel<%s, %d, %d, %d, %d>", conv ? "true" : "false", c.bm, c.nj, c.stages, c.occ);
+    snprintf(buf, n, "pdmk_ring::igemm_ring_kernel<%s, %d, %d, %d, %d, false>", conv ? "true" : "false", c.bm, c.nj, c.stages, c.occ);
     return 0;
 }
 int pdmk_gemm_ring_pick(const pdmk_gemm_args& g) { return pdmk_ring::pick_config(g, g.splitk); }
@@ -1089,6 +1190,7 @@
     if (g.dtype != PDMK_BF16 || g.b_mode != PDMK_B_ROWK || g.a_mode == PDMK_A_COLK) return 1;
     if ((g.K % 8) || (g.a_mode == PDMK_A_CONV && (g.conv_ci % 8))) return 1;
     if (g.ln_gamma && id < kNumConfigs + kNumHalo) return 1;
+    if (g.accumulate >= 3 && id >= kNumConfigs + kNumHalo) return 1;
     if (id >= kNumBase && id < kNumBase + kNumHalo) return conv_halo_launch(g, st, a_bytes, b_bytes, id - kNumBase);
     if (g.a_mode == PDMK_A_CONV && g.conv_mode >= 5) return 1;
     if (id >= kNumConfigs + kNumHalo) return pdmk_gemm_rowblock_launch(g, st, a_bytes, b_bytes, id - (kNumConfigs + kNumHalo));
@@ -1097,11 +1199,15 @@
     const Config c = kConfigs[id < kNumBase ? id : id - kNumHalo];
     const int bn = 32 * c.nj;
     dim3 grid(((g.M + c.bm - 1) / c.bm) * ((g.N + bn - 1) / bn), sk);
-    const bool conv = g.a_mode == PDMK_A_CONV;
+    const bool conv = g.a_mode == PDMK_A_CONV, inl = g.accumulate >= 3;
 #define PDMK_RING_GO(BMv, NJv, STv, OCv)                                                                              \
     case (BMv * 1000 + NJv * 100 + STv * 10 + OCv):                                                                   \
-        if (conv) hipLaunchKernelGGL((igemm_ring_kernel<true, BMv, NJv, STv, OCv>), grid, dim3(NT), 0, st, g,         \
-                                     (unsigned)a_bytes, (unsigned)b_bytes);                                           \
+        if (inl && conv) hipLaunchKernelGGL((igemm_ring_kernel<true, BMv, NJv, STv, OCv, true>), grid, dim3(NT), 0, st, g, \
+                                            (unsigned)a_bytes, (unsigned)b_bytes);                                    \
+        else if (inl) hipLaunchKernelGGL((igemm_ring_kernel<false, BMv, NJv, STv, OCv, true>), grid, dim3(NT), 0, st, g, \
+                                         (unsigned)a_bytes, (unsigned)b_bytes);                                       \
+        else if (conv) hipLaunchKernelGGL((igemm_ring_kernel<true, BMv, NJv, STv, OCv>), grid, dim3(NT), 0, st, g,    \
+                                          (unsigned)a_bytes, (unsigned)b_bytes);                                      \
         else hipLaunchKernelGGL((igemm_ring_kernel<false, BMv, NJv, STv, OCv>), grid, dim3(NT), 0, st, g,             \
                                 (unsigned)a_bytes, (unsigned)b_bytes);                                                \
         break;
@@ -1369,8 +1475,10 @@
     if (id >= kNumConfigs + kNumHalo) return 1;
     const bool conv = gs[0].a_mode == PDMK_A_CONV;
     GroupGrid G;
+    bool inl = false;
     for (int i = 0; i < n; ++i) {
         const pdmk_gemm_args& g = gs[i];
+        inl = inl || g.accumulate >= 3;
         if (g.dtype != PDMK_BF16 || g.b_mode != PDMK_B_ROWK || g.a_mode == PDMK_A_COLK) return 1;
         if ((g.K % 8) || (g.a_mode == PDMK_A_CONV && (g.conv_ci % 8))) return 1;
         if ((g.a_mode == PDMK_A_CONV) != conv) return 1;
@@ -1399,6 +1507,15 @@
             else hipLaunchKernelGGL((conv_halo_group_kernel<128, 4, 5, 264, 4>), grid, dim3(NT), 0, st, G.gg);
             return hipGetLastError() == hipSuccess ? 0 : -1000;
         }
+        if (inl) {
+            switch (id - kNumBase) {
+                case 0: hipLaunchKernelGGL((conv_halo_group_kernel<256, 5, 3, 400, 9, true>), grid, dim3(NT), 0, st, G.gg); break;
+                case 1: hipLaunchKernelGGL((conv_halo_group_kernel<256, 4, 3, 400, 9, true>), grid, dim3(NT), 0, st, G.gg); break;
+                case 2: hipLaunchKernelGGL((conv_halo_group_kernel<128, 5, 4, 264, 9, true>), grid, dim3(NT), 0, st, G.gg); break;
+                default: hipLaunchKernelGGL((conv_halo_group_kernel<128, 4, 5, 264, 9, true>), grid, dim3(NT), 0, st, G.gg); break;
+            }
+            return hipGetLastError() == hipSuccess ? 0 : -1000;
+        }
         switch (id - kNumBase) {
             case 0: hipLaunchKernelGGL((conv_halo_group_kernel<256, 5, 3, 400>), grid, dim3(NT), 0, st, G.gg); break;
             case 1: hipLaunchKernelGGL((conv_halo_group_kernel<256, 4, 3, 400>), grid, dim3(NT), 0, st, G.gg); break;
@@ -1410,7 +1527,9 @@
     const Config c = kConfigs[id < kNumBase ? id : id - kNumHalo];
 #define PDMK_RING_GGO(BMv, NJv, STv, OCv)                                                                             \
     case (BMv * 1000 + NJv * 100 + STv * 10 + OCv):                                                                   \
-        if (conv) hipLaunchKernelGGL((igemm_ring_group_kernel<true, BMv, NJv, STv, OCv>), grid, dim3(NT), 0, st, G.gg); \
+        if (inl && conv) hipLaunchKernelGGL((igemm_ring_group_kernel<true, BMv, NJv, STv, OCv, true>), grid, dim3(NT), 0, st, G.gg); \
+        else if (inl) hipLaunchKernelGGL((igemm_ring_group_kernel<false, BMv, NJv, STv, OCv, true>), grid, dim3(NT), 0, st, G.gg); \
+        else if (conv) hipLaunchKernelGGL((igemm_ring_group_kernel<true, BMv, NJv, STv, OCv>), grid, dim3(NT), 0, st, G.gg); \
         else hipLaunchKernelGGL((igemm_ring_group_kernel<false, BMv, NJv, STv, OCv>), grid, dim3(NT), 0, st, G.gg);   \
         break;
     switch (c.bm * 1000 + c.nj * 100 + c.stages * 10 + c.occ) {
diff --git a/unlearn-ft_amd/pdm/_pdmk.py b/unlearn-ft_amd/pdm/_pdmk.py
--- a/unlearn-ft_amd/pdm/_pdmk.py
+++ b/unlearn-ft_amd/pdm/_pdmk.py
@@ -37,7 +37,8 @@
                 ("conv_wo", i32), ("conv_mode", i32), ("conv_ld", i32),
                 ("dtype", i32), ("out_f32", i32), ("accumulate", i32), ("splitk", i32), ("alpha", f32), ("ldrv", i32),
                 ("epilogue", i32), ("ldc2", i32), ("C2", vp), ("colstat", vp), ("cs_ld", i32), ("cs_col0", i32),
-                ("ln_gamma", vp), ("ln_beta", vp), ("ln_stats", vp), ("ln_out", vp), ("ld_ln_out", i32), ("ln_eps", f32)]
+                ("ln_gamma", vp), ("ln_beta", vp), ("ln_stats", vp), ("ln_out", vp), ("ld_ln_out", i32), ("ln_eps", f32),
+                ("sk_ws", vp), ("sk_cnt", vp)]
 
 
 class PlmsRow(C.Structure):
@@ -50,6 +51,7 @@
     "pdmk_gemm": ([C.POINTER(GemmArgs), vp], i32),
     "pdmk_gemm_group": ([C.POINTER(GemmArgs), i32, vp, C.POINTER(i32)], i32),
     "pdmk_gemm_plan": ([C.POINTER(GemmArgs), vp, C.POINTER(i32)], i32),
+    "pdmk_gemm_plan_form": ([C.POINTER(GemmArgs), vp, C.POINTER(i32), C.POINTER(i32)], i32),
     "pdmk_gemm_ln_supported": ([C.POINTER(GemmArgs)], i32),
     "pdmk_conv_up2_supported": ([i32, i32, i32, i32, i32, i32], i32),
     "pdmk_up2_pack_weights": ([vp, vp, vp, i32, i32, i32, vp], i32),
@@ -114,6 +116,7 @@
     "pdmk_global_avgpool": ([vp, i32, vp, i32, i32, i32, vp], i32),
     "pdmk_fid_accumulate": ([vp, i32, i32, i32, vp, vp, vp], i32),
     "pdmk_gemm_splitk_workspace_bytes": ([i64, i32, i32], i64),
+    "pdmk_gemm_splitk_counters": ([i64, i32], i64),
     "pdmk_groupnorm_workspace_bytes": ([i32, i32], i64),
     "pdmk_groupnorm_bwd_part_workspace_bytes": ([i32, i32], i64),
     "pdmk_layernorm_bwd_part_workspace_bytes": ([i32, i32], i64),
@@ -240,7 +243,7 @@
         g0 = recs[0].g
         kind = ("bf16" if g0.dtype == BF16 else "f32", g0.a_mode, g0.b_mode, _lib.pdmk_gemm_last_candidate(), int(got.value))
         flops = sum(2.0 * (r.macs if r.macs is not None else r.g.M * r.g.N * r.g.K) for r in recs)
-        PROFILE.append((kind, flops, e0, e1, [(r.g.M, r.g.N, r.g.K, int(r.g.splitk), int(bool(r.g.R) or r.g.accumulate == 1))
+        PROFILE.append((kind, flops, e0, e1, [(r.g.M, r.g.N, r.g.K, int(r.g.splitk), int(bool(r.g.R) or r.g.accumulate in (1, 4)))
                                                for r in recs]))
     return int(got.value)
 
@@ -279,7 +282,8 @@
 
 def gemm(A, B, Cout, M, N, K, lda, ldb, ldc, *, bias=None, rowvec=None, rows_per_b=0, R=None, ldr=0,
          a_mode=A_ROWK, b_mode=B_ROWK, conv=None, dtype=None, out_f32=False, accumulate=False, splitk=1, alpha=1.0,
-         macs=None, colsum_out=None, ldrv=0, epilogue=EPI_NONE, C2=None, ldc2=0, colstat=None, ln=None):
+         macs=None, colsum_out=None, ldrv=0, epilogue=EPI_NONE, C2=None, ldc2=0, colstat=None, ln=None, sk_ws=None,
+         sk_cnt=None):
     g = GemmArgs()
     g.colsum_out = _p(colsum_out)
     g.A, g.B, g.C = _p(A), _p(B), _p(Cout)
@@ -296,10 +300,11 @@
     if colstat is not None:
         g.colstat, g.cs_ld, g.cs_col0 = _p(colstat[0]), colstat[0].shape[2], int(colstat[1])
     _set_ln(g, ln)
-    shape = (M, N, K, int(splitk), int(R is not None or int(accumulate) == 1))
+    g.sk_ws, g.sk_cnt = _p(sk_ws), _p(sk_cnt)
+    shape = (M, N, K, int(splitk), int(R is not None or int(accumulate) in (1, 4)))
     if RECORD is not None:
         RECORD.append(Rec("gemm", lambda: _launch_gemm(g, macs, shape), g=g, macs=macs,
-                          keep=(A, B, Cout, bias, rowvec, R, colsum_out, C2, colstat, ln)))
+                          keep=(A, B, Cout, bias, rowvec, R, colsum_out, C2, colstat, ln, sk_ws, sk_cnt)))
         return
     _launch_gemm(g, macs, shape)
 
@@ -445,7 +450,10 @@
     return buf.value.decode()
 
 
-def splitk_plan(A, B, M, N, K, lda, ldb, a_mode=A_ROWK, conv=None):
+FORM_TWO_PASS, FORM_INLAUNCH = 0, 1
+
+
+def splitk_plan_form(A, B, M, N, K, lda, ldb, a_mode=A_ROWK, conv=None):
     g = GemmArgs()
     g.A, g.B = _p(A), _p(B)
     g.M, g.N, g.K = M, N, K
@@ -455,9 +463,48 @@
         (g.conv_b, g.conv_hi, g.conv_wi, g.conv_ci, g.conv_ho, g.conv_wo, g.conv_mode, g.conv_ld) = conv
     g.dtype = dt(A)
     g.splitk, g.alpha = 1, 1.0
-    sk = i32(1)
-    _chk(_lib.pdmk_gemm_plan(C.byref(g), _st(), C.byref(sk)), "pdmk_gemm_plan")
-    return int(sk.value)
+    sk, form = i32(1), i32(0)
+    _chk(_lib.pdmk_gemm_plan_form(C.byref(g), _st(), C.byref(sk), C.byref(form)), "pdmk_gemm_plan_form")
+    return int(sk.value), int(form.value)
+
+
+def splitk_plan(A, B, M, N, K, lda, ldb, a_mode=A_ROWK, conv=None):
+    return splitk_plan_form(A, B, M, N, K, lda, ldb, a_mode, conv)[0]
+
+
+class SplitCounters:
+
+    def __init__(self, device, n=1 << 18):
+        self.buf = torch.zeros(n, device=device, dtype=torch.int32)
+        self.off = 0
+
+    def begin(self):
+        self.off = 0
+
+    def take(self, n):
+        n = (int(n) + 63) & ~63
+        if self.off + n > self.buf.numel():
+            return None
+        t = self.buf[self.off:self.off + n]
+        self.off += n
+        return t
+
+
+COUNTERS = None
+_DEFAULT_COUNTERS = {}
+
+
+def _default_counters(device):
+    dev = torch.device(device)
+    key = (dev.index if dev.index is not None else torch.cuda.current_device(), _st())
+    c = _DEFAULT_COUNTERS.get(key)
+    if c is None:
+        c = _DEFAULT_COUNTERS[key] = SplitCounters(dev)
+    return c
+
+
+def splitk_counters(M, N):
+    return _ws_bytes(_lib.pdmk_gemm_splitk_counters(M, N))
 
 
 def wgrad_plan(dy, x, M, N, K, lda, ldb, b_mode=B_COLK, conv=None, slabs=False):
@@ -477,17 +524,33 @@
 
 
 def gemm_auto(A, B, Cout, M, N, K, lda, ldb, ldc, *, bias=None, rowvec=None, rows_per_b=0, R=None, ldr=0,
-              a_mode=A_ROWK, conv=None, accumulate=False, macs=None, ldrv=0, colstat=None):
-    sk = splitk_plan(A, B, M, N, K, lda, ldb, a_mode, conv)
+              a_mode=A_ROWK, conv=None, accumulate=False, macs=None, ldrv=0, colstat=None, form=None, counters=None):
+    sk, pform = splitk_plan_form(A, B, M, N, K, lda, ldb, a_mode, conv)
     if sk == 1:
         gemm(A, B, Cout, M, N, K, lda, ldb, ldc, bias=bias, rowvec=rowvec, rows_per_b=rows_per_b, R=R, ldr=ldr,
              a_mode=a_mode, conv=conv, accumulate=accumulate, macs=macs, ldrv=ldrv, colstat=colstat)
         return colstat is not None
+    form = pform if form is None else form
     ws = torch.empty(_ws_bytes(_lib.pdmk_gemm_splitk_workspace_bytes(M, N, sk)) // 4, device=A.device, dtype=torch.float32)
+    if (form == FORM_INLAUNCH and INLAUNCH and colstat is None and dt(Cout) == BF16 and N % 8 == 0 and ldc % 8 == 0 and
+            (R is None or ldr % 8 == 0)):
+        if counters is None and COUNTERS is not None and COUNTERS.buf.device == A.device:
+            counters = COUNTERS
+        cnt = (counters if counters is not None else _default_counters(A.device)).take(splitk_counters(M, N))
+        if cnt is None and counters is None:
+            _default_counters(A.device).begin()
+            cnt = _default_counters(A.device).take(splitk_counters(M, N))
+        if cnt is not None:
+            gemm(A, B, Cout, M, N, K, lda, ldb, ldc, bias=bias, rowvec=rowvec, rows_per_b=rows_per_b, R=R, ldr=ldr, a_mode=a_mode,
+                 conv=conv, splitk=sk, accumulate=4 if accumulate else 3, macs=macs, ldrv=ldrv, sk_ws=ws, sk_cnt=cnt)
+            return False
     gemm(A, B, ws, M, N, K, lda, ldb, N, a_mode=a_mode, conv=conv, out_f32=True, splitk=sk, accumulate=2, macs=macs)
     splitk_finish(ws, Cout, M, N, ldc, sk, bias=bias, rowvec=rowvec, R=R, ldr=ldr, rows_per_b=rows_per_b, ldrv=ldrv,
                   accumulate=accumulate, colstat=colstat)
     return colstat is not None
+
+
+INLAUNCH = os.environ.get("PDMK_SPLITK_INLAUNCH", "1") != "0"
 
 
 @_recordable("splitk_finish")
diff --git a/unlearn-ft_amd/pdm/models/unet/engine.py b/unlearn-ft_amd/pdm/models/unet/engine.py
--- a/unlearn-ft_amd/pdm/models/unet/engine.py
+++ b/unlearn-ft_amd/pdm/models/unet/engine.py
@@ -74,6 +74,7 @@
         self._wg_items = None
         self._cs_arena, self._cs_off, self._cs_need, self._cs_old = None, 0, 0, []
         self._cs_views, self._cs_cats = {}, {}
+        self._sk_cnt = k.SplitCounters(self.dev)
 
     def _empty(self, rows, cols, dtype=None):
         return torch.empty((rows, cols), device=self.dev, dtype=dtype or self.dtype)
@@ -657,6 +658,8 @@
         self.train = train
         self.tape = []
         self._cs_begin()
+        self._sk_cnt.begin()
+        k.COUNTERS = self._sk_cnt
         T = ehs.shape[0] // B
         c0 = cfg.block_out_channels[0]
         k.TAG = "time_embedding"
@@ -735,6 +738,7 @@
 
     def backward(self):
         tape, self.tape = self.tape, []
+        k.COUNTERS = self._sk_cnt
         for fn in reversed(tape):
             fn()
         self._join_wgrad()
```

Measured after the change: 188.5 images/s. No clear change (-0.7%).
